# OpenPPL/ppq

Hardware: AMD Instinct MI355X
Metric: calibration samples/sec (RuntimeCalibrationPass, KL 2048-bin, ResNet-50 INT8) (higher is better)
Workload: dtype f32; 1 GPU; ResNet-50 topology (53 Conv + 1 Gemm, BN folded, seeded He init), RuntimeCalibrationPass kl 2048 bins, per-tensor INT8 activations, per-channel INT8 weights, 279 batches x 32 x 3x224x224 per GPU; samples=8928, batch=32, observed_tensors=72, rccl_ranks=1, async_observe=False, cache_params=False, channels_last=False, fuse_params=True, batch_observations=True, reuse_activations=False, replayed_batches=0, hip_graph=auto, graph_replays=0, miopen_find=False

## Files before the change

include/ppq_hip.h:

```cpp
#ifndef PPQ_HIP_H_
#define PPQ_HIP_H_

#include <stdint.h>

#ifdef __cplusplus
extern "C" {
#endif

typedef enum {
    PPQHIP_OK = 0,
    PPQHIP_ERR_INVALID_VALUE = -1,
    PPQHIP_ERR_UNSUPPORTED = -2,
    PPQHIP_ERR_HIP = -3
} ppqhip_status;

#define PPQHIP_ABI_VERSION 4

const char* ppqhip_last_error(void);
int ppqhip_version(void);
int ppqhip_device_arch(char* buf, int n);

int ppqhip_fq_linear_t(const float* x, const float* scale, const float* offset, float* out,
                       int64_t n, int clip_min, int clip_max, int rounding, void* stream);

// ... 49 lines not shown
    int64_t n, num_channel, elem_per_channel;
    int32_t clip_min, clip_max;
} ppqhip_lsq_job;
int ppqhip_fq_linear_c_bwd_multi(const ppqhip_lsq_job* jobs, int num_jobs, int rounding, void* stream);

int ppqhip_fq_float_t(const float* x, const float* scale, const float* offset, float* out,
                      int64_t n, int exponent, int mantissa, float clip_min, float clip_max,
                      int rounding, void* stream);

int ppqhip_fq_float_c(const float* x, const float* scale, const float* offset, float* out,
                      int64_t n, int64_t num_channel, int64_t elem_per_channel,
                      int exponent, int mantissa, float clip_min, float clip_max,
                      int rounding, void* stream);

typedef struct ppqhip_float_search_job {
    const float* x;
    int64_t rows, row_len;
    int32_t exponent, mantissa;
    float clip_min, clip_max;
} ppqhip_float_search_job;
int64_t ppqhip_float_scale_search_table_bytes(int num_jobs);
int ppqhip_float_scale_search(const ppqhip_float_search_job* jobs, int num_jobs, const float* candidates,
                              int num_candidates, int rounding, void* device_table, double* out, void* stream);

typedef struct ppqhip_fq_float_job {
    const float* x;
    const float* scale;
    const float* offset;
    float* out;
    int64_t n, num_channel, elem_per_channel;
    int32_t exponent, mantissa;
    float clip_min, clip_max;
} ppqhip_fq_float_job;
int64_t ppqhip_fq_float_multi_table_bytes(int num_jobs);
int ppqhip_fq_float_multi(const ppqhip_fq_float_job* jobs, int num_jobs, int rounding, void* device_table,
                          int upload, void* stream);

int ppqhip_fq_float_c_bwd(const float* x, const float* scale, const float* offset,
                          const float* grad_y, float* grad_x, float* grad_s, int64_t n,
                          int64_t num_channel, int64_t elem_per_channel,
                          int exponent, int mantissa, float clip_min, float clip_max,
                          int rounding, void* stream);

int64_t ppqhip_hist_workspace_bytes(int64_t n, int64_t num_bins);
int ppqhip_hist_sym_t(const float* x, int64_t n, float hist_scale, int clip_outliers,
                      int32_t* hist, int64_t num_bins, void* workspace, void* stream);

int ppqhip_hist_asym_t(const float* x, int64_t n, float min_value, float max_value,
                       int clip_outliers, int32_t* hist, int64_t num_bins, void* workspace,
                       void* stream);

int ppqhip_hist_sym_c(const float* x, int64_t n, int64_t num_channel, int64_t elem_per_channel,
                      float hist_scale, int clip_outliers, int32_t* hist, int64_t num_bins,
                      void* stream);

int ppqhip_hist_sym_c_scales(const float* x, int64_t n, int64_t num_channel, int64_t elem_per_channel,
                             const float* hist_scales, int clip_outliers, int32_t* hist,
                             int64_t num_bins, void* stream);
int ppqhip_hist_asym_c_ranges(const float* x, int64_t n, int64_t num_channel, int64_t elem_per_channel,
                              const float* mins, const float* maxs, int clip_outliers, int32_t* hist,
                              int64_t num_bins, void* stream);

int64_t ppqhip_quantile_workspace_bytes(int64_t n);
int ppqhip_quantile_t(const float* x, int64_t n, float q, float* dest, uint32_t* hint, void* workspace,
                      void* stream);

typedef struct ppqhip_quantile_job {
    const float* x;
    float* dest;
    uint32_t* hint;
    int64_t n;
} ppqhip_quantile_job;
int64_t ppqhip_quantile_multi_workspace_bytes(int num_jobs, int64_t total_elems);
int ppqhip_quantile_t_multi(const ppqhip_quantile_job* jobs, int num_jobs, float q, void* workspace,
                            void* stream);
void ppqhip_quantile_debug_layout(int64_t* out);
void ppqhip_quantile_hot_layout(int64_t* out);

int ppqhip_isotone_t(const float* x, int64_t n, float* dest, void* workspace, void* stream);

int64_t ppqhip_minmax_workspace_bytes(int64_t n);
int ppqhip_minmax_t(const float* x, int64_t n, float* minmax, void* workspace, void* stream);

int ppqhip_minmax_c(const float* x, int64_t n, int64_t num_channel, int64_t elem_per_channel,
                    float* mins, float* maxs, void* stream);

typedef struct ppqhip_minmax_c_job {
    const float* x;
    float* mins;
    float* maxs;
    int64_t n, num_channel, elem_per_channel;
    int32_t fresh, reserved;
} ppqhip_minmax_c_job;
int ppqhip_minmax_c_multi(const ppqhip_minmax_c_job* jobs, int num_jobs, void* stream);

int ppqhip_channel_sum(const float* x, int64_t n, int64_t num_channel, int64_t elem_per_channel,
                       double* sums, void* stream);

int64_t ppqhip_hist_rows(void);
int ppqhip_hist_sym_t_rows(const float* x, int64_t n, float hist_scale, int clip_outliers,
                           int32_t* rows, int64_t num_bins, void* stream);
int ppqhip_hist_asym_t_rows(const float* x, int64_t n, float min_value, float max_value,
                            int clip_outliers, int32_t* rows, int64_t num_bins, void* stream);
typedef struct ppqhip_minmax_job {
    const float* x;
    float* slots;
    int64_t n;
} ppqhip_minmax_job;
int ppqhip_minmax_t_slots_multi(const ppqhip_minmax_job* jobs, int num_jobs, void* stream);

typedef struct ppqhip_hist_job {
    const float* x;
    int32_t* rows;
    int64_t n;
    float p0, p1;
} ppqhip_hist_job;
int ppqhip_hist_t_rows_multi(const ppqhip_hist_job* jobs, int num_jobs, int asymmetric,
                             int clip_outliers, int64_t num_bins, void* stream);
int ppqhip_hist_rows_finish(const int32_t* rows, int64_t num_bins, int32_t* hist, void* stream);
int ppqhip_check_bin_rule(const float* x, int64_t n, float min_value, float hist_scale, int asymmetric, uint64_t* out, void* stream);
int64_t ppqhip_minmax_slots(void);
int ppqhip_minmax_t_slots(const float* x, int64_t n, float* slots, void* stream);
int ppqhip_minmax_slots_finish(const float* slots, float* minmax, void* stream);

float ppqhip_mse_loss_host(const int64_t* hist, int64_t num_bins, int start, int step, int end);

int64_t ppqhip_mse_search_workspace_bytes(int64_t num_hist);
int ppqhip_mse_search(const int32_t* hist, int64_t num_hist, int64_t num_bins,
                      const double* hist_scale, const double* min_value,
                      int quant_min, int quant_max, int symmetrical, int32_t* best,
                      void* workspace, void* stream);

int64_t ppqhip_kl_num_candidates(int64_t num_bins, int num_of_bits);
int ppqhip_kl_losses(const int32_t* hist, int64_t num_hist, int64_t num_bins, int num_of_bits,
                     double* losses, void* stream);

int ppqhip_tensor_clip_t(const float* value, const float* reference, const float* limit,
                         float* out, int64_t n, void* stream);
int ppqhip_tensor_clip_c(const float* value, const float* reference, const float* limit,
                         float* out, int64_t n, int64_t num_channel, int64_t elem_per_channel,
                         void* stream);
int ppqhip_rounding_loss(const float* x, const float* scale, const float* offset, float* out,
                         int64_t n, int64_t num_channel, int64_t elem_per_channel,
                         int clip_min, int clip_max, int rounding, void* stream);
int ppqhip_rounding_loss_bwd(const float* x, const float* dy, const float* scale,
                             const float* offset, float* dx, int64_t n, int64_t num_channel,
                             int64_t elem_per_channel, int clip_min, int clip_max, int rounding,
                             void* stream);

int ppqhip_bias_act(float* y, const float* bias, int64_t n, int64_t num_channel, int64_t elem_per_channel,
                    int relu, void* stream);
int ppqhip_bias_add_act(float* a, const float* bias_a, float* b, const float* bias_b, float* out,
                        int64_t n, int64_t num_channel, int64_t elem_per_channel, int relu, void* stream);

typedef struct ppqhip_adaround_job {
    const float* w;
    const float* v;
    const float* scale;
    const float* offset;
    float* out;
    const float* dy;
    int64_t n, num_channel, elem_per_channel;
    int32_t qmin, qmax;
} ppqhip_adaround_job;
int ppqhip_adaround_fwd_multi(const ppqhip_adaround_job* jobs, int num_jobs, void* stream);
int ppqhip_adaround_bwd_multi(const ppqhip_adaround_job* jobs, int num_jobs, const float* reg, void* stream);

typedef struct ppqhip_roundtune_job {
    const float* w;
    const float* r;
    const float* scale;
    const float* offset;
    float* out;
    int64_t n, num_channel, elem_per_channel;
    int32_t qmin, qmax;
} ppqhip_roundtune_job;
int ppqhip_roundtune_fwd_multi(const ppqhip_roundtune_job* jobs, int num_jobs, void* stream);

typedef struct ppqhip_fetch_rows_job {
    const float* x;
    const int32_t* index;
    float* out;
    int64_t rows, row_len, count;
} ppqhip_fetch_rows_job;
int ppqhip_fetch_rows_multi(const ppqhip_fetch_rows_job* jobs, int num_jobs, void* stream);
typedef struct ppqhip_measure_rows_job {
    const float* p;
    const float* r;
    const int32_t* index;
    double* sums;
    int64_t rows, row_len, count;
} ppqhip_measure_rows_job;
int ppqhip_measure_rows_multi(const ppqhip_measure_rows_job* jobs, int num_jobs, void* stream);
enum { PPQHIP_MEASURE_SNR = 0, PPQHIP_MEASURE_MSE = 1, PPQHIP_MEASURE_COSINE = 2 };
enum { PPQHIP_REDUCE_MEAN = 0, PPQHIP_REDUCE_MAX = 1 };
typedef struct ppqhip_measure_finish_job {
    const double* sums;
    double* acc;
    float* row_out;
    int64_t rows, count;
    int32_t method, reduce;
} ppqhip_measure_finish_job;
int ppqhip_measure_finish_multi(const ppqhip_measure_finish_job* jobs, int num_jobs, void* stream);

typedef struct ppqhip_equalize_segment {
    const float* base;
    int64_t extent;
    int64_t div, a, b;
    int64_t outer, stride, run;
    float multiplier;
    int32_t downstream;
} ppqhip_equalize_segment;
typedef struct ppqhip_equalize_scale_job {
    const ppqhip_equalize_segment* segments;
    float* scale;
    int32_t num_segments, num_channel;
    float value_threshold;
    int32_t reserved;
} ppqhip_equalize_scale_job;
int ppqhip_equalize_scale_multi(const ppqhip_equalize_scale_job* jobs, int num_jobs, void* stream);
typedef struct ppqhip_equalize_apply_job {
    float* x;
    const float* scale;
    int64_t n, run, inner, group_out;
    int64_t num_scale;
    int32_t divide, reserved;
} ppqhip_equalize_apply_job;
int ppqhip_equalize_apply_multi(const ppqhip_equalize_apply_job* jobs, int num_jobs, void* stream);

typedef struct ppqhip_split_plan_job {
    const ppqhip_equalize_segment* segments;
    int32_t* src_of;
    int32_t* count;
    int32_t num_segments, num_channel;
    float value_threshold;
    int32_t reserved;
} ppqhip_split_plan_job;
int ppqhip_split_plan_multi(const ppqhip_split_plan_job* jobs, int num_jobs, void* stream);
typedef struct ppqhip_split_apply_job {
    const float* x;
    float* out;
    const int32_t* src_of;
    int64_t n, run;
    int32_t num_channel, count;
} ppqhip_split_apply_job;
int ppqhip_split_apply_multi(const ppqhip_split_apply_job* jobs, int num_jobs, void* stream);

typedef struct ppqhip_ssd_scales_job {
    ppqhip_equalize_segment first, last;
    const float* act_range;
    float* scales;
    float* ranges;
    int32_t num_channel;
    float channel_ratio;
} ppqhip_ssd_scales_job;
int ppqhip_ssd_scales_multi(const ppqhip_ssd_scales_job* jobs, int num_jobs, void* stream);
typedef struct ppqhip_ssd_apply_job {
    const float* x;
    float* out;
    const float* scales;
    int64_t n, run, inner, group_out;
    int64_t num_channel;
    int32_t divide, reserved;
} ppqhip_ssd_apply_job;
int ppqhip_ssd_apply_multi(const ppqhip_ssd_apply_job* jobs, int num_jobs, void* stream);
typedef struct ppqhip_fq_measure_rows_job {
    const float* y;
    const float* r;
    const float* scale;
    const float* offset;
    double* sums;
    int64_t rows, count;
    int64_t num_channel, elem_per_channel;
    int32_t clip_min, clip_max, rounding, reserved;
} ppqhip_fq_measure_rows_job;
int ppqhip_fq_measure_rows_multi(const ppqhip_fq_measure_rows_job* jobs, int num_jobs, void* stream);

typedef struct ppqhip_stat_job {
    const float* p;
    const float* r;
    float* rec;
    int64_t n;
    int32_t bins, reserved;
} ppqhip_stat_job;
int ppqhip_stat_moments_multi(const ppqhip_stat_job* jobs, int num_jobs, void* stream);
int ppqhip_stat_shape_multi(const ppqhip_stat_job* jobs, int num_jobs, void* stream);

enum { PPQHIP_MXFP8_E4M3 = 0, PPQHIP_MXFP8_E5M2 = 1, PPQHIP_MXFP6_E3M2 = 2, PPQHIP_MXFP6_E2M3 = 3, PPQHIP_MXFP4_E2M1 = 4,
       PPQHIP_MXINT8 = 5 };
int ppqhip_mx_fq(const float* x, float* y, uint8_t* scale_codes, int64_t outer, int64_t axis_len, int64_t inner, int format,
                 void* stream);
typedef struct ppqhip_mx_job {
    const float* x;
    float* y;
    uint8_t* scale_codes;
    int64_t outer, axis_len, inner;
    int32_t format, reserved;
} ppqhip_mx_job;
int ppqhip_mx_fq_multi(const ppqhip_mx_job* jobs, int num_jobs, void* stream);

int ppqhip_mx_pack(const float* x, uint8_t* elements, uint8_t* scales, int64_t outer, int64_t axis_len, int64_t inner, int format,
                   void* stream);
typedef struct ppqhip_mx_pack_job {
    const float* x;
    uint8_t* elements;
    uint8_t* scales;
// ... 35 lines not shown
```

ppq_amd/_lib.py:

```python
import ctypes
import os

_HERE = os.path.dirname(os.path.abspath(__file__))
LIB_PATH = os.path.join(_HERE, 'libppq_hip.so')

c_f32p = ctypes.c_void_p
c_i32p = ctypes.c_void_p
c_f64p = ctypes.c_void_p
c_i64 = ctypes.c_int64
c_int = ctypes.c_int
c_flt = ctypes.c_float
c_vp = ctypes.c_void_p

ABI_VERSION = 4


class ProfEntry(ctypes.Structure):
    _fields_ = [('name', ctypes.c_char * 48), ('launches', ctypes.c_int64),
                ('total_ms', ctypes.c_double), ('total_bytes', ctypes.c_double)]


PROTOTYPES = {
    'ppqhip_last_error': (ctypes.c_char_p, []),
    'ppqhip_version': (c_int, []),
    'ppqhip_device_arch': (c_int, [ctypes.c_char_p, c_int]),
    'ppqhip_fq_linear_t': (c_int, [c_f32p, c_f32p, c_f32p, c_f32p, c_i64, c_int, c_int, c_int, c_vp]),
    'ppqhip_fq_linear_c': (c_int, [c_f32p, c_f32p, c_f32p, c_f32p, c_i64, c_i64, c_i64, c_int, c_int, c_int, c_vp]),
    'ppqhip_to_int_t': (c_int, [c_f32p, c_f32p, c_f32p, c_vp, c_i64, c_int, c_int, c_int, c_int, c_vp]),
    'ppqhip_to_int_c': (c_int, [c_f32p, c_f32p, c_f32p, c_vp, c_i64, c_i64, c_i64, c_int, c_int, c_int, c_int, c_vp]),
    'ppqhip_fq_linear_t_bwd': (c_int, [c_f32p, c_f32p, c_f32p, c_f32p, c_f32p, c_f32p, c_i64, c_int, c_int, c_int,
                                       c_vp]),
    'ppqhip_fq_linear_c_bwd': (c_int, [c_f32p, c_f32p, c_f32p, c_f32p, c_f32p, c_f32p, c_i64, c_i64, c_i64, c_int,
                                       c_int, c_int, c_vp]),
    'ppqhip_fq_linear_c_bwd_multi': (c_int, [c_vp, c_int, c_int, c_vp]),
    'ppqhip_fq_linear_t_bwd_partials': (c_i64, [c_i64]),
    'ppqhip_fq_linear_t_bwd_main': (c_int, [c_f32p, c_f32p, c_f32p, c_f32p, c_f32p, c_f32p, c_i64, c_int, c_int, c_int, c_vp]),
    'ppqhip_lsq_finish_multi': (c_int, [c_vp, c_int, c_vp]),
    'ppqhip_bias_act': (c_int, [c_f32p, c_f32p, c_i64, c_i64, c_i64, c_int, c_vp]),
    'ppqhip_bias_add_act': (c_int, [c_f32p, c_f32p, c_f32p, c_f32p, c_f32p, c_i64, c_i64, c_i64, c_int, c_vp]),
    'ppqhip_fq_float_t': (c_int, [c_f32p, c_f32p, c_f32p, c_f32p, c_i64, c_int, c_int, c_flt, c_flt, c_int, c_vp]),
    'ppqhip_fq_float_c': (c_int, [c_f32p, c_f32p, c_f32p, c_f32p, c_i64, c_i64, c_i64, c_int, c_int, c_flt, c_flt,
                                  c_int, c_vp]),
    'ppqhip_fq_float_c_bwd': (c_int, [c_f32p, c_f32p, c_f32p, c_f32p, c_f32p, c_f32p, c_i64, c_i64, c_i64, c_int,
                                      c_int, c_flt, c_flt, c_int, c_vp]),
    'ppqhip_hist_workspace_bytes': (c_i64, [c_i64, c_i64]),
    'ppqhip_hist_sym_t': (c_int, [c_f32p, c_i64, c_flt, c_int, c_i32p, c_i64, c_vp, c_vp]),
    'ppqhip_hist_asym_t': (c_int, [c_f32p, c_i64, c_flt, c_flt, c_int, c_i32p, c_i64, c_vp, c_vp]),
    'ppqhip_hist_sym_c': (c_int, [c_f32p, c_i64, c_i64, c_i64, c_flt, c_int, c_i32p, c_i64, c_vp]),
    'ppqhip_hist_sym_c_scales': (c_int, [c_f32p, c_i64, c_i64, c_i64, c_f32p, c_int, c_i32p, c_i64, c_vp]),
    'ppqhip_hist_asym_c_ranges': (c_int, [c_f32p, c_i64, c_i64, c_i64, c_f32p, c_f32p, c_int, c_i32p, c_i64, c_vp]),
    'ppqhip_quantile_workspace_bytes': (c_i64, [c_i64]),
    'ppqhip_quantile_t': (c_int, [c_f32p, c_i64, c_flt, c_f32p, c_vp, c_vp, c_vp]),
    'ppqhip_isotone_t': (c_int, [c_f32p, c_i64, c_f32p, c_vp, c_vp]),
    'ppqhip_minmax_workspace_bytes': (c_i64, [c_i64]),
    'ppqhip_minmax_t': (c_int, [c_f32p, c_i64, c_f32p, c_vp, c_vp]),
    'ppqhip_minmax_c': (c_int, [c_f32p, c_i64, c_i64, c_i64, c_f32p, c_f32p, c_vp]),
    'ppqhip_minmax_c_multi': (c_int, [c_vp, c_int, c_vp]),
    'ppqhip_fq_linear_multi_table_bytes': (c_i64, [c_int]),
    'ppqhip_fq_linear_multi': (c_int, [c_vp, c_int, c_int, c_vp, c_int, c_vp]),
    'ppqhip_float_scale_search_table_bytes': (c_i64, [c_int]),
    'ppqhip_float_scale_search': (c_int, [c_vp, c_int, c_vp, c_int, c_int, c_vp, c_vp, c_vp]),
    'ppqhip_fq_float_multi_table_bytes': (c_i64, [c_int]),
    'ppqhip_fq_float_multi': (c_int, [c_vp, c_int, c_int, c_vp, c_int, c_vp]),
    'ppqhip_quantile_multi_workspace_bytes': (c_i64, [c_int, c_i64]),
    'ppqhip_quantile_t_multi': (c_int, [c_vp, c_int, c_flt, c_vp, c_vp]),
    'ppqhip_quantile_debug_layout': (None, [c_vp]),
    'ppqhip_quantile_hot_layout': (None, [c_vp]),
    'ppqhip_minmax_t_slots_multi': (c_int, [c_vp, c_int, c_vp]),
    'ppqhip_hist_t_rows_multi': (c_int, [c_vp, c_int, c_int, c_int, c_i64, c_vp]),
    'ppqhip_channel_sum': (c_int, [c_f32p, c_i64, c_i64, c_i64, c_f64p, c_vp]),
    'ppqhip_hist_rows': (c_i64, []),
    'ppqhip_hist_sym_t_rows': (c_int, [c_f32p, c_i64, c_flt, c_int, c_i32p, c_i64, c_vp]),
    'ppqhip_hist_asym_t_rows': (c_int, [c_f32p, c_i64, c_flt, c_flt, c_int, c_i32p, c_i64, c_vp]),
    'ppqhip_hist_rows_finish': (c_int, [c_i32p, c_i64, c_i32p, c_vp]),
    'ppqhip_check_bin_rule': (c_int, [c_f32p, c_i64, c_flt, c_flt, c_int, c_vp, c_vp]),
    'ppqhip_minmax_slots': (c_i64, []),
    'ppqhip_minmax_t_slots': (c_int, [c_f32p, c_i64, c_f32p, c_vp]),
    'ppqhip_minmax_slots_finish': (c_int, [c_f32p, c_f32p, c_vp]),
    'ppqhip_mse_loss_host': (c_flt, [ctypes.POINTER(ctypes.c_int64), c_i64, c_int, c_int, c_int]),
    'ppqhip_mse_search_workspace_bytes': (c_i64, [c_i64]),
    'ppqhip_mse_search': (c_int, [c_i32p, c_i64, c_i64, c_f64p, c_f64p, c_int, c_int, c_int, c_i32p, c_vp, c_vp]),
    'ppqhip_kl_num_candidates': (c_i64, [c_i64, c_int]),
    'ppqhip_kl_losses': (c_int, [c_i32p, c_i64, c_i64, c_int, c_f64p, c_vp]),
    'ppqhip_tensor_clip_t': (c_int, [c_f32p, c_f32p, c_f32p, c_f32p, c_i64, c_vp]),
    'ppqhip_tensor_clip_c': (c_int, [c_f32p, c_f32p, c_f32p, c_f32p, c_i64, c_i64, c_i64, c_vp]),
    'ppqhip_rounding_loss': (c_int, [c_f32p, c_f32p, c_f32p, c_f32p, c_i64, c_i64, c_i64, c_int, c_int, c_int, c_vp]),
    'ppqhip_rounding_loss_bwd': (c_int, [c_f32p, c_f32p, c_f32p, c_f32p, c_f32p, c_i64, c_i64, c_i64, c_int, c_int,
                                         c_int, c_vp]),
    'ppqhip_adaround_fwd_multi': (c_int, [c_vp, c_int, c_vp]),
    'ppqhip_adaround_bwd_multi': (c_int, [c_vp, c_int, c_f32p, c_vp]),
    'ppqhip_roundtune_fwd_multi': (c_int, [c_vp, c_int, c_vp]),
    'ppqhip_equalize_scale_multi': (c_int, [c_vp, c_int, c_vp]),
    'ppqhip_equalize_apply_multi': (c_int, [c_vp, c_int, c_vp]),
    'ppqhip_split_plan_multi': (c_int, [c_vp, c_int, c_vp]),
    'ppqhip_split_apply_multi': (c_int, [c_vp, c_int, c_vp]),
    'ppqhip_ssd_scales_multi': (c_int, [c_vp, c_int, c_vp]),
    'ppqhip_ssd_apply_multi': (c_int, [c_vp, c_int, c_vp]),
    'ppqhip_fq_measure_rows_multi': (c_int, [c_vp, c_int, c_vp]),
    'ppqhip_fetch_rows_multi': (c_int, [c_vp, c_int, c_vp]),
    'ppqhip_measure_rows_multi': (c_int, [c_vp, c_int, c_vp]),
    'ppqhip_measure_finish_multi': (c_int, [c_vp, c_int, c_vp]),
    'ppqhip_stat_moments_multi': (c_int, [c_vp, c_int, c_vp]),
    'ppqhip_stat_shape_multi': (c_int, [c_vp, c_int, c_vp]),
    'ppqhip_mx_fq': (c_int, [c_f32p, c_f32p, c_vp, c_i64, c_i64, c_i64, c_int, c_vp]),
    'ppqhip_mx_fq_multi': (c_int, [c_vp, c_int, c_vp]),
    'ppqhip_mx_pack': (c_int, [c_f32p, c_vp, c_vp, c_i64, c_i64, c_i64, c_int, c_vp]),
    'ppqhip_mx_pack_multi': (c_int, [c_vp, c_int, c_vp]),
    'ppqhip_mx_unpack': (c_int, [c_vp, c_vp, c_f32p, c_i64, c_i64, c_i64, c_int, c_vp]),
    'ppqhip_mx_unpack_multi': (c_int, [c_vp, c_int, c_vp]),
    'ppqhip_mx_gemm': (c_int, [c_vp, c_vp, c_int, c_vp, c_vp, c_int, c_f32p, c_f32p, c_i64, c_i64, c_i64, c_vp]),
    'ppqhip_prof_enable': (c_int, [c_int]),
    'ppqhip_prof_collect': (c_int, [ctypes.POINTER(ProfEntry), c_int]),
    'ppqhip_prof_event_overhead_us': (ctypes.c_double, [c_vp, c_int]),
}

if not os.path.exists(LIB_PATH):
    raise ImportError(
        f'{LIB_PATH} is missing: the HIP kernel library has not been built.  Run '
        '`python -c "import __graft_entry__ as g; g.build()"` or `make -C ppq_amd/csrc` (needs hipcc, '
        'targets gfx950).  ppq_amd has no CPU / PyTorch fallback by design.')

import torch

_torch_hip = os.path.join(os.path.dirname(torch.__file__), 'lib', 'libamdhip64.so')
if os.path.exists(_torch_hip):
    ctypes.CDLL(_torch_hip, mode=ctypes.RTLD_GLOBAL)

try:
    lib = ctypes.CDLL(LIB_PATH)
except OSError as e:
    raise ImportError(f'cannot load {LIB_PATH}: {e}') from e

for _name, (_res, _args) in PROTOTYPES.items():
    _fn = getattr(lib, _name)
    _fn.restype = _res
    _fn.argtypes = _args


if lib.ppqhip_version() != ABI_VERSION:
    raise ImportError(f'{LIB_PATH} has ABI version {lib.ppqhip_version()}, this package needs {ABI_VERSION}: rebuild it '
                      '(`make -C ppq_amd/csrc` or `python -c "import __graft_entry__ as g; g.build()"`)')


def last_error() -> str:
    msg = lib.ppqhip_last_error()
    return msg.decode('utf-8', 'replace') if msg else ''
```

ppq_amd/calibration.py:

```python
import time
from math import ceil
from typing import Callable, Dict, Iterable, List

from .core import QuantizationStates, state_value
from .distributed import merge_observers
from .observer import OperationObserver, TorchHistObserver, render_observers


class QuantizationOptimizationPass:
    def __init__(self, name: str = 'Default Quanzation Optim') -> None:
        self.name = name

    def apply(self, graph, **kwargs) -> None:
        self.optimize(graph, **kwargs)

    def optimize(self, graph, **kwargs) -> None:
        raise NotImplementedError('Implement this function first.')

    def __str__(self) -> str:
        return 'QuantizationOptimizationPass[' + self.name + ']'


class RuntimeCalibrationPass(QuantizationOptimizationPass):
    AUTO_GRAPH_ISSUE_FRACTION = 0.7
    AUTO_GRAPH_MIN_STEPS = 12

    def __init__(self, method: str = None, override: bool = False, calib_steps: int = 32,
                 process_group=None, check_steps: bool = True, async_observe: bool = False,
                 use_hip_graph: bool = False, batch_observations: bool = True,
                 reuse_activations: bool = False, reuse_budget_bytes: int = 64 << 30,
                 queue_bytes: int = None) -> None:
        super().__init__(name='PPQ Runtime Calibration Pass')
        self._method = method
        self._observers: Dict[str, OperationObserver] = {}
        self._collate_fn = None
        self._calib_steps = calib_steps
        self._override = override
        self._process_group = process_group
        self._check_steps = check_steps
        self._async_observe = async_observe
        self._use_hip_graph = use_hip_graph
        self._batch_observations = batch_observations
        self._queue = None
        self._reuse_activations = reuse_activations
        self._queue_bytes = queue_bytes
        self._reuse_budget = reuse_budget_bytes
        self._replay: list = []
        self._replay_bytes = 0
        self.replay_peak_bytes = 0
        self.replayed_batches = 0
        self._recording = False
        self.graph_replays = 0
        self.graph_decisions = []
        self.merge_stats = []
        self._side_stream = None

    def _batches(self, dataloader: Iterable) -> list:
        out = []
        for calib_epoch in range(ceil(self._calib_steps / len(dataloader))):
            for data in dataloader:
                if self._collate_fn is not None:
                    data = self._collate_fn(data)
                out.append(data)
                if len(out) >= self._calib_steps: return out
        return out

    def _graph_replayable(self, batches: list, hooks: Dict[str, object]) -> bool:
        import torch
        from .observer import ConstantObserver, TorchHistObserver, TorchMinMaxObserver, TorchMSEObserver
        if not self._use_hip_graph or len(batches) < 4: return False
        if not all(isinstance(b, torch.Tensor) and b.is_cuda and b.shape == batches[0].shape
                   and b.dtype == batches[0].dtype for b in batches): return False
        safe = (TorchMinMaxObserver, TorchHistObserver, TorchMSEObserver, ConstantObserver)
        return all(type(ob) in safe for hook in hooks.values() for ob in hook._observer_table.values())

    @ staticmethod
    def _forward_fn(executor):
        return executor.forward

    def _forward(self, executor, data, hooks, output_names):
        import torch
        recording = self._queue is not None and self._recording
        if recording: self._queue.recorder = []
        with torch.no_grad():
            self._forward_fn(executor)(inputs=data, hooks=hooks, output_names=output_names)
        if self._queue is not None: self._queue.flush()
        if recording:
            rec, self._queue.recorder = self._queue.recorder, None
            size = sum(v.numel() * 4 for _, v in rec)
            if self._replay_bytes + size <= self._reuse_budget:
                self._replay.append(rec); self._replay_bytes += size
                self.replay_peak_bytes = max(self.replay_peak_bytes, self._replay_bytes)
            else: self._recording = False

    def _replay_phase2(self, batches: list) -> int:
        n = min(len(self._replay), len(batches))
        for i in range(n):
            for ob, value in self._replay[i]: ob.observe(value)
            self._queue.flush()
            self._replay[i] = None
        self._replay, self._replay_bytes = [], 0
        self.replayed_batches += n
        return n

    def calibrate(self, desc: str, dataloader: Iterable, executor, hooks: Dict[str, object],
                  output_names: List[str] = None):
        import torch
        batches = self._batches(dataloader)
        if self._replay and not self._recording:
            batches = batches[self._replay_phase2(batches):]
            if not batches: return
        if not self._graph_replayable(batches, hooks):
            for data in batches:
                self._forward(executor, data, hooks, output_names)
            return
        self._forward(executor, batches[0], hooks, output_names)
        first = 1
        if self._use_hip_graph == 'auto':
            torch.cuda.synchronize()
            t0 = time.perf_counter()
            self._forward(executor, batches[1], hooks, output_names)
            t1 = time.perf_counter()
            torch.cuda.synchronize()
            t2 = time.perf_counter()
            first = 2
            launch_bound = (t1 - t0) > self.AUTO_GRAPH_ISSUE_FRACTION * (t2 - t0)
            self.graph_decisions.append({'phase': desc, 'issue_ms': (t1 - t0) * 1e3, 'total_ms': (t2 - t0) * 1e3,
                                         'graph': bool(launch_bound and len(batches) - first >= self.AUTO_GRAPH_MIN_STEPS)})
            if not self.graph_decisions[-1]['graph']:
                for data in batches[first:]:
                    self._forward(executor, data, hooks, output_names)
                return
        self._recording = False
        static_in = torch.empty_like(batches[0])
        torch.cuda.synchronize()
        graph = torch.cuda.CUDAGraph()
        with torch.cuda.graph(graph):
            self._forward(executor, static_in, hooks, output_names)
            if self._side_stream is not None:
                torch.cuda.current_stream().wait_stream(self._side_stream)
        for data in batches[first:]:
            static_in.copy_(data, non_blocking=True)
            graph.replay()
            self.graph_replays += 1

    def _all_tensor_observers(self):
        return [ob for op_ob in self._observers.values() for ob in op_ob.observers()]

    def _render(self):
        observers = self._all_tensor_observers()
        if self._queue is not None: self._queue.flush()
        if self._side_stream is not None:
            import torch
            torch.cuda.current_stream().wait_stream(self._side_stream)
        if merge_observers(observers, group=self._process_group):
            from . import distributed
            self.merge_stats.append(dict(distributed.last_merge_stats))
        render_observers(observers)

    def optimize(self, graph, dataloader: Iterable, executor, calib_steps: int = 32,
                 collate_fn: Callable = None, **kwargs) -> None:
        if collate_fn is not None: self._collate_fn = collate_fn
        if calib_steps is not None: self._calib_steps = calib_steps
        if self._check_steps:
            assert self._calib_steps >= 8, (
                'Insufficient Calibration Detected, to get a better quantization performance, '
                'more calibration steps is required, we strongly recommend you to prepare more calibration data '
                'and more calibration steps is preferred here. (at least 8)')
            assert self._calib_steps <= 512, (
                'Calibration steps is too large, ppq can quantize your network within 8-512 '
                'calibration steps. More calibration steps will greatly delay ppq\'s calibration procedure. '
                'Reset your calib_steps parameter please.')

        if self._override:
            for operation in graph.operations.values():
                if not hasattr(operation, 'config'): continue
                for config, var in operation.config_with_variable:
                    if (not var.is_parameter and state_value(config.state) == QuantizationStates.ACTIVATED.value
                            and config.dominated_by == config):
                        config.state = type(config.state).INITIAL

        self._observers = {}
        hooks = {}
        import torch
        if self._async_observe and torch.cuda.is_available():
            self._side_stream = torch.cuda.Stream()
        for op_name, operation in graph.operations.items():
            if not hasattr(operation, 'config'): continue
            for config, var in operation.config_with_variable:
                if not var.is_parameter and self._method is not None:
                    config.observer_algorithm = self._method
            observer = OperationObserver(operation=executor._graph.operations[op_name], monitor_parameter=False)
            observer.hook.stream = self._side_stream
            self._observers[op_name] = observer
            hooks[op_name] = observer.hook

        self._queue = None
        if self._batch_observations and self._side_stream is None:
            from .observer import ObservationQueue
            self._queue = ObservationQueue() if self._queue_bytes is None else ObservationQueue(self._queue_bytes)
        for ob in self._all_tensor_observers(): ob.queue = self._queue

        self._replay, self._replay_bytes = [], 0
        self._recording = bool(self._reuse_activations and self._queue is not None)
        self.calibrate(desc='Calibration Progress(Phase 1)', dataloader=dataloader, executor=executor,
                       hooks=hooks, output_names=None)
        self._recording = False
        self._render()
        if self._replay:
            for observer in self._observers.values():
                for cfg, ob in observer.hook._observer_table.items():
                    if (not getattr(ob._watch_on, 'is_parameter', False)
                            and QuantizationStates.is_activated(cfg.state)):
                        self._replay, self._replay_bytes = [], 0
                        break
                if not self._replay: break

        pop_list = []
        for op_name, observer in self._observers.items():
            if all([not isinstance(var_observer, TorchHistObserver)
                    for var_observer in observer.observers()]):
                pop_list.append(op_name)
        for op_name in pop_list:
            self._observers.pop(op_name)
            hooks.pop(op_name)

        if len(hooks) > 0:
            self.calibrate(desc='Calibration Progress(Phase 2)', dataloader=dataloader, executor=executor,
                           hooks=hooks, output_names=None)
            self._render()


class PPLDSPTIReCalibrationPass(RuntimeCalibrationPass):
    def __init__(self, method: str = None, override: bool = False) -> None:
        super().__init__(method, override)
        self.name = 'PPQ ReCalibration For Computing Op Pass'

    def optimize(self, graph, dataloader: Iterable, executor, calib_steps: int, collate_fn: Callable = None, **kwargs) -> None:
# ... 91 lines not shown
```

ppq_amd/csrc/epilogue.hip:

```cpp
#include "common.hpp"

namespace ppqhip {
namespace {

constexpr int kEpTileU = 2;
constexpr int kEpSmallU = 1;
constexpr long long kEpSmallElems = 1ll << 20;

struct EpArgs {
    float* a;
    const float* bias_a;
    float* b;
    const float* bias_b;
    float* out;
    uint32_t nvec;
    uint32_t tail;
    int ntail;
    FastDiv epc;
    FastDiv nc;
};

__device__ __forceinline__ uint32_t channel_of(uint32_t i, const FastDiv& epc, const FastDiv& nc) {
    const uint32_t row = fdiv(i, epc);
    return row - fdiv(row, nc) * nc.d;
}

__device__ __forceinline__ float act(float v, bool relu) {
    return (relu && !__builtin_isnan(v)) ? __builtin_fmaxf(v, 0.f) : v;
}

__device__ __forceinline__ float4 add4(const float4& x, const float4& y) {
    return make_float4(x.x + y.x, x.y + y.y, x.z + y.z, x.w + y.w);
}

template <bool RELU>
__device__ __forceinline__ float4 act4(const float4& v) {
    return make_float4(act(v.x, RELU), act(v.y, RELU), act(v.z, RELU), act(v.w, RELU));
}

template <bool PLANE>
__device__ __forceinline__ float4 bias4(const float* __restrict__ bias, uint32_t v, const FastDiv& epc, const FastDiv& nc) {
    if (PLANE) {
        const float t = bias[channel_of(v, epc, nc)];
        return make_float4(t, t, t, t);
    }
    const uint32_t i = v * 4u;
    return make_float4(bias[channel_of(i, epc, nc)], bias[channel_of(i + 1, epc, nc)], bias[channel_of(i + 2, epc, nc)],
                       bias[channel_of(i + 3, epc, nc)]);
}

template <bool RESID, bool BIAS_B, bool RELU>
__device__ __forceinline__ void epilogue_elem(const EpArgs& p, uint32_t i, const FastDiv& epc) {
    const uint32_t c = channel_of(i, epc, p.nc);
    const float x = p.a[i] + p.bias_a[c];
    if (!RESID) { p.a[i] = act(x, RELU); return; }
    p.a[i] = x;
    float y = p.b[i];
    if (BIAS_B) { y = y + p.bias_b[c]; p.b[i] = y; }
    p.out[i] = act(x + y, RELU);
}

template <int U, bool RESID, bool BIAS_B, bool RELU, bool PLANE>
__global__ __launch_bounds__(kBlock) void epilogue_kernel(EpArgs p) {
    const uint32_t base = blockIdx.x * (kBlock * U) + threadIdx.x;
    float4* a4 = reinterpret_cast<float4*>(p.a);
    float4* b4 = reinterpret_cast<float4*>(p.b);
    float4* o4 = reinterpret_cast<float4*>(p.out);
    float4 a[U], ba[U], b[U], bb[U];
#pragma unroll
    for (int k = 0; k < U; k++) {
        const uint32_t vv = min(base + k * kBlock, p.nvec - 1);
        a[k] = a4[vv];
        ba[k] = bias4<PLANE>(p.bias_a, vv, p.epc, p.nc);
        if (RESID) b[k] = b4[vv];
        if (BIAS_B) bb[k] = bias4<PLANE>(p.bias_b, vv, p.epc, p.nc);
    }
#pragma unroll
    for (int k = 0; k < U; k++) {
        const uint32_t vv = base + k * kBlock;
        if (vv >= p.nvec) continue;
        const float4 x = add4(a[k], ba[k]);
        if (!RESID) { a4[vv] = act4<RELU>(x); continue; }
        a4[vv] = x;
        float4 y = b[k];
        if (BIAS_B) { y = add4(y, bb[k]); b4[vv] = y; }
        o4[vv] = act4<RELU>(add4(x, y));
    }
    if (!PLANE && blockIdx.x == 0 && (int)threadIdx.x < p.ntail)
        epilogue_elem<RESID, BIAS_B, RELU>(p, p.tail + threadIdx.x, p.epc);
}

template <bool RESID, bool BIAS_B, bool RELU>
__global__ __launch_bounds__(kBlock) void epilogue_scalar_kernel(EpArgs p) {
    const uint32_t stride = gridDim.x * kBlock;
    for (uint32_t i = blockIdx.x * kBlock + threadIdx.x; i < (uint32_t)p.ntail; i += stride)
        epilogue_elem<RESID, BIAS_B, RELU>(p, i, p.epc);
}

template <bool RESID, bool BIAS_B, bool RELU>
void launch_epilogue(EpArgs p, int64_t n, int64_t C, int64_t epc, bool aligned, hipStream_t st) {
    p.nc = make_fastdiv((uint32_t)C);
    if (!aligned || n < 4) {
        p.nvec = 0; p.tail = 0; p.ntail = (int)n;
        p.epc = make_fastdiv((uint32_t)epc);
        hipLaunchKernelGGL((epilogue_scalar_kernel<RESID, BIAS_B, RELU>), dim3(stream_grid(n, kBlock)), dim3(kBlock), 0, st, p);
        return;
    }
    p.nvec = (uint32_t)(n >> 2);
    p.tail = p.nvec * 4u;
    p.ntail = (int)(n & 3);
    const bool plane = (epc % 4 == 0);
    p.epc = make_fastdiv((uint32_t)(plane ? epc / 4 : epc));
#define PPQ_LAUNCH_EP(U, PLANE)                                                                                          \
    hipLaunchKernelGGL((epilogue_kernel<U, RESID, BIAS_B, RELU, PLANE>), dim3((p.nvec + kBlock * U - 1) / (kBlock * U)),   \
                       dim3(kBlock), 0, st, p)
    if (n <= kEpSmallElems) {
        if (plane) PPQ_LAUNCH_EP(kEpSmallU, true); else PPQ_LAUNCH_EP(kEpSmallU, false);
    } else {
        if (plane) PPQ_LAUNCH_EP(kEpTileU, true); else PPQ_LAUNCH_EP(kEpTileU, false);
    }
#undef PPQ_LAUNCH_EP
}

int validate(int64_t n, int64_t C, int64_t epc, const char* what) {
    if (n <= 0 || n > 0x7fffffffLL) {
        set_error("%s: n=%lld is empty or has more than 2^31 - 1 elements", what, (long long)n);
        return PPQHIP_ERR_INVALID_VALUE;
    }
    if (C <= 0 || epc <= 0 || C > 0x7fffffffLL || epc > 0x7fffffffLL || n % (C * epc) != 0) {
        set_error("%s: n=%lld is not [outer, %lld channels, %lld elem/channel]", what, (long long)n, (long long)C,
                  (long long)epc);
        return PPQHIP_ERR_INVALID_VALUE;
    }
    return PPQHIP_OK;
}

}
}

using namespace ppqhip;

extern "C" {

int ppqhip_bias_act(float* y, const float* bias, int64_t n, int64_t num_channel, int64_t elem_per_channel, int relu,
                    void* stream) {
    if (int st = validate(n, num_channel, elem_per_channel, "bias_act")) return st;
    if (!y || !bias) { set_error("bias_act: null pointer"); return PPQHIP_ERR_INVALID_VALUE; }
    hipStream_t s = (hipStream_t)stream;
    EpArgs p{};
    p.a = y; p.bias_a = bias;
    const bool aligned = aligned16(y);
    if (relu) launch_epilogue<false, false, true>(p, n, num_channel, elem_per_channel, aligned, s);
    else launch_epilogue<false, false, false>(p, n, num_channel, elem_per_channel, aligned, s);
    return finish_launch("bias_act");
}

int ppqhip_bias_add_act(float* a, const float* bias_a, float* b, const float* bias_b, float* out, int64_t n,
                        int64_t num_channel, int64_t elem_per_channel, int relu, void* stream) {
    if (int st = validate(n, num_channel, elem_per_channel, "bias_add_act")) return st;
    if (!a || !bias_a || !b || !out) { set_error("bias_add_act: null pointer"); return PPQHIP_ERR_INVALID_VALUE; }
    hipStream_t s = (hipStream_t)stream;
    EpArgs p{};
    p.a = a; p.bias_a = bias_a; p.b = b; p.bias_b = bias_b; p.out = out;
    const bool aligned = aligned16(a) && aligned16(b) && aligned16(out);
    if (bias_b) {
        if (relu) launch_epilogue<true, true, true>(p, n, num_channel, elem_per_channel, aligned, s);
        else launch_epilogue<true, true, false>(p, n, num_channel, elem_per_channel, aligned, s);
    } else {
        if (relu) launch_epilogue<true, false, true>(p, n, num_channel, elem_per_channel, aligned, s);
        else launch_epilogue<true, false, false>(p, n, num_channel, elem_per_channel, aligned, s);
    }
    return finish_launch("bias_add_act");
}

}
```

ppq_amd/csrc/hist.hip:

```cpp
#include "common.hpp"

namespace ppqhip {

constexpr int kMaxLdsBins = 16384;
constexpr int kLdsBudgetInts = 2048;
constexpr int kHistBlock = 512;
constexpr int kHistWgPerCu = 2;
constexpr int kHistU = 2;
constexpr int kHistMinTiles = 2;
constexpr int kHistAtomicMaxWg = 128;
constexpr long long kHistNtElems = 48ll << 20;
constexpr int kHistRows = kNumCU * kHistWgPerCu;
constexpr uint32_t kTileVec = (uint32_t)kHistBlock * kHistU;
constexpr uint32_t kTileElems = kTileVec * 4;
static_assert(kHistBlock % 64 == 0 && kHistBlock >= 64 && kHistBlock <= 1024, "histogram workgroup: whole waves");

typedef float v2f __attribute__((ext_vector_type(2)));

struct BinRule {
    float a;
    float hs;
    float rcp;
    int bins;
    int clip;
    int asym;
};
static BinRule make_rule(float a, float hs, int bins, int clip, int asym) {
    BinRule r; r.a = a; r.hs = hs; r.rcp = 1.0f / hs; r.bins = bins; r.clip = clip; r.asym = asym;
    return r;
}

__device__ __forceinline__ bool quotient_is_safe(float t) {
    return __builtin_fabsf(t - __builtin_rintf(t)) >= __builtin_fabsf(t) * 0x1p-22f;
}

__device__ __forceinline__ int f2i_abs(float t) {
    int r;
    asm("v_cvt_i32_f32_e64 %0, |%1|" : "=v"(r) : "v"(t));
    return r;
}
__device__ __forceinline__ int f2i_floor(float t) {
    int r;
    asm("v_cvt_flr_i32_f32 %0, %1" : "=v"(r) : "v"(t));
    return r;
}

template <bool ASYM, bool CLIP, bool HOT>
struct Binner : WaveBinCounter<ASYM, CLIP, HOT> {
    using Base = WaveBinCounter<ASYM, CLIP, HOT>;
    using Base::h; using Base::last; using Base::hot_bin; using Base::hot_cnt;
    float a0, hs, rcp;

    __device__ __forceinline__ void set_rule(float a, float scale) { a0 = a; hs = scale; rcp = 1.0f / scale; }

    __device__ __forceinline__ void bins4(const float4& v, int (&b)[4]) const {
        v2f x01 = {v.x, v.y}, x23 = {v.z, v.w};
        if (ASYM) { x01 = x01 - a0; x23 = x23 - a0; }
        const v2f t01 = x01 * rcp, t23 = x23 * rcp;
        const v2f r01 = {__builtin_rintf(t01.x), __builtin_rintf(t01.y)};
        const v2f r23 = {__builtin_rintf(t23.x), __builtin_rintf(t23.y)};
        const v2f d01 = t01 - r01, d23 = t23 - r23;
        const v2f e01 = t01 * 0x1p-22f, e23 = t23 * 0x1p-22f;
        const bool u0 = !(__builtin_fabsf(d01.x) >= __builtin_fabsf(e01.x));
        const bool u1 = !(__builtin_fabsf(d01.y) >= __builtin_fabsf(e01.y));
        const bool u2 = !(__builtin_fabsf(d23.x) >= __builtin_fabsf(e23.x));
        const bool u3 = !(__builtin_fabsf(d23.y) >= __builtin_fabsf(e23.y));
        b[0] = ASYM ? f2i_floor(t01.x) : f2i_abs(t01.x);
        b[1] = ASYM ? f2i_floor(t01.y) : f2i_abs(t01.y);
        b[2] = ASYM ? f2i_floor(t23.x) : f2i_abs(t23.x);
        b[3] = ASYM ? f2i_floor(t23.y) : f2i_abs(t23.y);
        if (u0 | u1 | u2 | u3) {
            if (u0) b[0] = exact_bin(ASYM ? x01.x : __builtin_fabsf(v.x));
            if (u1) b[1] = exact_bin(ASYM ? x01.y : __builtin_fabsf(v.y));
            if (u2) b[2] = exact_bin(ASYM ? x23.x : __builtin_fabsf(v.z));
            if (u3) b[3] = exact_bin(ASYM ? x23.y : __builtin_fabsf(v.w));
        }
    }
    __device__ __forceinline__ int exact_bin(float a) const { return f2i_sat(__builtin_floorf(a / hs)); }

    __device__ __forceinline__ int bin1(float v) const {
        const float a = ASYM ? (v - a0) : __builtin_fabsf(v);
        const float t = a * rcp;
        if (quotient_is_safe(t)) return ASYM ? f2i_floor(t) : f2i_abs(t);
        return exact_bin(a);
    }

};

constexpr int kReduceBins = 32, kReduceSlices = 32, kReduceBlock = kReduceBins * kReduceSlices;
__global__ __launch_bounds__(kReduceBlock) void hist_reduce_kernel(const int* __restrict__ partial, int count, int bins,
                                                                   int* __restrict__ hist) {
    __shared__ int lds[kReduceSlices][kReduceBins];
    const int lane_bin = threadIdx.x % kReduceBins, slice = threadIdx.x / kReduceBins;
    const int b = blockIdx.x * kReduceBins + lane_bin;
    int total = 0;
    if (b < bins) {
        int i = slice;
        for (; i + 15 * kReduceSlices < count; i += 16 * kReduceSlices) {
            int v[16];
#pragma unroll
            for (int k = 0; k < 16; k++) v[k] = partial[(size_t)(i + k * kReduceSlices) * bins + b];
#pragma unroll
            for (int k = 0; k < 16; k++) total += v[k];
        }
        for (; i < count; i += kReduceSlices) total += partial[(size_t)i * bins + b];
    }
    lds[slice][lane_bin] = total;
    __syncthreads();
    if (slice == 0 && b < bins) {
        int t = 0;
#pragma unroll
        for (int k = 0; k < kReduceSlices; k++) t += lds[k][lane_bin];
        if (t) hist[b] += t;
    }
}

constexpr int kMultiMax = 96;
enum FlushMode : int {
    FLUSH_ROWS_ADD = 0,
    FLUSH_ROWS_STORE = 1,
    FLUSH_ATOMIC = 2
};
struct HistJob {
    const float* x;
    int* rows;
    uint32_t n;
    float a, hs;
    uint32_t first_tile;
};
struct HistJobs {
    HistJob job[kMultiMax];
    uint32_t count;
    uint32_t total_tiles;
    int bins, copies, mode;
};
__host__ __device__ inline uint32_t job_tiles(uint32_t n, bool vec_ok) {
    if (!vec_ok) return (n + kTileElems - 1) / kTileElems;
    const uint32_t full = (n >> 2) / kTileVec;
    return full + (n > full * kTileElems ? 1u : 0u);
}

__device__ __forceinline__ void lds_hist_flush(int* lds, int bins, int copies, int* __restrict__ dst, int mode) {
    asm volatile("s_waitcnt lgkmcnt(0)" ::: "memory");
    __syncthreads();
    for (int b = threadIdx.x; b < bins; b += kHistBlock) {
        int s = 0;
        for (int c = 0; c < copies; c++) { s += lds[c * bins + b]; lds[c * bins + b] = 0; }
        if (mode == FLUSH_ROWS_STORE) dst[b] = s;
        else if (s) {
            if (mode == FLUSH_ROWS_ADD) dst[b] += s;
            else atomicAdd(&dst[b], s);
        }
    }
    __syncthreads();
}

template <bool ASYM, bool CLIP, bool HOT, bool NT>
__global__ __launch_bounds__(kHistBlock, (kHistBlock * kHistWgPerCu + 255) / 256)
void hist_persistent_kernel(const HistJobs jobs) {
    extern __shared__ int lds[];
    const uint32_t G = gridDim.x, g = blockIdx.x;
    uint32_t t, t_end;
    even_split(jobs.total_tiles, G, g, t, t_end);
    const int bins = jobs.bins, copies = jobs.copies;
    bool zeroed = false;
    auto zero_lds = [&]() {
        if (zeroed) return;
        for (int i = threadIdx.x; i < copies * bins; i += kHistBlock) lds[i] = 0;
        asm volatile("s_waitcnt lgkmcnt(0)\n\ts_barrier" ::: "memory");
        zeroed = true;
    };
    if (t >= t_end) {
        if (jobs.mode == FLUSH_ROWS_STORE) for (int b = threadIdx.x; b < bins; b += kHistBlock) jobs.job[0].rows[(size_t)g * bins + b] = 0;
        return;
    }
    uint32_t lo = 0, hi = jobs.count;
    while (hi - lo > 1) {
        const uint32_t mid = (lo + hi) >> 1;
        if (jobs.job[mid].first_tile <= t) lo = mid; else hi = mid;
    }
    Binner<ASYM, CLIP, HOT> acc;
    acc.init(lds + ((threadIdx.x >> 6) % copies) * bins, bins);

    for (uint32_t j = lo; t < t_end; j++) {
        const HistJob& job = jobs.job[j];
        const uint32_t j_end = (j + 1 < jobs.count) ? jobs.job[j + 1].first_tile : jobs.total_tiles;
        uint32_t k = t - job.first_tile;
        const uint32_t k1 = min(t_end, j_end) - job.first_tile;
        t = min(t_end, j_end);
        acc.set_rule(job.a, job.hs);
        const float* __restrict__ x = job.x;
        const uint32_t n = job.n;
        const bool vec_ok = (reinterpret_cast<uintptr_t>(x) & 15u) == 0;
        const uint32_t full = vec_ok ? (n >> 2) / kTileVec : 0u;
        const uint32_t kf = min(k1, full);
        if (k < kf) {
            const float4* xv = reinterpret_cast<const float4*>(x) + threadIdx.x;
            float4 bufa[kHistU], bufb[kHistU];
            auto fetch = [&](float4 (&buf)[kHistU], uint32_t tile) {
                const float4* p = xv + (size_t)tile * kTileVec;
#pragma unroll
                for (int u = 0; u < kHistU; u++) buf[u] = load4<NT>(p + u * kHistBlock);
            };
            auto consume = [&](const float4 (&buf)[kHistU], uint32_t tile) {
#pragma unroll
                for (int u = 0; u < kHistU; u++) {
                    int b[4];
                    acc.bins4(buf[u], b);
                    if (u == 0) acc.elect(b[0], true);
                    if (CLIP && HOT) acc.commit4_exec(b);
                    else {
                        acc.template commit<true>(b[0], true); acc.template commit<true>(b[1], true);
                        acc.template commit<true>(b[2], true); acc.template commit<true>(b[3], true);
                    }
                }
            };
            fetch(bufa, k);
            zero_lds();
            for (;;) {
                fetch(bufb, min(k + 1, kf - 1));
                consume(bufa, k);
                if (++k >= kf) break;
                fetch(bufa, min(k + 1, kf - 1));
                consume(bufb, k);
                if (++k >= kf) break;
            }
        }
        zero_lds();
        for (; k < k1; k++) {
            const uint32_t e0 = k * kTileElems + threadIdx.x;
#pragma unroll 4
            for (int r = 0; r < 4 * kHistU; r++) {
                const uint32_t i = e0 + r * kHistBlock;
                const bool in = i < n;
                const float a = in ? x[i] : 0.f;
                const int b = acc.bin1(a);
                if ((r & 3) == 0) acc.elect(b, in);
                acc.template commit<false>(b, in);
            }
        }
// ... 659 lines not shown
```

ppq_amd/ffi.py:

```python
import math
import threading
import weakref
from typing import List

import numpy as np
import torch

from . import _lib
from ._lib import lib

_KERNEL_FAILURE = 'Kernel Failure, '


_raw_stream = torch._C._cuda_getCurrentRawStream
_get_device = torch._C._cuda_getDevice


def _stream() -> int:
    return _raw_stream(_get_device())


def _check(t: torch.Tensor, dtype: torch.dtype, name: str) -> None:
    if not isinstance(t, torch.Tensor):
        raise TypeError(f'{name}: expected a torch.Tensor, got {type(t)}')
# ... 7 lines not shown

_F32 = torch.float32


def _f32(t, name):
    try:
        if t.dtype is _F32 and t.is_cuda and t.numel() > 0: return
    except AttributeError:
        pass
    _check(t, torch.float32, name + '(Expect to be FP32)')


def _dense(t: torch.Tensor, channel_axis=None) -> torch.Tensor:
    if t.is_contiguous(): return t
    if channel_axis is None or channel_axis % t.dim() == 0:
        if t.dim() == 4 and t.is_contiguous(memory_format=torch.channels_last): return t
        if t.dim() == 5 and t.is_contiguous(memory_format=torch.channels_last_3d): return t
    return t.contiguous()


def _raise(status: int) -> None:
    if status != 0:
        raise RuntimeError(_KERNEL_FAILURE + _lib.last_error())


def _geometry(shape, channel_axis: int):
    ndim = len(shape)
    if channel_axis < 0: channel_axis += ndim
    if not 0 <= channel_axis < ndim:
        raise RuntimeError(_KERNEL_FAILURE + f'channel_axis {channel_axis} out of range for a {ndim}-d tensor')
    epc = 1
    for d in shape[channel_axis + 1:]:
        epc *= int(d)
    return int(shape[channel_axis]), epc


class _DeviceOf:
    __slots__ = ('idx', 'prev')

    def __init__(self, t: torch.Tensor):
        self.idx = t.device.index
        self.prev = None

    def __enter__(self):
        if self.idx is not None and self.idx != _get_device():
            self.prev = _get_device()
            torch.cuda.set_device(self.idx)

    def __exit__(self, *a):
        if self.prev is not None:
            torch.cuda.set_device(self.prev)


_workspaces = {}
_MAX_WORKSPACES = 16


def _workspace(device: torch.device, nbytes: int) -> torch.Tensor:
    key = (device.index, _stream())
    ws = _workspaces.pop(key, None)
    if ws is None or ws.numel() < nbytes:
        ws = torch.empty(max(nbytes, 1 << 16), dtype=torch.uint8, device=device)
    _workspaces[key] = ws
    while len(_workspaces) > _MAX_WORKSPACES:
        _workspaces.pop(next(iter(_workspaces)))
    return ws


_MINMAX_JOB = np.dtype([('x', '<u8'), ('slots', '<u8'), ('n', '<i8')])
_FQ_JOB = np.dtype([('x', '<u8'), ('scale', '<u8'), ('offset', '<u8'), ('out', '<u8'), ('n', '<i8'),
                    ('num_channel', '<i8'), ('elem_per_channel', '<i8'), ('clip_min', '<i4'), ('clip_max', '<i4')])
_FQ_FLOAT_JOB = np.dtype([('x', '<u8'), ('scale', '<u8'), ('offset', '<u8'), ('out', '<u8'), ('n', '<i8'),
                          ('num_channel', '<i8'), ('elem_per_channel', '<i8'), ('exponent', '<i4'), ('mantissa', '<i4'),
                          ('clip_min', '<f4'), ('clip_max', '<f4')])
_FLOAT_SEARCH_JOB = np.dtype([('x', '<u8'), ('rows', '<i8'), ('row_len', '<i8'), ('exponent', '<i4'), ('mantissa', '<i4'),
                              ('clip_min', '<f4'), ('clip_max', '<f4')])
_LSQ_JOB = np.dtype([('x', '<u8'), ('scale', '<u8'), ('offset', '<u8'), ('grad_y', '<u8'), ('grad_x', '<u8'), ('grad_s', '<u8'),
                     ('n', '<i8'), ('num_channel', '<i8'), ('elem_per_channel', '<i8'), ('clip_min', '<i4'), ('clip_max', '<i4')])
_LSQ_FINISH_JOB = np.dtype([('partial', '<u8'), ('grad_s', '<u8'), ('n', '<i8'), ('clip_min', '<i4'), ('clip_max', '<i4')])
_MINMAX_C_JOB = np.dtype([('x', '<u8'), ('mins', '<u8'), ('maxs', '<u8'), ('n', '<i8'), ('num_channel', '<i8'),
                          ('elem_per_channel', '<i8'), ('fresh', '<i4'), ('reserved', '<i4')])
_QUANTILE_JOB = np.dtype([('x', '<u8'), ('dest', '<u8'), ('hint', '<u8'), ('n', '<i8')])

_owner_hints = weakref.WeakKeyDictionary()
_hint_owner = threading.local()


def quantile_hint(device: torch.device) -> torch.Tensor:
    return torch.zeros(8, dtype=torch.int32, device=device)


class quantile_hint_owner:
    __slots__ = ('owner', 'prev')

    def __init__(self, owner):
        self.owner, self.prev = owner, None

    def __enter__(self):
        self.prev = getattr(_hint_owner, 'current', None)
        _hint_owner.current = self.owner
        return self

    def __exit__(self, *a):
        _hint_owner.current = self.prev


def _owner_quantile_hint(device: torch.device, numel: int, q: float):
    owner = getattr(_hint_owner, 'current', None)
    if owner is None: return None
    try: per = _owner_hints.setdefault(owner, {})
    except TypeError: return None
    key = (device.index, int(numel), float(q))
    h = per.get(key)
    if h is None: h = per[key] = quantile_hint(device)
    return h


_HIST_JOB = np.dtype([('x', '<u8'), ('rows', '<u8'), ('n', '<i8'), ('p0', '<f4'), ('p1', '<f4')])


def _epilogue_geometry(ts, bias_list):
    t0 = ts[0]
    if not isinstance(t0, torch.Tensor) or t0.dtype is not _F32 or not t0.is_cuda or t0.dim() != 4 or t0.numel() == 0:
        return None
    shape, strides, dev = t0.shape, t0.stride(), t0.device
    for t in ts[1:]:
        if not isinstance(t, torch.Tensor) or t.dtype is not _F32 or t.device != dev or t.shape != shape or t.stride() != strides:
            return None
    C = int(shape[1])
    for bias in bias_list:
        if (not isinstance(bias, torch.Tensor) or bias.dtype is not _F32 or bias.device != dev or bias.dim() != 1
                or bias.numel() != C or not bias.is_contiguous()):
            return None
    if t0.is_contiguous(): return C, int(shape[2]) * int(shape[3])
    if t0.is_contiguous(memory_format=torch.channels_last): return C, 1
    return None


def bias_act_(y: torch.Tensor, bias: torch.Tensor, relu: bool) -> bool:
    geo = _epilogue_geometry([y], [bias])
    if geo is None: return False
    with _DeviceOf(y):
        _raise(lib.ppqhip_bias_act(y.data_ptr(), bias.data_ptr(), y.numel(), geo[0], geo[1], 1 if relu else 0, _stream()))
    return True


def bias_add_act(a: torch.Tensor, bias_a: torch.Tensor, b: torch.Tensor, bias_b, relu: bool):
    geo = _epilogue_geometry([a, b], [bias_a] if bias_b is None else [bias_a, bias_b])
    if geo is None or a.data_ptr() == b.data_ptr(): return None
    out = torch.empty_like(a)
    with _DeviceOf(a):
        _raise(lib.ppqhip_bias_add_act(a.data_ptr(), bias_a.data_ptr(), b.data_ptr(), 0 if bias_b is None else bias_b.data_ptr(),
                                       out.data_ptr(), a.numel(), geo[0], geo[1], 1 if relu else 0, _stream()))
    return out


_ADAROUND_JOB = np.dtype([('w', '<u8'), ('v', '<u8'), ('scale', '<u8'), ('offset', '<u8'), ('out', '<u8'), ('dy', '<u8'),
                          ('n', '<i8'), ('num_channel', '<i8'), ('elem_per_channel', '<i8'), ('qmin', '<i4'), ('qmax', '<i4')])


def _adaround_table(items, outs, dys=None):
    n = len(items)
    if len(outs) != n or (dys is not None and len(dys) != n):
        raise RuntimeError(_KERNEL_FAILURE + 'AdaRound: argument lists differ in length')
    jobs = np.zeros(n, dtype=_ADAROUND_JOB)
    dev = items[0][0].device
    for k, (w, v, s, o, axis, qmin, qmax) in enumerate(items):
        ts = [('Value', w), ('Rounding', v), ('Scale', s), ('Offset', o), ('Out', outs[k])] + ([('Dy', dys[k])] if dys is not None else [])
        for name, t in ts:
            _f32(t, name)
            if t.device != dev: raise RuntimeError(_KERNEL_FAILURE + f'AdaRound: item {k}: {name} is on another device')
            if not t.is_contiguous(): raise RuntimeError(_KERNEL_FAILURE + f'AdaRound: item {k}: {name} is not contiguous')
        for name, t in ts[1:2] + ts[4:]:
            if t.shape != w.shape: raise RuntimeError(_KERNEL_FAILURE + f'AdaRound: item {k}: {name} is not shaped like the weight')
        C, epc = _geometry(w.shape, axis) if axis is not None else (1, w.numel())
        if s.numel() != C or o.numel() != C:
            raise RuntimeError(_KERNEL_FAILURE + f'AdaRound: item {k}: scale / offset need {C} elements')
        jobs[k] = (w.data_ptr(), v.data_ptr(), s.data_ptr(), o.data_ptr(), outs[k].data_ptr(),
                   dys[k].data_ptr() if dys is not None else 0, w.numel(), C, epc, int(qmin), int(qmax))
    return jobs


def adaround_forward_multi(items, outs=None) -> List[torch.Tensor]:
    if not items: return []
    if outs is None: outs = [torch.empty_like(it[0]) for it in items]
    jobs = _adaround_table(items, outs)
    with _DeviceOf(items[0][0]):
        _raise(lib.ppqhip_adaround_fwd_multi(jobs.ctypes.data, len(items), _stream()))
    return outs


def adaround_backward_multi(items, dys, reg: torch.Tensor, dvs=None) -> List[torch.Tensor]:
    if not items: return []
    _f32(reg, 'Reg')
    if reg.numel() != 3 or not reg.is_contiguous() or reg.device != items[0][0].device:
        raise RuntimeError(_KERNEL_FAILURE + 'AdaRound: reg must be a contiguous float32[3] on the weights\' device')
    if dvs is None: dvs = [torch.empty_like(it[0]) for it in items]
    jobs = _adaround_table(items, dvs, dys)
    with _DeviceOf(items[0][0]):
        _raise(lib.ppqhip_adaround_bwd_multi(jobs.ctypes.data, len(items), reg.data_ptr(), _stream()))
    return dvs


_ROUNDTUNE_JOB = np.dtype([('w', '<u8'), ('r', '<u8'), ('scale', '<u8'), ('offset', '<u8'), ('out', '<u8'),
                           ('n', '<i8'), ('num_channel', '<i8'), ('elem_per_channel', '<i8'), ('qmin', '<i4'), ('qmax', '<i4')])


def _roundtune_table(items, outs):
    n = len(items)
    if len(outs) != n: raise RuntimeError(_KERNEL_FAILURE + 'RoundTuning: argument lists differ in length')
    jobs = np.zeros(n, dtype=_ROUNDTUNE_JOB)
    dev = items[0][0].device
    for k, (w, r, s, o, axis, qmin, qmax) in enumerate(items):
        ts = [('Value', w), ('Rounding', r), ('Scale', s), ('Offset', o), ('Out', outs[k])]
        for name, t in ts:
            _f32(t, name)
            if t.device != dev: raise RuntimeError(_KERNEL_FAILURE + f'RoundTuning: item {k}: {name} is on another device')
            if not t.is_contiguous(): raise RuntimeError(_KERNEL_FAILURE + f'RoundTuning: item {k}: {name} is not contiguous')
        for name, t in ts[1:2] + ts[4:]:
            if t.shape != w.shape: raise RuntimeError(_KERNEL_FAILURE + f'RoundTuning: item {k}: {name} is not shaped like the weight')
        C, epc = _geometry(w.shape, axis) if axis is not None else (1, w.numel())
        if s.numel() != C or o.numel() != C:
            raise RuntimeError(_KERNEL_FAILURE + f'RoundTuning: item {k}: scale / offset need {C} elements')
        jobs[k] = (w.data_ptr(), r.data_ptr(), s.data_ptr(), o.data_ptr(), outs[k].data_ptr(), w.numel(), C, epc, int(qmin), int(qmax))
    return jobs


def roundtune_forward_multi(items, outs=None) -> List[torch.Tensor]:
    if not items: return []
    if outs is None: outs = [torch.empty_like(it[0]) for it in items]
    jobs = _roundtune_table(items, outs)
    with _DeviceOf(items[0][0]):
        _raise(lib.ppqhip_roundtune_fwd_multi(jobs.ctypes.data, len(items), _stream()))
    return outs


_EQ_SEGMENT = np.dtype([('base', '<u8'), ('extent', '<i8'), ('div', '<i8'), ('a', '<i8'), ('b', '<i8'), ('outer', '<i8'),
                        ('stride', '<i8'), ('run', '<i8'), ('multiplier', '<f4'), ('downstream', '<i4')])
_EQ_SCALE_JOB = np.dtype([('segments', '<u8'), ('scale', '<u8'), ('num_segments', '<i4'), ('num_channel', '<i4'),
                          ('value_threshold', '<f4'), ('reserved', '<i4')])
_EQ_APPLY_JOB = np.dtype([('x', '<u8'), ('scale', '<u8'), ('n', '<i8'), ('run', '<i8'), ('inner', '<i8'), ('group_out', '<i8'),
                          ('num_scale', '<i8'), ('divide', '<i4'), ('reserved', '<i4')])


def _eq_tensor(t, what: str, k: int, dev):
    _f32(t, what)
    if t.device != dev: raise RuntimeError(_KERNEL_FAILURE + f'Equalization: item {k}: {what} is on another device')
    if not t.is_contiguous(): raise RuntimeError(_KERNEL_FAILURE + f'Equalization: item {k}: {what} is not contiguous')


def _segment_record(segment, k: int, dev, what: str = 'Value') -> tuple:
    t, div, a, b, outer, stride, run, mult, down = segment
    _eq_tensor(t, what, k, dev)
    return (t.data_ptr(), t.numel(), int(div), int(a), int(b), int(outer), int(stride), int(run), float(mult), 1 if down else 0)


class EqualizeTable:
    __slots__ = ('jobs', 'segments', 'keep', 'entry')

    def __init__(self, jobs, segments, keep, entry):
        self.jobs, self.segments, self.keep, self.entry = jobs, segments, keep, entry

    def __len__(self) -> int: return len(self.jobs)

    def run(self) -> None:
        if len(self.jobs) == 0: return
        with _DeviceOf(self.keep[0]):
            _raise(self.entry(self.jobs.ctypes.data, len(self.jobs), _stream()))


def equalize_scale_table(items) -> EqualizeTable:
    jobs = np.zeros(len(items), dtype=_EQ_SCALE_JOB)
    segs = np.zeros(sum(len(it[2]) for it in items), dtype=_EQ_SEGMENT)
    keep, records = [], []
    dev = items[0][0].device if items else None
    for k, (scale, threshold, segments) in enumerate(items):
        _eq_tensor(scale, 'Scale', k, dev)
        keep.append(scale)
        jobs[k] = (segs.ctypes.data + len(records) * _EQ_SEGMENT.itemsize, scale.data_ptr(), len(segments), scale.numel(), float(threshold), 0)
        for segment in segments:
            records.append(_segment_record(segment, k, dev))
            keep.append(segment[0])
    segs[:] = records
    return EqualizeTable(jobs, segs, keep, lib.ppqhip_equalize_scale_multi)


def equalize_apply_table(items) -> EqualizeTable:
    jobs = np.zeros(len(items), dtype=_EQ_APPLY_JOB)
    keep = []
    dev = items[0][0].device if items else None
    for k, (x, scale, run, inner, group_out, divide) in enumerate(items):
        _eq_tensor(x, 'Value', k, dev); _eq_tensor(scale, 'Scale', k, dev)
        keep += [x, scale]
        jobs[k] = (x.data_ptr(), scale.data_ptr(), x.numel(), int(run), int(inner), int(group_out), scale.numel(), 1 if divide else 0, 0)
    return EqualizeTable(jobs, None, keep, lib.ppqhip_equalize_apply_multi)


def equalize_scale_multi(items) -> None:
    (items if isinstance(items, EqualizeTable) else equalize_scale_table(items)).run()


def equalize_apply_multi(items) -> None:
    (items if isinstance(items, EqualizeTable) else equalize_apply_table(items)).run()


_SPLIT_PLAN_JOB = np.dtype([('segments', '<u8'), ('src_of', '<u8'), ('count', '<u8'), ('num_segments', '<i4'), ('num_channel', '<i4'),
# ... 1498 lines not shown
```

ppq_amd/harness.py:

```python
from typing import Callable, Dict, List, Optional

import torch
import torch.nn.functional as F

from .core import LinearQuantizationConfig, QuantizationStates, TensorQuantizationConfig, is_initial
from .core import QuantizationProperty as P
from .qfunction import PPQuantFunction

PASSIVE_OPERATIONS = {'MaxPool', 'GlobalMaxPool', 'Reshape', 'Flatten', 'Identity', 'Dropout', 'Slice', 'Pad', 'Resize',
                      'Split', 'Transpose', 'Interp', 'Squeeze', 'Unsqueeze'}
COMPUTING_OP = {'Conv', 'Gemm', 'ConvTranspose', 'MatMul'}


class Variable:
    def __init__(self, name: str, value: torch.Tensor = None, is_parameter: bool = False):
        self.name = name
        self.value = value
        self.stored_value = None
        self.is_parameter = is_parameter
        self.dest_ops: List['Operation'] = []
        self.source_op: Optional['Operation'] = None

    def __hash__(self): return hash(self.name)
    def __eq__(self, o): return isinstance(o, Variable) and o.name == self.name
# ... 60 lines not shown
        return self

    def baking_parameters(self, quant_func: Callable):
        for config, var in self.config_with_variable:
            if var.is_parameter and QuantizationStates.is_activated(config.state):
                var.value = quant_func(var.value, config)
                config.state = (QuantizationStates.BAKED if config.state == QuantizationStates.ACTIVATED
                                else QuantizationStates.PASSIVE_BAKED)


class BaseGraph:
    def __init__(self, name: str):
        self.name = name
        self.operations: Dict[str, Operation] = {}
        self.variables: Dict[str, Variable] = {}
        self.inputs: Dict[str, Variable] = {}
        self.outputs: Dict[str, Variable] = {}

    def create_variable(self, name: str, value=None, is_parameter=False) -> Variable:
        v = Variable(name, value, is_parameter)
        self.variables[name] = v
        return v

    def create_operation(self, op_type: str, name: str, inputs: List[Variable], attributes: dict = None) -> Variable:
        out = self.create_variable(name + '_out')
        op = Operation(name, op_type, attributes, list(inputs), [out])
        out.source_op = op
        for v in inputs: v.dest_ops.append(op)
        self.operations[name] = op
        return out

    def topological_sort(self) -> List[Operation]:
        return list(self.operations.values())


def _forward(op: Operation, x: List[torch.Tensor]):
    t, a = op.type, op.attributes
    if t == 'Conv':
        return F.conv2d(x[0], x[1], x[2] if len(x) > 2 else None, stride=a.get('strides', 1),
                        padding=a.get('pads', 0), groups=a.get('group', 1))
    if t == 'Gemm': return F.linear(x[0], x[1], x[2] if len(x) > 2 else None)
    if t == 'MatMul': return torch.matmul(x[0], x[1])
    if t == 'Relu': return F.relu(x[0])
    if t == 'Gelu': return F.gelu(x[0])
    if t == 'Add': return x[0] + x[1]
    if t == 'MaxPool': return F.max_pool2d(x[0], a['kernel_shape'], a.get('strides', 1), a.get('pads', 0))
    if t == 'GlobalAveragePool': return F.adaptive_avg_pool2d(x[0], 1)
    if t == 'Flatten': return torch.flatten(x[0], 1)
    if t == 'LayerNormalization': return F.layer_norm(x[0], x[0].shape[-1:], x[1], x[2])
    if t == 'Softmax': return F.softmax(x[0], dim=a.get('axis', -1))
    if t == 'Mul': return x[0] * (x[1] if len(x) > 1 else a['value'])
    if t == 'Reshape': return x[0].reshape(a['shape'])
    if t == 'Transpose': return x[0].permute(a['perm'])
    if t == 'Concat': return torch.cat([v.expand(x[-1].shape[0], *v.shape[1:]) if v.shape[0] == 1 else v for v in x],
                                       dim=a.get('axis', 1))
    if t == 'Slice': return x[0].narrow(a['axis'], a['start'], a['length'])
    if t == 'Resize': return F.interpolate(x[0], scale_factor=a.get('scale', 2), mode=a.get('mode', 'nearest'))
    raise NotImplementedError(f'Graph op: {op.name}({op.type}) has no backend implementation')


class EpilogueGroup:
    __slots__ = ('kind', 'ops', 'convs', 'add', 'relu')

    def __init__(self, kind, ops, convs, add, relu):
        self.kind, self.ops, self.convs, self.add, self.relu = kind, ops, convs, add, relu

    def __repr__(self): return f'{self.kind}({", ".join(op.name for op in self.ops)})'


def _in_cfg(op, i):
    return op.config.input_quantization_config[i] if isinstance(op, QuantableOperation) else None


def _out_cfg(op, i):
    return op.config.output_quantization_config[i] if isinstance(op, QuantableOperation) else None


def plan_epilogues(operations: List[Operation], hooks: Dict[str, object] = None, keep=(), passes_through: Callable = None,
                   grad_enabled: bool = False) -> List[EpilogueGroup]:
    if grad_enabled: return []
    from .observer import CalibrationHook
    hooks = hooks or {}
    keep = set(keep)
    if passes_through is None:
        def passes_through(c): return not QuantizationStates.is_activated(c.state)

    def through(*cfgs): return all(c is None or passes_through(c) for c in cfgs)

    def hooks_ok(members, unwritten):
        for op in members:
            h = hooks.get(op.name)
            if h is None: continue
            if type(h) is not CalibrationHook: return False
            if any(c is not None and c in h._observer_table for c in unwritten): return False
        return True

    def conv_ok(op):
        return (op.type == 'Conv' and len(op.inputs) == 3 and op.inputs[2].is_parameter and len(op.outputs) == 1
                and op.outputs[0].name not in keep)

    def only_feeds(v, op): return len(v.dest_ops) == 1 and v.dest_ops[0] is op

    def relu_after(op, i):
        if i >= len(operations): return None
        r = operations[i]
        out = op.outputs[0]
        if r.type != 'Relu' or len(r.inputs) != 1 or r.inputs[0] is not out or not only_feeds(out, r) or out.name in keep:
            return None
        return r

    def try_p2(i):
        for n_conv in (2, 1):
            j = i + n_conv
            if j + 1 >= len(operations): continue
            add, convs = operations[j], operations[i:j]
            if add.type != 'Add' or len(add.inputs) != 2 or len(add.outputs) != 1 or not all(conv_ok(c) for c in convs): continue
            by_out = {c.outputs[0].name: c for c in convs}
            x0, x1 = add.inputs
            if x0.name not in by_out or x0 is x1: continue
            if n_conv == 2 and x1.name not in by_out: continue
            ordered = [by_out[x0.name]] + ([by_out[x1.name]] if n_conv == 2 else [])
            if not all(only_feeds(c.outputs[0], add) for c in convs): continue
            relu = relu_after(add, j + 1)
            if relu is None: continue
            unwritten = (_out_cfg(add, 0), _in_cfg(relu, 0))
            between = [_out_cfg(c, 0) for c in convs] + [_in_cfg(add, 0), _in_cfg(add, 1)]
            if not through(*unwritten, *between): return None
            members = list(operations[i:j + 2])
            if not hooks_ok(members, unwritten): return None
            return EpilogueGroup('P2', members, ordered, add, relu)
        return None

    def try_p1(i):
        conv = operations[i]
        if not conv_ok(conv): return None
        relu = relu_after(conv, i + 1)
        if relu is None: return None
        unwritten = (_out_cfg(conv, 0), _in_cfg(relu, 0))
        if not through(*unwritten) or not hooks_ok([conv, relu], unwritten): return None
        return EpilogueGroup('P1', [conv, relu], [conv], None, relu)

    groups, i = [], 0
    while i < len(operations):
        g = try_p2(i) if operations[i].type == 'Conv' else None
        if g is None and operations[i].type == 'Conv': g = try_p1(i)
        if g is None:
            i += 1
            continue
        groups.append(g)
        i += len(g.ops)
    return groups


class TorchExecutor:
    def __init__(self, graph: BaseGraph, device: str = 'cuda'):
        self._graph = graph
        self._device = device
        self._default_quant_fn = PPQuantFunction
        self.cache_parameter_quantization = False
        self._param_cache: Dict[str, tuple] = {}
        self.fuse_parameter_quantization = True
        self._plans: list = []
        self._plan_signature = None
        self._plan_cache: Dict[tuple, list] = {}
        self._fused: Dict[tuple, torch.Tensor] = {}
        self._delegates: Dict[object, Callable] = {}
        self.fuse_epilogues = True
        self._epilogue_cache: Dict[tuple, dict] = {}
        self.channels_last = False
        for v in graph.variables.values():
            if v.is_parameter and v.value is not None: v.value = v.value.to(device)

    def use_channels_last(self) -> 'TorchExecutor':
        self.channels_last = True
        for v in self._graph.variables.values():
            if v.is_parameter and isinstance(v.value, torch.Tensor) and v.value.dim() == 4:
                v.value = v.value.contiguous(memory_format=torch.channels_last)
        return self

    def _place(self, value: torch.Tensor) -> torch.Tensor:
        value = value.to(self._device)
        if self.channels_last and value.dim() == 4: value = value.contiguous(memory_format=torch.channels_last)
        return value

    def register_quantize_delegate(self, config, delegator: Callable) -> None:
        self._delegates[config] = delegator

    def remove_quantize_delegate(self, config) -> None:
        self._delegates.pop(config, None)

    def quantize_function(self, tensor: torch.Tensor, config=None) -> torch.Tensor:
        if self._delegates and config in self._delegates:
            return self._delegates[config](tensor, config)
        return self._default_quant_fn(tensor, config)

    def forward_with_gradient(self, inputs, output_names: List[str] = None, hooks=None):
        return TorchExecutor.forward.__wrapped__(self, inputs, output_names, hooks)

    def partial_graph_forward(self, operations: List[Operation], feed_dict: Dict[str, torch.Tensor],
                              output_names: List[str], with_gradient: bool = False) -> List[torch.Tensor]:
        if not with_gradient:
            with torch.no_grad(): return self._partial_graph_forward(operations, feed_dict, output_names)
        return self._partial_graph_forward(operations, feed_dict, output_names)

    def _partial_graph_forward(self, operations, feed_dict, output_names):
        g = self._graph
        for name, value in feed_dict.items(): g.variables[name].value = self._place(value)
        results = [None] * len(output_names)
        self._fused_parameters(operations)
        plan, fused_done = self._epilogue_plan(operations, None, output_names), set()
        for op in operations:
            if op.name in fused_done: continue
            grp = plan.get(op.name)
            vals = self._run_epilogue(grp, lambda v: v.value, None) if grp is not None else None
            if vals is not None:
                for m in grp.ops:
                    fused_done.add(m.name)
                    for v in m.outputs:
                        v.value = vals[v.name]
                        if v.name in output_names: results[output_names.index(v.name)] = v.value
                continue
            raw_in = [v.value for v in op.inputs]
            if any(x is None for x in raw_in):
                raise ValueError(f'partial_graph_forward: input of {op.name} was not fed')
            if isinstance(op, QuantableOperation):
                qin = [self._quantize_parameter(v, c) if v.is_parameter else self.quantize_function(x, c)
                       for v, x, c in zip(op.inputs, raw_in, op.config.input_quantization_config)]
            else: qin = raw_in
            outs = _forward(op, qin)
            outs = list(outs) if isinstance(outs, (list, tuple)) else [outs]
            if isinstance(op, QuantableOperation):
                outs = [self.quantize_function(y, c) for y, c in zip(outs, op.config.output_quantization_config)]
            for v, y in zip(op.outputs, outs):
                v.value = y
                if v.name in output_names: results[output_names.index(v.name)] = y
        for v in g.variables.values():
            if not v.is_parameter: v.value = None
        return results

    def _fused_parameters(self, operations=None) -> None:
        self._fused = {}
        if not self.fuse_parameter_quantization or self._default_quant_fn is not PPQuantFunction: return
        from .ffi import FloatingQuantizePlan, LinearQuantizePlan
        todo, sig = [], []
        for op in (self._graph.operations.values() if operations is None else operations):
            if not isinstance(op, QuantableOperation): continue
            for v, c in zip(op.inputs, op.config.input_quantization_config):
                if not (v.is_parameter and isinstance(v.value, torch.Tensor) and v.value.is_cuda): continue
                if not QuantizationStates.is_activated(c.state) or c in self._delegates: continue
                pol = c.policy
                floating = pol.has_property(P.FLOATING)
                if not (pol.has_property(P.LINEAR) or floating) or pol.has_property(P.DYNAMIC): continue
                if v.value.dtype != torch.float32 or v.value.requires_grad or v.value.numel() == 0: continue
                if not (isinstance(c.scale, torch.Tensor) and isinstance(c.offset, torch.Tensor)): continue
                axis = c.channel_axis if pol.has_property(P.PER_CHANNEL) else None
                if not LinearQuantizePlan.accepts(v.value, c.scale, c.offset, axis): continue
                rnd = int(getattr(c.rounding, 'value', c.rounding))
                todo.append((v, c, axis, rnd, floating))
                sig.append((v.name, id(c), v.value.data_ptr(), c.scale.data_ptr(), c.offset.data_ptr(), tuple(v.value.shape), c.scale.numel(),
                            axis, c.quant_min, c.quant_max, rnd, floating,
                            (c.exponent_bits, c.mantissa_bits) if floating else None))
        if not todo:
            self._plans, self._plan_signature = [], None
            return
        cached = self._plan_cache.get(tuple(sig))
        if cached is not None:
            self._plan_cache[tuple(sig)] = self._plan_cache.pop(tuple(sig))
            self._plans, self._plan_signature = cached, sig
        if sig != self._plan_signature:
            groups: Dict[tuple, list] = {}
            for item in todo: groups.setdefault((item[3], item[4]), []).append(item)
            self._plans = []
            for (rnd, floating), items in groups.items():
                if floating:
                    plan = FloatingQuantizePlan([(v.value, c.scale, c.offset, axis, c.exponent_bits, c.mantissa_bits,
                                                  c.quant_min, c.quant_max) for v, c, axis, _, _ in items], rounding=rnd)
                else:
                    plan = LinearQuantizePlan([(v.value, c.scale, c.offset, axis, c.quant_min, c.quant_max)
                                               for v, c, axis, _, _ in items], rounding=rnd)
                self._plans.append((plan, [(v.name, id(c)) for v, c, _, _, _ in items]))
            self._plan_signature = sig
            if len(self._plan_cache) >= 8: self._plan_cache.pop(next(iter(self._plan_cache)))
            self._plan_cache[tuple(sig)] = self._plans
        for plan, keys in self._plans:
            for key, out in zip(keys, plan.run()): self._fused[key] = out

    def _epilogue_plan(self, operations: List[Operation], hooks, output_names) -> Dict[str, EpilogueGroup]:
        if not self.fuse_epilogues or torch.is_grad_enabled() or self._default_quant_fn is not PPQuantFunction: return {}
        states = tuple(c.state for op in operations if isinstance(op, QuantableOperation)
                       for c in (*op.config.input_quantization_config, *op.config.output_quantization_config))
        sig = (tuple(op.name for op in operations), tuple((k, id(h)) for k, h in hooks.items()) if hooks else (),
               tuple(output_names or ()), tuple(id(c) for c in self._delegates), states)
        plan = self._epilogue_cache.get(sig)
        if plan is None:
            delegates = self._delegates

            def passes_through(c): return not QuantizationStates.is_activated(c.state) and c not in delegates
            groups = plan_epilogues(operations, hooks, set(self._graph.outputs) | set(output_names or ()), passes_through)
            plan = {g.ops[0].name: g for g in groups}
            if len(self._epilogue_cache) >= 8: self._epilogue_cache.pop(next(iter(self._epilogue_cache)))
            self._epilogue_cache[sig] = plan
        return plan

    def _run_epilogue(self, grp: EpilogueGroup, raw_of: Callable, hooks) -> Optional[Dict[str, torch.Tensor]]:
        from .ffi import bias_act_, bias_add_act
        for conv in grp.convs:
            x, w = raw_of(conv.inputs[0]), conv.inputs[1].value
            if not (isinstance(x, torch.Tensor) and x.is_cuda and x.dtype == torch.float32 and x.dim() == 4
                    and isinstance(w, torch.Tensor) and w.dim() == 4): return None
            fmt = torch.channels_last if self.channels_last else torch.contiguous_format
            if not (x.is_contiguous(memory_format=fmt) and w.is_contiguous(memory_format=fmt)): return None
        if grp.add is not None:
            b_var = grp.add.inputs[1]
            if b_var.source_op not in grp.convs:
                b = raw_of(b_var)
                if not (isinstance(b, torch.Tensor) and b.is_cuda and b.dtype == torch.float32): return None
        hooks = hooks or {}
        ys, biases, qins = {}, {}, {}
        for conv in grp.ops[:len(grp.convs)]:
            raw_in = [raw_of(v) for v in conv.inputs]
            qin, in_cfgs = raw_in, None
            if isinstance(conv, QuantableOperation):
                in_cfgs = list(conv.config.input_quantization_config)
                qin = [self._quantize_parameter(v, c) if v.is_parameter else self.quantize_function(x, c)
                       for v, x, c in zip(conv.inputs, raw_in, in_cfgs)]
            hook = hooks.get(conv.name)
            if hook is not None: qin = hook.pre_forward_hook(inputs=raw_in, quant_inputs=qin, quant_configs=in_cfgs)
            a = conv.attributes
            ys[conv.name] = F.conv2d(qin[0], qin[1], None, stride=a.get('strides', 1), padding=a.get('pads', 0),
                                     groups=a.get('group', 1))
            biases[conv.name] = qin[2]
            qins[conv.name] = qin
        if grp.kind == 'P1':
            conv = grp.convs[0]
            y = ys[conv.name]
            if not bias_act_(y, biases[conv.name], relu=True):
                y.add_(biases[conv.name].view(1, -1, 1, 1)).relu_()
            tail = {conv.name: y, grp.relu.name: y}
        else:
            conv_a = grp.convs[0]
            a = ys[conv_a.name]
            conv_b = grp.convs[1] if len(grp.convs) > 1 else None
            b = ys[conv_b.name] if conv_b is not None else raw_of(grp.add.inputs[1])
            out = bias_add_act(a, biases[conv_a.name], b, biases[conv_b.name] if conv_b is not None else None, relu=True)
            if out is None:
                a.add_(biases[conv_a.name].view(1, -1, 1, 1))
                if conv_b is not None: b.add_(biases[conv_b.name].view(1, -1, 1, 1))
                out = F.relu(a + b)
            tail = {conv_a.name: a, grp.add.name: out, grp.relu.name: out}
            if conv_b is not None: tail[conv_b.name] = b
        values: Dict[str, torch.Tensor] = {}
        for op in grp.ops:
            hook = hooks.get(op.name)
            quantable = isinstance(op, QuantableOperation)
            if op.type != 'Conv':
                raw_in = [values[v.name] if v.name in values else raw_of(v) for v in op.inputs]
                qin, in_cfgs = raw_in, None
                if quantable:
                    in_cfgs = list(op.config.input_quantization_config)
                    qin = [self.quantize_function(x, c) for x, c in zip(raw_in, in_cfgs)]
                if hook is not None: hook.pre_forward_hook(inputs=raw_in, quant_inputs=qin, quant_configs=in_cfgs)
            outs = fp_outs = [tail[op.name]]
            out_cfgs = None
            if quantable:
                out_cfgs = list(op.config.output_quantization_config)
                outs = [self.quantize_function(y, c) for y, c in zip(outs, out_cfgs)]
            if hook is not None:
                outs = hook.post_forward_hook(outputs=fp_outs, quant_outputs=outs, quant_configs=out_cfgs)
            for v, y in zip(op.outputs, outs): values[v.name] = y
        return values

    def _quantize_parameter(self, var: Variable, config) -> torch.Tensor:
        hit = self._fused.get((var.name, id(config)))
        if hit is not None: return hit
        """A parameter and its scale do not change between calibration forwards, so its fake-quantised
        value is computed once and kept resident (the reference recomputes it every forward until
        ParameterBakingPass; same values, ppq/executor/torch.py:516-518).  The cache entry is keyed on
        the identity + version of value, scale and offset and on the config state."""
        if not self.cache_parameter_quantization or not QuantizationStates.is_activated(config.state):
            return self.quantize_function(var.value, config)
        key = (var.value.data_ptr(), var.value._version, id(config.scale), config.scale._version,
               id(config.offset), config.offset._version, int(getattr(config.state, 'value', config.state)))
        hit = self._param_cache.get(var.name)
        if hit is not None and hit[0] == key: return hit[1]
        q = self.quantize_function(var.value, config)
        self._param_cache[var.name] = (key, q)
        return q

    @ torch.no_grad()
    def forward_cached(self, inputs, output_names: List[str], cache: Dict[str, torch.Tensor]) -> List[torch.Tensor]:
        g = self._graph
        if isinstance(inputs, torch.Tensor): inputs = {next(iter(g.inputs)): inputs}
        elif isinstance(inputs, (list, tuple)): inputs = {k: v for k, v in zip(g.inputs, inputs)}
        for name, value in inputs.items():
            if name not in cache: cache[name] = self._place(value)
        need, stack = set(), [g.variables[n] for n in output_names]
        while stack:
            v = stack.pop()
            if v.name in cache or v.is_parameter: continue
            op = v.source_op
            if op is None: raise ValueError(f'forward_cached: graph input {v.name} was not fed')
            if op.name in need: continue
            need.add(op.name)
            stack.extend(op.inputs)
        ops = [op for op in g.topological_sort() if op.name in need]
        if ops: self._fused_parameters(ops)
        plan, fused_done = (self._epilogue_plan(ops, None, output_names) if ops else {}), set()
        for op in ops:
            if op.name in fused_done: continue
            grp = plan.get(op.name)
            vals = (self._run_epilogue(grp, lambda v: v.value if v.is_parameter else cache[v.name], None)
                    if grp is not None else None)
            if vals is not None:
                hidden = grp.relu.inputs[0].name
                for m in grp.ops:
                    fused_done.add(m.name)
                    for v in m.outputs:
                        if v.name != hidden: cache[v.name] = vals[v.name]
                continue
            raw_in = [v.value if v.is_parameter else cache[v.name] for v in op.inputs]
            if isinstance(op, QuantableOperation):
                qin = [self._quantize_parameter(v, c) if v.is_parameter else self.quantize_function(x, c)
                       for v, x, c in zip(op.inputs, raw_in, op.config.input_quantization_config)]
            else: qin = raw_in
            outs = _forward(op, qin)
            outs = list(outs) if isinstance(outs, (list, tuple)) else [outs]
            if isinstance(op, QuantableOperation):
                outs = [self.quantize_function(y, c) for y, c in zip(outs, op.config.output_quantization_config)]
            for v, y in zip(op.outputs, outs): cache[v.name] = y
        return [cache[n] for n in output_names]

    @ torch.no_grad()
    def forward(self, inputs, output_names: List[str] = None, hooks: Dict[str, object] = None) -> List[torch.Tensor]:
        g = self._graph
        if isinstance(inputs, torch.Tensor): inputs = {next(iter(g.inputs)): inputs}
        elif isinstance(inputs, (list, tuple)): inputs = {k: v for k, v in zip(g.inputs, inputs)}
        for name, value in inputs.items(): g.variables[name].value = self._place(value)
        stop_early = output_names is not None and not hooks
        if output_names is None: output_names = list(g.outputs)
        results = [None] * len(output_names)
        visited = set()
        self._fused_parameters()
        ops = g.topological_sort()
        plan, fused_done = self._epilogue_plan(ops, hooks, output_names), set()

        def finish(op, outs):
            for v, y in zip(op.outputs, outs):
                v.value = y
                if v.name in output_names: results[output_names.index(v.name)] = y
            visited.add(op.name)
            for v in op.inputs:
                if not v.is_parameter and all(d.name in visited for d in v.dest_ops): v.value = None

        for op in ops:
            if op.name in fused_done: continue
            grp = plan.get(op.name)
            vals = self._run_epilogue(grp, lambda v: v.value, hooks) if grp is not None else None
            if vals is not None:
                for m in grp.ops:
                    fused_done.add(m.name)
                    finish(m, [vals[v.name] for v in m.outputs])
                if stop_early and all(r is not None for r in results): break
                continue
            hook = hooks.get(op.name) if hooks else None
            raw_in = [v.value for v in op.inputs]
            qin = raw_in
            quantable = isinstance(op, QuantableOperation)
            if quantable:
                in_cfgs = list(op.config.input_quantization_config)
                qin = [self._quantize_parameter(v, c) if v.is_parameter else self.quantize_function(x, c)
                       for v, x, c in zip(op.inputs, raw_in, in_cfgs)]
            if hook is not None:
                qin = hook.pre_forward_hook(inputs=raw_in, quant_inputs=qin, quant_configs=in_cfgs)
            outs = _forward(op, qin)
            outs = list(outs) if isinstance(outs, (list, tuple)) else [outs]
            fp_outs = outs
            if quantable:
                out_cfgs = list(op.config.output_quantization_config)
                outs = [self.quantize_function(y, c) for y, c in zip(outs, out_cfgs)]
            if hook is not None:
                outs = hook.post_forward_hook(outputs=fp_outs, quant_outputs=outs, quant_configs=out_cfgs)
            finish(op, outs)
            if stop_early and all(r is not None for r in results): break
        for v in g.variables.values():
            if not v.is_parameter: v.value = None
        return results


def quantize_graph(graph: BaseGraph, activation_algorithm: str = 'kl', per_channel_weight: bool = True,
                   symmetrical: bool = True, weight_symmetrical: bool = True, num_of_bits: int = 8,
                   hist_bins: int = None, fp8: bool = False, passive_bias: bool = False) -> None:
    qmin, qmax = (-(2 ** (num_of_bits - 1)), 2 ** (num_of_bits - 1) - 1) if symmetrical else (0, 2 ** num_of_bits - 1)
    wmin, wmax = (-(2 ** (num_of_bits - 1)), 2 ** (num_of_bits - 1) - 1) if weight_symmetrical else (0, 2 ** num_of_bits - 1)

    def act_cfg():
        if fp8:
            from .core import FloatingQuantizationConfig
            return FloatingQuantizationConfig(calibration='floating')
        c = LinearQuantizationConfig(symmetrical=symmetrical, quant_min=qmin, quant_max=qmax, num_of_bits=num_of_bits,
                                     calibration=activation_algorithm)
        if hist_bins is not None: c.detail['OBSERVER_KL_HIST_BINS_MANUL_OVERRIDE'] = hist_bins
        return c

    for name, op in list(graph.operations.items()):
        in_cfgs = []
        for i, v in enumerate(op.inputs):
            if v.is_parameter and op.type in COMPUTING_OP and i == 1:
                in_cfgs.append(LinearQuantizationConfig(symmetrical=weight_symmetrical, quant_min=wmin, quant_max=wmax,
                                                        num_of_bits=num_of_bits, calibration='minmax',
                                                        channel_axis=0 if per_channel_weight else None))
            elif v.is_parameter and passive_bias and not fp8 and op.type in COMPUTING_OP and i == 2:
                in_cfgs.append(LinearQuantizationConfig(symmetrical=True, quant_min=-(2 ** 31 - 1), quant_max=2 ** 31 - 1, num_of_bits=32,
                                                        calibration=None, channel_axis=0 if per_channel_weight else None))
                in_cfgs[-1].state = QuantizationStates.PASSIVE_INIT
            elif v.is_parameter:
                c = act_cfg(); c.state = QuantizationStates.FP32
                in_cfgs.append(c)
            else:
                in_cfgs.append(act_cfg())
        qop = QuantableOperation(op, OperationQuantizationConfig(in_cfgs, [act_cfg() for _ in op.outputs]))
        for v in qop.inputs: v.dest_ops[v.dest_ops.index(op)] = qop
# ... 253 lines not shown
```

ppq_amd/observer.py:

```python
from typing import Dict, List, Optional, Sequence, Tuple

import weakref

import numpy as np
import torch

from .core import (OBSERVER_FLOATING_MSE_FETCHES, OBSERVER_ISOTONE_OBSERVER_AXIS, OBSERVER_KL_HIST_BINS, OBSERVER_KL_HIST_BINS_MANUL_OVERRIDE,
                   OBSERVER_MIN_SCALE, OBSERVER_MIN_SCALE_MANUL_OVERRIDE, OBSERVER_MSE_HIST_BINS,
                   OBSERVER_PERCENTILE, OBSERVER_PERCENTILE_MANUL_OVERRIDE, is_initial, set_activated)
from .core import QuantizationProperty as P
from .core import RoundingPolicy
from .ffi import CUDA, quantile_hint
from .round import ppq_numerical_round, ppq_round_to_power_of_2


def minmax_to_scale_offset(min_val: float, max_val: float, config,
                           scale_threshold: float = OBSERVER_MIN_SCALE) -> Tuple[float, float]:
    if OBSERVER_MIN_SCALE_MANUL_OVERRIDE in config.detail:
        scale_threshold = config.detail[OBSERVER_MIN_SCALE_MANUL_OVERRIDE]
    scale, offset = 1, 0
    if min_val > 0: min_val = 0
    if max_val < 0: max_val = 0
    if config.policy.has_property(P.ASYMMETRICAL):
        range = float(max_val - min_val)
        scale = range / (config.quant_max - config.quant_min)
        scale = max(scale, scale_threshold)
        offset = ppq_numerical_round(float(-min_val / scale))
    elif config.policy.has_property(P.SYMMETRICAL):
        range = 2 * float(max(abs(max_val), abs(min_val)))
        scale = range / (config.quant_max - config.quant_min)
        scale = max(scale, scale_threshold)
        offset = 0
    else:
        raise TypeError('Tensor Min Max Observer Excepts either ASYMMETRICAL or SYMMETRICAL quantization config.')
    if config.policy.has_property(P.POWER_OF_2):
        scale = ppq_round_to_power_of_2(scale, policy=RoundingPolicy.ROUND_UP)
    return scale, offset


def minmax_to_scale_offset_channels(mins: np.ndarray, maxs: np.ndarray, config,
                                    scale_threshold: float = OBSERVER_MIN_SCALE) -> Tuple[list, list]:
    if config.policy.has_property(P.POWER_OF_2) or mins.dtype != np.float32 or maxs.dtype != np.float32:
        pairs = [minmax_to_scale_offset(a, b, config, scale_threshold) for a, b in zip(mins, maxs)]
        return [p[0] for p in pairs], [p[1] for p in pairs]
    if OBSERVER_MIN_SCALE_MANUL_OVERRIDE in config.detail:
        scale_threshold = config.detail[OBSERVER_MIN_SCALE_MANUL_OVERRIDE]
    zero = np.float32(0)
    lo = np.where(mins > 0, zero, mins)
    hi = np.where(maxs < 0, zero, maxs)
    levels = config.quant_max - config.quant_min
    if config.policy.has_property(P.ASYMMETRICAL):
        with np.errstate(over='ignore', divide='ignore', invalid='ignore'):
            scale = (hi - lo).astype(np.float64) / levels
            scale = np.where(scale_threshold > scale, scale_threshold, scale)
            offset = np.rint(((-lo) / scale.astype(np.float32)).astype(np.float64))
        return scale.tolist(), [int(v) for v in offset.tolist()]
    if config.policy.has_property(P.SYMMETRICAL):
        a, b = np.abs(hi), np.abs(lo)
        m = np.where(b > a, b, a)
        scale = 2 * m.astype(np.float64) / levels
        scale = np.where(scale_threshold > scale, scale_threshold, scale)
        return scale.tolist(), [0] * int(scale.size)
    raise TypeError('Tensor Min Max Observer Excepts either ASYMMETRICAL or SYMMETRICAL quantization config.')


_DEFERRED_SETS: Optional[list] = None


def _set_per_tensor(config, scale: float, offset: float, device) -> None:
    if _DEFERRED_SETS is not None:
        _DEFERRED_SETS.append((config, scale, offset, device))
        return
    config.scale = torch.tensor([scale], dtype=torch.float32, device=device).squeeze(0)
    config.offset = torch.tensor([offset], dtype=torch.float32, device=device).squeeze(0)
    set_activated(config)


def _flush_deferred_sets(pending: list) -> None:
    by_dev: Dict[object, list] = {}
    for item in pending: by_dev.setdefault(torch.device(item[3]), []).append(item)
    for dev, items in by_dev.items():
        chunks = [np.asarray(v, dtype=np.float32).reshape(-1) for _, s, o, _ in items for v in (s, o)]
        flat = torch.from_numpy(np.concatenate(chunks)).to(dev)
        pos = 0
        for k, (config, s, _, _) in enumerate(items):
            if isinstance(s, (list, tuple)):
                C = len(s)
                config.scale, config.offset = flat[pos: pos + C], flat[pos + C: pos + 2 * C]
                pos += 2 * C
            else:
                config.scale, config.offset = flat[pos], flat[pos + 1]
                pos += 2
            set_activated(config)


class ObservationQueue:
    def __init__(self, max_pending_bytes: int = 4 << 30):
        self._minmax = []
        self._minmax_c = []
        self._hist = {}
        self._quantile = {}
        self._bytes = 0
        self._max = max_pending_bytes
        self.launches = 0
        self.recorder: Optional[list] = None

    def __len__(self):
        return (len(self._minmax) + len(self._minmax_c) + sum(len(v) for v in self._hist.values())
                + sum(len(v) for v in self._quantile.values()))

    def _grow(self, value) -> None:
        self._bytes += value.numel() * 4
        if self._bytes > self._max: self.flush()

    def add_minmax(self, value: torch.Tensor, slots: torch.Tensor) -> None:
        self._minmax.append((value, slots))
        self._grow(value)

    def add_minmax_c(self, value: torch.Tensor, channel_axis: int, mins: torch.Tensor, maxs: torch.Tensor, fresh: bool) -> None:
        if any(m.data_ptr() == mins.data_ptr() for _, _, m, _, _ in self._minmax_c): self.flush()
        self._minmax_c.append((value, channel_axis, mins, maxs, bool(fresh)))
        self._grow(value)

    def add_hist(self, value: torch.Tensor, rows: torch.Tensor, asymmetric: bool, p0: float, p1: float = 0.0) -> None:
        self._hist.setdefault((bool(asymmetric), rows.shape[1], value.device), []).append((value, rows, p0, p1))
        self._grow(value)

    def add_quantile(self, value: torch.Tensor, q: float, hint: Optional[torch.Tensor] = None) -> torch.Tensor:
        dest = torch.empty(2, dtype=torch.float32, device=value.device)
        self._quantile.setdefault((float(q), value.device), []).append((value, dest, hint))
        self._grow(value)
        return dest

    def flush(self) -> None:
        if self._quantile:
            pending, self._quantile = self._quantile, {}
            for (q, _), items in pending.items():
                hints, seen = [h for _, _, h in items], set()
                for k in range(len(hints) - 1, -1, -1):
                    if hints[k] is None: continue
                    key = hints[k].data_ptr()
                    if key in seen: hints[k] = None
                    else: seen.add(key)
                CUDA.Quantile_Multi([v for v, _, _ in items], q, [d for _, d, _ in items], hints)
                self.launches += 1
        if self._minmax:
            by_dev = {}
            for v, sl in self._minmax: by_dev.setdefault(v.device, []).append((v, sl))
            self._minmax = []
            for items in by_dev.values():
                CUDA.MinMax_T_Slots_Multi([v for v, _ in items], [sl for _, sl in items])
                self.launches += 1
        if self._minmax_c:
            by_dev = {}
            for it in self._minmax_c: by_dev.setdefault(it[0].device, []).append(it)
            self._minmax_c = []
            for dev, items in by_dev.items():
                CUDA.MinMax_C_Multi([i[0] for i in items], [i[1] for i in items], [i[2] for i in items],
                                    [i[3] for i in items], [i[4] for i in items])
                self.launches += 1
        if self._hist:
            pending, self._hist = self._hist, {}
            for (asym, _, _), items in pending.items():
                vs, rows = [i[0] for i in items], [i[1] for i in items]
                if asym:
                    CUDA.Histogram_Asymmetric_T_Rows_Multi([i[2] for i in items], [i[3] for i in items], vs, rows)
                else:
                    CUDA.Histogram_T_Rows_Multi(vs, rows, [i[2] for i in items])
                self.launches += 1
        self._bytes = 0


SIBLING_PREFETCH = False
_LIVE_OBSERVERS: "weakref.WeakSet" = weakref.WeakSet()
_PREFETCHING = False


def _prefetch_siblings(ob) -> None:
    global _PREFETCHING
    if not SIBLING_PREFETCH or _PREFETCHING: return
    _PREFETCHING = True
    try:
        def device_of(o):
            t = getattr(o, '_hist', None) if getattr(o, '_hist', None) is not None else getattr(o, '_range', None)
            return None if t is None else t.device
        dev = device_of(ob)
        sibs = [o for o in list(_LIVE_OBSERVERS) if isinstance(o, TorchMinMaxObserver) and is_initial(o._quant_cfg) and device_of(o) == dev]
        if ob not in sibs: sibs.append(ob)
        _prefetch(sibs)
    finally:
        _PREFETCHING = False


class BaseTensorObserver:
    queue: Optional[ObservationQueue] = None

    def __init__(self, watch_on, quant_cfg):
        self._watch_on = watch_on
        self._quant_cfg = quant_cfg
        _LIVE_OBSERVERS.add(self)

    def _drain(self) -> None:
        if self.queue is not None and len(self.queue): self.queue.flush()

    def observe(self, value):
        raise NotImplementedError('Implement this function first.')

    def render_quantization_config(self):
        raise NotImplementedError('Implement this function first.')

    def __str__(self) -> str:
        return ('PPQ Tensor Observer (' + self.__class__.__name__ + ') mount on variable ' +
                getattr(self._watch_on, 'name', str(self._watch_on)) + ' observing algorithm: ' +
                str(self._quant_cfg.observer_algorithm))

    def report(self) -> str:
        return ''

    def pending_range(self) -> Optional[torch.Tensor]:
        return None

    def take_range(self, host: np.ndarray) -> None:
        """Receive the host copy of ``pending_range()`` (fetched for all observers at once)."""

    def reducible(self) -> List[Tuple[torch.Tensor, str]]:
        return []

    def gatherable(self) -> List[torch.Tensor]:
        return []

    def take_gathered(self, merged: List[torch.Tensor]) -> None:
        pass


_RANGE_SEEDS: Dict[object, tuple] = {}


def _range_seed(device) -> tuple:
    hit = _RANGE_SEEDS.get(device)
    if hit is None:
        one = torch.tensor([float('inf'), float('-inf')], dtype=torch.float32, device=device)
        hit = _RANGE_SEEDS[device] = (one, one.repeat(CUDA.minmax_slots(), 1).contiguous())
    return hit


class TorchMinMaxObserver(BaseTensorObserver):
    def __init__(self, watch_on, quant_cfg):
        super().__init__(watch_on, quant_cfg)
        self._range: Optional[torch.Tensor] = None
        self._slots: Optional[torch.Tensor] = None
        self._slots_dirty = False
        self._queued_c = False
        self._host_range: Optional[np.ndarray] = None
        self._observed = False

    @ torch.no_grad()
    def observe(self, value: torch.Tensor):
        assert isinstance(value, torch.Tensor), 'TorchMinMaxObserver can only deal with torch Tensor values'
        assert value.numel() > 0, (f'You are observing an empty tensor({getattr(self._watch_on, "name", "")}).')
        if not is_initial(self._quant_cfg): return
        cfg = self._quant_cfg
        if cfg.policy.has_property(P.PER_TENSOR):
            if self._range is None:
                seed = _range_seed(value.device)
                self._range = seed[0].clone()
                self._slots = seed[1].clone()
            if self.queue is not None and value.is_cuda: self.queue.add_minmax(value, self._slots)
            else: CUDA.MinMax_T_Slots(value, self._slots)
            self._slots_dirty = True
        elif cfg.policy.has_property(P.PER_CHANNEL):
            queued = (self.queue is not None and value.is_cuda and CUDA.minmax_c_outer_is_one(value, cfg.channel_axis))
            fresh = False
            if self._range is None:
                C = value.shape[cfg.channel_axis]
                self._range = torch.empty((2, C), dtype=torch.float32, device=value.device)
                fresh = queued and CUDA.minmax_c_fresh_ok(value, cfg.channel_axis)
                if not fresh: self._range[0].fill_(float('inf')); self._range[1].fill_(float('-inf'))
            if queued:
                self.queue.add_minmax_c(value, cfg.channel_axis, self._range[0], self._range[1], fresh)
                self._queued_c = True
            else: CUDA.MinMax_C(value, cfg.channel_axis, self._range[0], self._range[1])
        else:
            raise TypeError('Min-max Observer only work with per-tensor or per-channel quantize policy.')
        self._observed = True
        self._host_range = None

    def _fold(self) -> None:
        if self._queued_c:
            self._drain()
            self._queued_c = False
        if self._slots_dirty:
            self._drain()
            CUDA.MinMax_Slots_Finish(self._slots, self._range)
            self._slots_dirty = False

    def pending_range(self):
        if not (is_initial(self._quant_cfg) and self._observed): return None
        self._fold()
        return self._range

    def take_range(self, host: np.ndarray) -> None:
        self._host_range = host

    def reducible(self):
        if self._range is None: return []
        self._fold()
        if self._range.ndim == 1: return [(self._range[0:1], 'min'), (self._range[1:2], 'max')]
        return [(self._range[0], 'min'), (self._range[1], 'max')]

    def _range_on_host(self) -> np.ndarray:
        if not self._observed:
            raise ValueError('Can not render quantization config yet, Observer data collator is empty. '
                             'Invoke observe() function before render config.')
        if self._host_range is None: _prefetch_siblings(self)
        if self._host_range is None:
            self._fold()
            self._host_range = self._range.cpu().numpy()
        return self._host_range

    def render_quantization_config(self):
        if not is_initial(self._quant_cfg): return
        cfg = self._quant_cfg
        r = self._range_on_host()
        device = self._range.device
        if cfg.policy.has_property(P.PER_TENSOR):
            scale, offset = minmax_to_scale_offset(min_val=float(r[0]), max_val=float(r[1]), config=cfg)
            _set_per_tensor(cfg, scale, offset, device)
        elif cfg.policy.has_property(P.PER_CHANNEL):
            scales, offsets = minmax_to_scale_offset_channels(np.ascontiguousarray(r[0]), np.ascontiguousarray(r[1]), cfg)
            if _DEFERRED_SETS is not None:
                _DEFERRED_SETS.append((cfg, scales, offsets, device))
                return
            cfg.scale = torch.tensor(scales, dtype=torch.float32, device=device)
            cfg.offset = torch.tensor(offsets, dtype=torch.float32, device=device)
            set_activated(cfg)
        else:
            raise TypeError('Min-max Observer only work with per-tensor or per-channel quantize policy.')


class TorchHistObserver(TorchMinMaxObserver):
    def __init__(self, watch_on, quant_cfg, hist_bins: int = OBSERVER_KL_HIST_BINS):
        self._phase = 'Detecting Minmax'
        self._hist = None
        self._rows = None
        self._rows_dirty = False
        self._hist_scale = None
        self._min = None
        self._max = None
        self._losses: Optional[np.ndarray] = None
        if OBSERVER_KL_HIST_BINS_MANUL_OVERRIDE in quant_cfg.detail:
            hist_bins = quant_cfg.detail[OBSERVER_KL_HIST_BINS_MANUL_OVERRIDE]
        self._hist_bins = hist_bins
        super().__init__(watch_on, quant_cfg)

    def observe(self, value: torch.Tensor):
        if not is_initial(self._quant_cfg): return
        assert value.numel() > 0, (f'You are observing an empty tensor({getattr(self._watch_on, "name", "")}).')
        if self._phase == 'Detecting Minmax':
            if self.queue is not None and self.queue.recorder is not None and value.is_cuda:
                self.queue.recorder.append((self, value))
            return super().observe(value)
        elif self._phase == 'Collating Hist':
            self._losses = None
            if getattr(self, '_best', None) is not None: self._best = None
            if self._hist is None:
                self._hist = torch.zeros(size=(self._hist_bins,), dtype=torch.int32, device=value.device)
                if self._hist_bins <= 16384:
                    self._rows = torch.zeros(size=(CUDA.hist_rows(), self._hist_bins), dtype=torch.int32,
                                             device=value.device)
            if self._quant_cfg.policy.has_property(P.ASYMMETRICAL):
                if self._rows is not None:
                    if self.queue is not None: self.queue.add_hist(value, self._rows, True, self._min, self._max)
                    else: CUDA.Histogram_Asymmetric_T_Rows(self._min, self._max, tensor=value, rows=self._rows)
                    self._rows_dirty = True
                else:
                    CUDA.Histogram_Asymmetric_T(self._min, self._max, tensor=value, histogram=self._hist)
            elif self._quant_cfg.policy.has_property(P.SYMMETRICAL):
                if self._rows is not None:
                    if self.queue is not None: self.queue.add_hist(value, self._rows, False, self._hist_scale)
                    else: CUDA.Histogram_T_Rows(tensor=value, rows=self._rows, scale=self._hist_scale)
                    self._rows_dirty = True
                else:
                    CUDA.Histogram_T(tensor=value, histogram=self._hist, scale=self._hist_scale)
            else:
                raise TypeError('Quantization Property is invalid, expect either ASYMMETRICAL or SYMMETRICAL config here.')

    def pending_range(self):
        return super().pending_range() if self._phase == 'Detecting Minmax' else None

    def _fold_hist(self) -> None:
        if self._rows_dirty:
            self._drain()
            CUDA.Histogram_Rows_Finish(self._rows, self._hist)
            self._rows_dirty = False
            if self._rows.is_cuda: self._rows.record_stream(torch.cuda.current_stream(self._rows.device))
            self._rows = None

    def histogram(self) -> Optional[torch.Tensor]:
        self._fold_hist()
        return self._hist

    def reducible(self):
        if self._phase == 'Detecting Minmax': return super().reducible()
        return [(self.histogram(), 'sum')] if self._hist is not None else []

    search_kind = 'kl'

    def search_key(self):
        return ('kl', self._hist_bins, self._quant_cfg.num_of_bits)

    def take_losses(self, losses: np.ndarray) -> None:
        self._losses = losses

    def hist_to_scale_offset(self, histogram: torch.Tensor, hist_bins: int, hist_scale: float, config,
                             scale_threshold: float = OBSERVER_MIN_SCALE) -> Tuple[float, int]:
        if config.policy.has_property(P.ASYMMETRICAL):
            raise PermissionError('KL observer is not designed for ASYMMETRICAL quantization')
        if OBSERVER_MIN_SCALE_MANUL_OVERRIDE in config.detail:
            scale_threshold = config.detail[OBSERVER_MIN_SCALE_MANUL_OVERRIDE]
        quant_bins = 2 ** (config.num_of_bits - 1)
        if self._losses is None: _prefetch_siblings(self)
        if self._losses is None:
            self._losses = CUDA.KLLosses(histogram, config.num_of_bits).cpu().numpy()[0]
        losses = [{'kl': float(kl), 'bin_range': (j + 1) * quant_bins} for j, kl in enumerate(self._losses)]
        best_bin_range = sorted(losses, key=lambda x: x['kl'])[0]['bin_range']
        scale, offset = (best_bin_range / self._hist_bins) * hist_scale * (self._hist_bins / quant_bins), 0
        scale = max(scale, scale_threshold)
        if config.policy.has_property(P.POWER_OF_2):
            scale = ppq_round_to_power_of_2(scale, policy=RoundingPolicy.ROUND_HALF_UP)
        return scale, offset

    def render_quantization_config(self):
        if not is_initial(self._quant_cfg): return
        if not self._quant_cfg.policy.has_property(P.PER_TENSOR):
            raise ValueError('Hist observer can only apply with per-tensor quantization config.')
        if self._phase == 'Detecting Minmax':
            r = self._range_on_host()
            min_val, max_val = float(r[0]), float(r[1])
            if self._quant_cfg.policy.has_property(P.SYMMETRICAL):
                hist_range = float(max(abs(max_val), abs(min_val)))
            else:
                hist_range = max_val - min_val
            self._min = min_val
            self._max = max_val
            self._hist_scale = hist_range / self._hist_bins
            self._phase = 'Collating Hist'
        elif self._phase == 'Collating Hist':
            if self._hist is None:
                raise ValueError('Can not render quantization config yet, histogram is empty. '
                                 'Invoke observe() function before render config.')
            scale, offset = self.hist_to_scale_offset(histogram=self.histogram(), hist_bins=self._hist_bins,
                                                      hist_scale=self._hist_scale, config=self._quant_cfg)
            _set_per_tensor(self._quant_cfg, scale, offset, self._hist.device)


class ChannelwiseKLObserver(TorchHistObserver):
    def __init__(self, watch_on, quant_cfg, hist_bins: int = OBSERVER_KL_HIST_BINS):
        super().__init__(watch_on, quant_cfg, hist_bins)
        if not quant_cfg.policy.has_property(P.PER_CHANNEL) or not quant_cfg.policy.has_property(P.SYMMETRICAL):
            raise TypeError('ChannelwiseKLObserver needs a symmetrical per-channel config.')
        self._scales_dev: Optional[torch.Tensor] = None

    def observe(self, value: torch.Tensor):
        if not is_initial(self._quant_cfg): return
        assert value.numel() > 0, (f'You are observing an empty tensor({getattr(self._watch_on, "name", "")}).')
        if self._phase == 'Detecting Minmax':
            return TorchMinMaxObserver.observe(self, value)
        C = value.shape[self._quant_cfg.channel_axis]
        if self._hist is None:
            self._hist = torch.zeros(size=(C, self._hist_bins), dtype=torch.int32, device=value.device)
        CUDA.Histogram_C_Scales(value, self._quant_cfg.channel_axis, self._hist, self._scales_dev)

    def histogram(self): return self._hist

    def render_quantization_config(self):
        cfg = self._quant_cfg
        if not is_initial(cfg): return
        if self._phase == 'Detecting Minmax':
            r = self._range_on_host()
            hs = [float(max(abs(float(hi)), abs(float(lo)))) / self._hist_bins for lo, hi in zip(r[0], r[1])]
            self._hist_scale = hs
            self._scales_dev = torch.tensor(hs, dtype=torch.float32, device=self._range.device)
            self._phase = 'Collating Hist'
            return
        if self._hist is None:
            raise ValueError('Can not render quantization config yet, histogram is empty. '
                             'Invoke observe() function before render config.')
        losses = CUDA.KLLosses(self._hist, cfg.num_of_bits).cpu().numpy()
        scales = []
        for c in range(self._hist.shape[0]):
            self._losses = losses[c]
            scale, _ = self.hist_to_scale_offset(self._hist[c], self._hist_bins, self._hist_scale[c], cfg)
            scales.append(scale)
        self._losses = None
        cfg.scale = torch.tensor(scales, dtype=torch.float32, device=self._hist.device)
        cfg.offset = torch.zeros(len(scales), dtype=torch.float32, device=self._hist.device)
        set_activated(cfg)


class TorchPercentileObserver(BaseTensorObserver):
    def __init__(self, watch_on, quant_cfg):
        super().__init__(watch_on, quant_cfg)
        if OBSERVER_PERCENTILE_MANUL_OVERRIDE not in quant_cfg.detail:
            self._percentile = OBSERVER_PERCENTILE
        else: self._percentile = quant_cfg.detail[OBSERVER_PERCENTILE_MANUL_OVERRIDE]
        self._percentile_collector = []
        self._sum: Optional[torch.Tensor] = None
        self._hint: Optional[torch.Tensor] = None

    @ torch.no_grad()
    def observe(self, value: torch.Tensor):
        if not is_initial(self._quant_cfg): return
        assert value is not None, ('You are observing an Empty Tensor. '
                                   '(This Error is usually due to you have a wrong Quantizer configuration.)')
        assert value.numel() > 0, (f'You are observing an empty tensor({getattr(self._watch_on, "name", "")}).')
        assert isinstance(value, torch.Tensor), 'TorchMinMaxObserver can only deal with torch Tensor values'
        if self._quant_cfg.policy.has_property(P.PER_TENSOR):
            if value.is_cuda and (self._hint is None or self._hint.device != value.device):
                self._hint = quantile_hint(value.device)
            if self.queue is not None and value.is_cuda:
                self._percentile_collector.append(self.queue.add_quantile(value, self._percentile, self._hint).view(1, -1))
            else:
                self._percentile_collector.append(CUDA.Quantile_Hinted(value, self._percentile, self._hint).view(1, -1))
        elif self._quant_cfg.policy.has_property(P.PER_CHANNEL):
            raise PermissionError('Percentile observer can not deal with per channel quantization.')
        else:
            raise TypeError('Min-max Observer only work with per-tensor or per-channel quantize policy.')

    def _fold(self):
        self._drain()
        if self._percentile_collector:
            stacked = torch.cat(self._percentile_collector, dim=0).float()
            part = torch.cat([stacked.sum(dim=0), stacked.new_tensor([float(stacked.shape[0])])])
            self._sum = part if self._sum is None else self._sum + part
            self._percentile_collector = []

    def reducible(self):
        self._fold()
        return [(self._sum, 'sum')] if self._sum is not None else []

    def render_quantization_config(self):
        if not is_initial(self._quant_cfg): return
        if self._quant_cfg.policy.has_property(P.PER_TENSOR):
            single_shard = self._sum is None
            if single_shard and len(self._percentile_collector) == 0:
                raise ValueError('Can not render quantization config yet, Observer data collator is empty. '
                                 'Invoke observe() function before render config.')
            self._drain()
            if single_shard:
                device = self._percentile_collector[-1].device
                mean = torch.cat(self._percentile_collector, dim=0).float().mean(dim=0).cpu()
            else:
                self._fold()
                device = self._sum.device
                mean = (self._sum[:2] / self._sum[2]).cpu()
            scale, offset = minmax_to_scale_offset(min_val=mean[1].item(), max_val=mean[0].item(),
                                                   config=self._quant_cfg)
            _set_per_tensor(self._quant_cfg, scale, offset, device)
        elif self._quant_cfg.policy.has_property(P.PER_CHANNEL):
            raise PermissionError('Percentile observer can not deal with per channel quantization.')
        else:
            raise TypeError('Min-max Observer only work with per-tensor or per-channel quantize policy.')


class TorchMSEObserver(TorchHistObserver):
    search_kind = 'mse'

    def __init__(self, watch_on, quant_cfg, bins: int = OBSERVER_MSE_HIST_BINS):
        super().__init__(watch_on, quant_cfg)
        self._hist_bins = bins
        self._best: Optional[np.ndarray] = None

    def search_key(self):
        cfg = self._quant_cfg
        return ('mse', self._hist_bins, cfg.quant_min, cfg.quant_max, cfg.policy.has_property(P.SYMMETRICAL))

    def take_best(self, best: np.ndarray) -> None:
        self._best = best

    def compute_mse_loss(self, histogram: list, start: int, step: int, end: int) -> float:
        return CUDA.compute_mse_loss(histogram=histogram, start=start, step=step, end=end)

    def hist_to_scale_offset(self, histogram: torch.Tensor, hist_bins: int, hist_scale: float, config,
                             scale_threshold: float = OBSERVER_MIN_SCALE) -> Tuple[float, int]:
        if OBSERVER_MIN_SCALE_MANUL_OVERRIDE in config.detail:
            scale_threshold = config.detail[OBSERVER_MIN_SCALE_MANUL_OVERRIDE]
        if config.policy.has_property(P.PER_CHANNEL):
            raise PermissionError('Torch Mse observer do not support PER_CHANNEL policy now, please wait.')
        symmetrical = config.policy.has_property(P.SYMMETRICAL)
        if self._best is None: _prefetch_siblings(self)
        if self._best is None:
            dev = histogram.device
            self._best = CUDA.MseSearch(histogram.reshape(1, -1),
                                        torch.tensor([hist_scale], dtype=torch.float64, device=dev),
                                        torch.tensor([self._min], dtype=torch.float64, device=dev),
                                        config.quant_min, config.quant_max, symmetrical).cpu().numpy()[0]
        best_start, best_end = int(self._best[0]), int(self._best[1])
        if not symmetrical:
            range_min, range_max = (best_start * hist_scale) + self._min, (best_end * hist_scale) + self._min
        else:
            range_min, range_max = -(best_end * hist_scale), (best_end * hist_scale)
        return minmax_to_scale_offset(range_min, range_max, config, scale_threshold)


class ChannelwiseMSEObserver(TorchMSEObserver):
    def __init__(self, watch_on, quant_cfg, bins: int = OBSERVER_MSE_HIST_BINS):
        super().__init__(watch_on, quant_cfg, bins)
        if not quant_cfg.policy.has_property(P.PER_CHANNEL):
            raise TypeError('ChannelwiseMSEObserver needs a per-channel config.')
        self._mins_dev = self._maxs_dev = self._scales_dev = None

    def observe(self, value: torch.Tensor):
        if not is_initial(self._quant_cfg): return
        assert value.numel() > 0, (f'You are observing an empty tensor({getattr(self._watch_on, "name", "")}).')
        if self._phase == 'Detecting Minmax':
            return TorchMinMaxObserver.observe(self, value)
        cfg = self._quant_cfg
        C = value.shape[cfg.channel_axis]
        if self._hist is None:
            self._hist = torch.zeros(size=(C, self._hist_bins), dtype=torch.int32, device=value.device)
        if cfg.policy.has_property(P.ASYMMETRICAL):
            CUDA.Histogram_Asymmetric_C_Ranges(value, cfg.channel_axis, self._hist, self._mins_dev, self._maxs_dev)
        else:
            CUDA.Histogram_C_Scales(value, cfg.channel_axis, self._hist, self._scales_dev)

    def histogram(self): return self._hist

    def reducible(self):
        if self._phase == 'Detecting Minmax': return TorchMinMaxObserver.reducible(self)
        return [(self._hist, 'sum')] if self._hist is not None else []

    def render_quantization_config(self):
        cfg = self._quant_cfg
        if not is_initial(cfg): return
        sym = cfg.policy.has_property(P.SYMMETRICAL)
        if self._phase == 'Detecting Minmax':
            r = self._range_on_host()
            self._min = [float(v) for v in r[0]]
            self._max = [float(v) for v in r[1]]
            self._hist_scale = [(float(max(abs(hi), abs(lo))) if sym else (hi - lo)) / self._hist_bins
                                for lo, hi in zip(self._min, self._max)]
            dev = self._range.device
            self._mins_dev = torch.tensor(self._min, dtype=torch.float32, device=dev)
            self._maxs_dev = torch.tensor(self._max, dtype=torch.float32, device=dev)
            self._scales_dev = torch.tensor(self._hist_scale, dtype=torch.float32, device=dev)
            self._phase = 'Collating Hist'
            return
        if self._hist is None:
            raise ValueError('Can not render quantization config yet, histogram is empty. '
                             'Invoke observe() function before render config.')
        dev = self._hist.device
        best = CUDA.MseSearch(self._hist, torch.tensor(self._hist_scale, dtype=torch.float64, device=dev),
                              torch.tensor(self._min, dtype=torch.float64, device=dev), cfg.quant_min, cfg.quant_max,
                              sym).cpu().numpy()
        scale_threshold = cfg.detail.get(OBSERVER_MIN_SCALE_MANUL_OVERRIDE, OBSERVER_MIN_SCALE)
        scales, offsets = [], []
        for c in range(self._hist.shape[0]):
            start, end, hs = int(best[c][0]), int(best[c][1]), self._hist_scale[c]
            if sym: range_min, range_max = -(end * hs), (end * hs)
            else: range_min, range_max = (start * hs) + self._min[c], (end * hs) + self._min[c]
            s_, o_ = minmax_to_scale_offset(range_min, range_max, cfg, scale_threshold)
            scales.append(s_); offsets.append(o_)
        cfg.scale = torch.tensor(scales, dtype=torch.float32, device=dev)
        cfg.offset = torch.tensor(offsets, dtype=torch.float32, device=dev)
        set_activated(cfg)


class ConstantObserver(BaseTensorObserver):
    def __init__(self, watch_on, quant_cfg):
        super().__init__(watch_on, quant_cfg)
        self._value_shape = None
        self._value_device = None

    @ torch.no_grad()
    def observe(self, value: torch.Tensor):
        if not is_initial(self._quant_cfg): return
        self._value_shape = value.shape
        self._value_device = value.device

    def render_quantization_config(self):
        if not is_initial(self._quant_cfg): return
        device = self._value_device
        cfg = self._quant_cfg
        if cfg.policy.has_property(P.FLOATING):
            if cfg.policy.has_property(P.PER_TENSOR):
                _set_per_tensor(cfg, 1.0, 0.0, device)
            elif cfg.policy.has_property(P.PER_CHANNEL):
                num = self._value_shape[cfg.channel_axis]
                cfg.scale = torch.ones(num, dtype=torch.float32, device=device)
                cfg.offset = torch.zeros(num, dtype=torch.float32, device=device)
                set_activated(cfg)
        else:
            raise TypeError('This Observer is designed for floating quantization.')


def tensor_random_fetch(tensor: torch.Tensor, num_of_fetches: int = 1024) -> torch.Tensor:
    tensor = tensor.flatten()
    indexer = torch.randint(low=0, high=tensor.numel(), size=[num_of_fetches], device=tensor.device)
    return tensor.index_select(dim=0, index=indexer)


def channel_random_fetch(tensor: torch.Tensor, fetchs_per_channel: int = 1024, channel_axis: int = 0) -> torch.Tensor:
    tensor = tensor.transpose(0, channel_axis).flatten(start_dim=1)
    indexer = torch.randint(low=0, high=tensor.shape[-1], size=[fetchs_per_channel], device=tensor.device)
    return tensor.index_select(dim=-1, index=indexer)


class DirectMSEObserver(BaseTensorObserver):
    SCALE_CANDIDATES = [.0078125, .03125, .125, 1.0, 4.0, 16.0, 64.0]

    def __init__(self, watch_on, quant_cfg):
        super().__init__(watch_on, quant_cfg)
        if not quant_cfg.policy.has_property(P.FLOATING):
            raise TypeError('MSE Floating Observer is designed for floating quantization.')
        if not quant_cfg.policy.has_property(P.POWER_OF_2):
            raise TypeError('MSE Floating Observer is designed for power-of-2 quantization.')
        self._collector = []
        self._fetches = OBSERVER_FLOATING_MSE_FETCHES

    @ torch.no_grad()
    def observe(self, value: torch.Tensor):
        if not is_initial(self._quant_cfg): return
        cfg = self._quant_cfg
        if cfg.policy.has_property(P.PER_CHANNEL):
            if getattr(self._watch_on, 'is_parameter', False):
                value = torch.transpose(value, dim0=0, dim1=cfg.channel_axis)
                self._collector.append(torch.flatten(value, start_dim=1))
            else:
                self._collector.append(channel_random_fetch(value, fetchs_per_channel=self._fetches,
                                                            channel_axis=cfg.channel_axis))
        if cfg.policy.has_property(P.PER_TENSOR):
            self._collector.append(tensor_random_fetch(value, num_of_fetches=self._fetches))

    def search_item(self):
        cfg = self._quant_cfg
        if cfg.policy.has_property(P.PER_CHANNEL): fp = torch.cat(self._collector, dim=-1).contiguous()
        else: fp = torch.cat(self._collector, dim=0).reshape(1, -1).contiguous()
        return (fp, cfg.exponent_bits, cfg.mantissa_bits, cfg.quant_min, cfg.quant_max)

    def take_squared_errors(self, sse: torch.Tensor, row_len: int) -> None:
        per_channel = self._quant_cfg.policy.has_property(P.PER_CHANNEL)
        self._sse = sse if per_channel else sse.reshape(-1)
        self._count = torch.full([sse.shape[0] if per_channel else 1], float(row_len), dtype=torch.float64, device=sse.device)

    def take_best(self, index) -> None:
        self._best = list(index)

    def _squared_errors(self):
        item = self.search_item()
        r = int(getattr(self._quant_cfg.rounding, 'value', self._quant_cfg.rounding))
        self.take_squared_errors(CUDA.FloatScaleSearch([item], self.SCALE_CANDIDATES, r), item[0].shape[1])
        return self._sse, self._count

    def reducible(self):
        if not is_initial(self._quant_cfg) or not self._collector: return []
        self._sse, self._count = self._squared_errors()
        return [(self._sse, 'sum'), (self._count, 'sum')]

    def render_quantization_config(self):
        if not is_initial(self._quant_cfg): return
        if not self._collector:
            raise PermissionError('Observer collector is empty, you should invoke observe function'
                                  ' before render quantization config.')
        cfg = self._quant_cfg
        r = int(getattr(cfg.rounding, 'value', cfg.rounding))
        e, m, lo, hi = cfg.exponent_bits, cfg.mantissa_bits, cfg.quant_min, cfg.quant_max
        best = getattr(self, '_best', None)
        if best is not None:
            dev = self._collector[0].device
            cfg.scale = torch.tensor([self.SCALE_CANDIDATES[i] for i in best], dtype=torch.float32, device=dev)
            cfg.offset = torch.zeros(len(best), dtype=torch.float32, device=dev)
            self._best = self._sse = None
            set_activated(cfg)
            return
        merged = getattr(self, '_sse', None)
        if merged is not None:
            mean = merged / (self._count.unsqueeze(-1) if merged.ndim == 2 else self._count)
            dev = merged.device
            if cfg.policy.has_property(P.PER_CHANNEL):
                index = torch.argmin(mean, dim=-1).cpu().tolist()
                cfg.scale = torch.tensor([self.SCALE_CANDIDATES[i] for i in index], dtype=torch.float32, device=dev)
                cfg.offset = torch.zeros(len(index), dtype=torch.float32, device=dev)
            else:
                best_scale = sorted(zip(mean.cpu().tolist(), self.SCALE_CANDIDATES))[0][1]
                cfg.scale = torch.tensor([best_scale], dtype=torch.float32, device=dev)
                cfg.offset = torch.zeros(1, dtype=torch.float32, device=dev)
            self._sse = None
            set_activated(cfg)
            return
        if cfg.policy.has_property(P.PER_CHANNEL):
            fp = torch.cat(self._collector, dim=-1).contiguous()
            C = fp.shape[0]
            zeros = torch.zeros(C, dtype=torch.float32, device=fp.device)
            losses = []
            for scale in self.SCALE_CANDIDATES:
                s = torch.full([C], scale, dtype=torch.float32, device=fp.device)
                qt = CUDA.FloatingQuantize_C(fp, s, zeros, 0, e, m, lo, hi, r)
                losses.append(torch.mean(torch.square(qt - fp), dim=-1, keepdim=True))
            index = torch.argmin(torch.cat(losses, dim=-1), dim=-1).cpu().tolist()
            cfg.scale = torch.tensor([self.SCALE_CANDIDATES[i] for i in index], dtype=torch.float32, device=fp.device)
            cfg.offset = zeros
        else:
            fp = torch.cat(self._collector, dim=0).contiguous()
            zero = torch.zeros(1, dtype=torch.float32, device=fp.device)
            losses = []
            for scale in self.SCALE_CANDIDATES:
                s = torch.full([1], scale, dtype=torch.float32, device=fp.device)
                qt = CUDA.FloatingQuantize_T(fp, s, zero, e, m, lo, hi, r)
                losses.append(torch.mean(torch.square(qt - fp)).reshape(1))
            host = torch.cat(losses).cpu().tolist()
            best_scale = sorted(zip(host, self.SCALE_CANDIDATES))[0][1]
            cfg.scale = torch.tensor([best_scale], dtype=torch.float32, device=fp.device)
            cfg.offset = zero
        set_activated(cfg)


class TorchIsotoneObserver(BaseTensorObserver):
    def __init__(self, watch_on, quant_cfg):
        super().__init__(watch_on, quant_cfg)
        self._pairs: List[torch.Tensor] = []
        self.axis = quant_cfg.detail.get(OBSERVER_ISOTONE_OBSERVER_AXIS, -1)

    @ torch.no_grad()
    def observe(self, value: torch.Tensor):
        if not is_initial(self._quant_cfg): return
        assert isinstance(value, torch.Tensor), 'IsotoneObserver can only deal with torch Tensor values'
        assert value.numel() > 0, f'You are observing an empty tensor({getattr(self._watch_on, "name", "?")}).'
        policy = self._quant_cfg.policy
        if policy.has_property(P.PER_CHANNEL):
            raise TypeError('Isotone Observer is not designed for channelwise quantization.')
        if not policy.has_property(P.PER_TENSOR):
            raise TypeError('Isotone Observer only work with per-tensor or per-channel quantize policy.')
        rows = value
        if rows.ndim > 1: rows = rows.transpose(self.axis, -1).flatten(0, -2)
        top2 = torch.topk(rows, k=2, dim=self.axis, largest=True, sorted=True).values
        self._pairs.append(top2.reshape(1, -1) if top2.ndim <= 1 else top2)

    def gatherable(self):
        if not is_initial(self._quant_cfg) or not self._pairs: return []
        self._pairs = [torch.cat(self._pairs, dim=0).contiguous()]
        return [self._pairs[0]]

    def take_gathered(self, merged):
        self._pairs = [merged[0]]

    def render_quantization_config(self):
        cfg = self._quant_cfg
        if not is_initial(cfg): return
        device = self._pairs[-1].device
        pairs = torch.cat(self._pairs, dim=0).cpu().numpy().astype(np.float32, copy=False)
        l1, l2 = pairs[:, 0], pairs[:, 1]
        if cfg.policy.has_property(P.SYMMETRICAL): l1, l2 = np.abs(l1), np.abs(l2)
        f32 = np.float32
        lower = np.maximum(l2 / f32(cfg.quant_max - .51), f32(0))
        upper = f32(2) * (l1 - np.maximum(l2, f32(0)))
        usable = (upper > lower) & (l1 > 0)

        def _tensor(v): return torch.tensor([v], dtype=torch.float32, device=device).squeeze(0)
        if not usable.any():
            scale, offset = minmax_to_scale_offset(min_val=0, max_val=l1[-1], config=cfg)
            cfg.scale, cfg.offset = _tensor(scale), _tensor(offset)
            set_activated(cfg)
            return
        ends = np.concatenate([upper[usable], lower[usable]])
        opens = np.concatenate([np.zeros(int(usable.sum()), np.int8), np.ones(int(usable.sum()), np.int8)])
        order = np.lexsort((opens, ends))
        depth = np.cumsum(np.where(opens[order] == 1, 1, -1))
        best = int(np.argmax(depth))
        cfg.scale, cfg.offset = _tensor(ends[order][best]), _tensor(0)
        set_activated(cfg)
        self.s_candidates = [(v, 'min' if o else 'max') for v, o in zip(ends[order].tolist(), opens[order].tolist())]


OBSERVER_TABLE = {
    'minmax': TorchMinMaxObserver,
    'kl': TorchHistObserver,
    'kl_channel': ChannelwiseKLObserver,
    'percentile': TorchPercentileObserver,
    'mse': TorchMSEObserver,
    'mse_channel': ChannelwiseMSEObserver,
    'isotone': TorchIsotoneObserver,
    'constant': ConstantObserver,
    'floating': DirectMSEObserver,
}


def register_calibration_observer(algorithm: str, observer: type) -> None:
    if not isinstance(observer, type):
        raise TypeError(f'You can only register an observer CLASS as custimized ppq observer, however {type(observer)} is given. ')
    if not issubclass(observer, BaseTensorObserver):
        raise TypeError('Regitsing observer must be a subclass of BaseTensorObserver.')
    OBSERVER_TABLE[str(algorithm).lower()] = observer


class TensorObserverFactroy:
    def __init__(self) -> None:
        raise NotImplementedError('Observer Factory can not be initialized, use TensorObserverFactroy.build_observer instead.')

    @ classmethod
    def build_observer(cls, variable, config) -> BaseTensorObserver:
        algorithm = str(config.observer_algorithm.lower())
        if algorithm not in OBSERVER_TABLE:
            raise ValueError(f'Observer type not understand, Except one of {OBSERVER_TABLE.keys()}, '
                             f'while {str(algorithm)} was given.')
        return OBSERVER_TABLE[algorithm](watch_on=variable, quant_cfg=config)


class CalibrationHook:
    def __init__(self, operation, observer_table: Dict[object, BaseTensorObserver], stream=None) -> None:
        self._hook_to = operation
        self._operation = operation
        self._observer_table = observer_table
        self.stream = stream

    def _observe_all(self, values: list, quant_configs: list) -> None:
        todo = [(v, self._observer_table[c]) for v, c in zip(values, quant_configs) if c in self._observer_table]
        if not todo: return
        if self.stream is None or not todo[0][0].is_cuda:
            for v, ob in todo: ob.observe(v)
            return
        self.stream.wait_stream(torch.cuda.current_stream(todo[0][0].device))
        with torch.cuda.stream(self.stream):
            capturing = torch.cuda.is_current_stream_capturing()
            for v, ob in todo:
                ob.observe(v)
                if not capturing: v.record_stream(self.stream)

    def pre_forward_hook(self, inputs: list, quant_inputs: list, quant_configs: list) -> list:
        self._observe_all(inputs, quant_configs)
        return quant_inputs

    def post_forward_hook(self, outputs: list, quant_outputs: list, quant_configs: list) -> list:
        self._observe_all(outputs, quant_configs)
        return quant_outputs

    def render_quantization_config(self):
        if self.stream is not None: torch.cuda.current_stream().wait_stream(self.stream)
        for _, observer in self._observer_table.items():
            observer.render_quantization_config()
            observer.report()

    def __str__(self) -> str:
        return ''.join([observer.__str__() + '\n' for _, observer in self._observer_table.items()])


class OperationObserver:
    def __init__(self, operation, monitor_parameter: bool = True, monitor_outputs: bool = True,
                 monitor_inputs: bool = True) -> None:
        if not hasattr(operation, 'config'):
            raise TypeError(f'Only QuantableOP instance can apply an Observer, while {type(operation)} was given.')
        self._operation = operation
        self._hook = self.build_hook(monitor_parameter=monitor_parameter, monitor_outputs=monitor_outputs,
                                     monitor_inputs=monitor_inputs)

    def render_quantization_config(self):
        self.hook.render_quantization_config()

    def build_hook(self, monitor_parameter: bool, monitor_outputs: bool, monitor_inputs: bool) -> CalibrationHook:
        observer_table = {}
        for var, config in zip(self._operation.inputs, self._operation.config.input_quantization_config):
            if is_initial(config):
                if var in self._operation.parameters and monitor_parameter:
                    observer_table[config] = TensorObserverFactroy.build_observer(var, config)
                elif monitor_inputs:
                    observer_table[config] = TensorObserverFactroy.build_observer(var, config)
        if monitor_outputs:
            for var, config in zip(self._operation.outputs, self._operation.config.output_quantization_config):
                if is_initial(config):
                    observer_table[config] = TensorObserverFactroy.build_observer(var, config)
        return CalibrationHook(operation=self._operation, observer_table=observer_table)

    @ property
    def hook(self) -> CalibrationHook:
        return self._hook

    def observers(self) -> List[BaseTensorObserver]:
        return list(self._hook._observer_table.values())

    def report(self) -> str:
        return str(self._hook)


def render_observers(observers: Sequence[BaseTensorObserver]) -> None:
    observers = [ob for ob in observers if is_initial(ob._quant_cfg)]
    _prefetch(observers)
    global _DEFERRED_SETS
    _DEFERRED_SETS = pending = []
    try:
        for ob in observers:
            ob.render_quantization_config()
    finally:
        _DEFERRED_SETS = None
        _flush_deferred_sets(pending)


def _prefetch(observers: Sequence[BaseTensorObserver]) -> None:
    pend = [(ob, ob.pending_range()) for ob in observers if getattr(ob, '_host_range', None) is None]
    pend = [(ob, r) for ob, r in pend if r is not None]
    if pend:
        flat = torch.cat([r.reshape(-1) for _, r in pend]).cpu().numpy()
        pos = 0
        for ob, r in pend:
            n = r.numel()
            ob.take_range(flat[pos: pos + n].reshape(tuple(r.shape)))
            pos += n
    groups: Dict[tuple, List[TorchHistObserver]] = {}
    for ob in observers:
        if isinstance(ob, TorchHistObserver) and ob._phase == 'Collating Hist' and ob._hist is not None:
            if ob._losses is not None or getattr(ob, '_best', None) is not None: continue
            if ob._quant_cfg.policy.has_property(P.PER_TENSOR):
                groups.setdefault(ob.search_key(), []).append(ob)
    for key, obs in groups.items():
        hists = torch.stack([ob.histogram() for ob in obs])
        if key[0] == 'kl':
            if any(ob._quant_cfg.policy.has_property(P.ASYMMETRICAL) for ob in obs): continue
            losses = CUDA.KLLosses(hists, key[2]).cpu().numpy()
            for ob, l in zip(obs, losses): ob.take_losses(l)
        else:
            dev = hists.device
            hs = torch.tensor([ob._hist_scale for ob in obs], dtype=torch.float64, device=dev)
            mn = torch.tensor([ob._min for ob in obs], dtype=torch.float64, device=dev)
            best = CUDA.MseSearch(hists, hs, mn, key[2], key[3], key[4]).cpu().numpy()
            for ob, b in zip(obs, best): ob.take_best(b)
    fobs = [ob for ob in observers if isinstance(ob, DirectMSEObserver) and ob._collector]
    if fobs:
        by_round: Dict[int, list] = {}
        for ob in fobs:
            if getattr(ob, '_sse', None) is None:
                by_round.setdefault(int(getattr(ob._quant_cfg.rounding, 'value', ob._quant_cfg.rounding)), []).append(ob)
        for r, obs in by_round.items():
            items = [ob.search_item() for ob in obs]
            sse = CUDA.FloatScaleSearch(items, DirectMSEObserver.SCALE_CANDIDATES, r)
            pos = 0
            for ob, it in zip(obs, items):
                rows = it[0].shape[0]
                ob.take_squared_errors(sse[pos: pos + rows], it[0].shape[1]); pos += rows
        means = [(ob._sse.reshape(-1, len(DirectMSEObserver.SCALE_CANDIDATES)) / ob._count.reshape(-1, 1)) for ob in fobs]
        best = torch.argmin(torch.cat(means), dim=-1).cpu().tolist()
        pos = 0
        for ob, m in zip(fobs, means):
            ob.take_best(best[pos: pos + m.shape[0]]); pos += m.shape[0]
```

Measured before the change: 3518 samples/s.

## Fuse calibration min/max and histogram statistics into bias-activation epilogue kernels

Adds epilogue kernels that apply bias, residual add and ReLU while also gathering per-tensor min/max or histogram statistics into the observer's slot or row buffers. The executor passes observer sinks to these kernels and skips the separate observe launches for tensors they have already covered. The aim is to avoid re-reading each activation from HBM in a standalone statistics kernel, and to cut kernel launches. In exchange, the epilogue kernels use more LDS and registers and carry more template variants. There is a fallback path for unsupported cases such as unaligned pointers, ReLU off, or histograms that exceed the LDS limit.

New measurement: 3604 samples/s, median of 4. +2.4%, better.

```diff
diff --git a/include/ppq_hip.h b/include/ppq_hip.h
--- a/include/ppq_hip.h
+++ b/include/ppq_hip.h
@@ -225,6 +225,20 @@
                     int relu, void* stream);
 int ppqhip_bias_add_act(float* a, const float* bias_a, float* b, const float* bias_b, float* out,
                         int64_t n, int64_t num_channel, int64_t elem_per_channel, int relu, void* stream);
+
+typedef struct ppqhip_epilogue_sink {
+    float* slots;
+    int32_t* rows;
+    int32_t kind;
+    int32_t num_bins, clip_outliers;
+    float p0, p1;
+    int32_t store;
+} ppqhip_epilogue_sink;
+int ppqhip_bias_act_stat(float* y, const float* bias, int64_t n, int64_t num_channel, int64_t elem_per_channel, int relu,
+                         const ppqhip_epilogue_sink* sinks, void* stream);
+int ppqhip_bias_add_act_stat(float* a, const float* bias_a, float* b, const float* bias_b, float* out, int64_t n,
+                             int64_t num_channel, int64_t elem_per_channel, int relu, const ppqhip_epilogue_sink* sinks,
+                             void* stream);
 
 typedef struct ppqhip_adaround_job {
     const float* w;
diff --git a/ppq_amd/_lib.py b/ppq_amd/_lib.py
--- a/ppq_amd/_lib.py
+++ b/ppq_amd/_lib.py
@@ -38,6 +38,8 @@
     'ppqhip_lsq_finish_multi': (c_int, [c_vp, c_int, c_vp]),
     'ppqhip_bias_act': (c_int, [c_f32p, c_f32p, c_i64, c_i64, c_i64, c_int, c_vp]),
     'ppqhip_bias_add_act': (c_int, [c_f32p, c_f32p, c_f32p, c_f32p, c_f32p, c_i64, c_i64, c_i64, c_int, c_vp]),
+    'ppqhip_bias_act_stat': (c_int, [c_f32p, c_f32p, c_i64, c_i64, c_i64, c_int, c_vp, c_vp]),
+    'ppqhip_bias_add_act_stat': (c_int, [c_f32p, c_f32p, c_f32p, c_f32p, c_f32p, c_i64, c_i64, c_i64, c_int, c_vp, c_vp]),
     'ppqhip_fq_float_t': (c_int, [c_f32p, c_f32p, c_f32p, c_f32p, c_i64, c_int, c_int, c_flt, c_flt, c_int, c_vp]),
     'ppqhip_fq_float_c': (c_int, [c_f32p, c_f32p, c_f32p, c_f32p, c_i64, c_i64, c_i64, c_int, c_int, c_flt, c_flt,
                                   c_int, c_vp]),
diff --git a/ppq_amd/calibration.py b/ppq_amd/calibration.py
--- a/ppq_amd/calibration.py
+++ b/ppq_amd/calibration.py
@@ -29,7 +29,7 @@
                  process_group=None, check_steps: bool = True, async_observe: bool = False,
                  use_hip_graph: bool = False, batch_observations: bool = True,
                  reuse_activations: bool = False, reuse_budget_bytes: int = 64 << 30,
-                 queue_bytes: int = None) -> None:
+                 queue_bytes: int = None, fuse_statistics: bool = True) -> None:
         super().__init__(name='PPQ Runtime Calibration Pass')
         self._method = method
         self._observers: Dict[str, OperationObserver] = {}
@@ -41,6 +41,7 @@
         self._async_observe = async_observe
         self._use_hip_graph = use_hip_graph
         self._batch_observations = batch_observations
+        self._fuse_statistics = fuse_statistics
         self._queue = None
         self._reuse_activations = reuse_activations
         self._queue_bytes = queue_bytes
@@ -82,8 +83,14 @@
         import torch
         recording = self._queue is not None and self._recording
         if recording: self._queue.recorder = []
-        with torch.no_grad():
-            self._forward_fn(executor)(inputs=data, hooks=hooks, output_names=output_names)
+        fuse = (self._fuse_statistics and self._queue is not None and not self._reuse_activations
+                and hasattr(executor, 'fuse_statistics'))
+        if fuse: previous, executor.fuse_statistics = executor.fuse_statistics, True
+        try:
+            with torch.no_grad():
+                self._forward_fn(executor)(inputs=data, hooks=hooks, output_names=output_names)
+        finally:
+            if fuse: executor.fuse_statistics = previous
         if self._queue is not None: self._queue.flush()
         if recording:
             rec, self._queue.recorder = self._queue.recorder, None
diff --git a/ppq_amd/csrc/epilogue.hip b/ppq_amd/csrc/epilogue.hip
--- a/ppq_amd/csrc/epilogue.hip
+++ b/ppq_amd/csrc/epilogue.hip
@@ -1,4 +1,5 @@
 #include "common.hpp"
+#include "hist_binner.hpp"
 
 namespace ppqhip {
 namespace {
@@ -120,6 +121,309 @@
         if (plane) PPQ_LAUNCH_EP(kEpTileU, true); else PPQ_LAUNCH_EP(kEpTileU, false);
     }
 #undef PPQ_LAUNCH_EP
+}
+
+constexpr int kEpSinks = 3;
+constexpr size_t kEpStatLdsBytes = 64u << 10;
+enum EpStat : int { EP_MINMAX = 0, EP_HIST_SYM = 1, EP_HIST_ASYM = 2 };
+
+struct EpSinkArg {
+    float* slots;
+    int* rows;
+    float a0, hs;
+    int lds_off;
+    int on;
+    int store;
+};
+struct EpStatArgs {
+    EpArgs p;
+    EpSinkArg sink[kEpSinks];
+    uint32_t tiles;
+    uint32_t full;
+    int bins;
+};
+
+template <bool RESID, bool BIAS_B, bool PLANE, int STAT, bool CLIP, bool NT>
+__global__ __launch_bounds__(kHistBlock, (kHistBlock * kHistWgPerCu + 255) / 256)
+void epilogue_stat_kernel(const EpStatArgs q) {
+    extern __shared__ int lds[];
+    constexpr bool HIST = STAT != EP_MINMAX, ASYM = STAT == EP_HIST_ASYM;
+    constexpr int NS = RESID ? 3 : 1;
+    const EpArgs& p = q.p;
+    const uint32_t g = blockIdx.x;
+    uint32_t t, t_end;
+    even_split(q.tiles, gridDim.x, g, t, t_end);
+    if (t >= t_end) return;
+    float4* a4 = reinterpret_cast<float4*>(p.a);
+    float4* b4 = reinterpret_cast<float4*>(p.b);
+    float4* o4 = reinterpret_cast<float4*>(p.out);
+    const int bins = q.bins;
+
+    Binner<ASYM, CLIP, true> acc[NS];
+    float mn[NS], mx[NS];
+#pragma unroll
+    for (int s = 0; s < NS; s++) {
+        if (HIST) { acc[s].init(lds + q.sink[s].lds_off, bins); acc[s].set_rule(q.sink[s].a0, q.sink[s].hs); }
+        mn[s] = INFINITY; mx[s] = -INFINITY;
+    }
+    bool zeroed = !HIST;
+    auto zero_lds = [&]() __attribute__((always_inline)) {
+        if (zeroed) return;
+        int total = 0;
+#pragma unroll
+        for (int s = 0; s < NS; s++) if (q.sink[s].on) total += bins;
+        for (int i = threadIdx.x; i < total; i += kHistBlock) lds[i] = 0;
+        asm volatile("s_waitcnt lgkmcnt(0)\n\ts_barrier" ::: "memory");
+        zeroed = true;
+    };
+    auto stat4 = [&](int s, const float4& v, bool first) __attribute__((always_inline)) {
+        if (!q.sink[s].on) return;
+        if (HIST) {
+            int b[4];
+            acc[s].bins4(v, b);
+            if (first) acc[s].elect(b[0], true);
+            if (CLIP) acc[s].commit4_exec(b);
+            else {
+                acc[s].template commit<true>(b[0], true); acc[s].template commit<true>(b[1], true);
+                acc[s].template commit<true>(b[2], true); acc[s].template commit<true>(b[3], true);
+            }
+        } else {
+            mn[s] = fminf(fminf(mn[s], v.x), fminf(v.y, fminf(v.z, v.w)));
+            mx[s] = fmaxf(fmaxf(mx[s], v.x), fmaxf(v.y, fmaxf(v.z, v.w)));
+        }
+    };
+    auto stat1 = [&](int s, float v, bool in, bool first) __attribute__((always_inline)) {
+        if (!q.sink[s].on) return;
+        if (HIST) {
+            const int b = acc[s].bin1(v);
+            if (first) acc[s].elect(b, in);
+            acc[s].template commit<false>(b, in);
+        } else if (in) { mn[s] = fminf(mn[s], v); mx[s] = fmaxf(mx[s], v); }
+    };
+
+    struct Tile { float4 a[kHistU], ba[kHistU], b[kHistU], bb[kHistU]; };
+    auto fetch = [&](Tile& T, uint32_t tile) __attribute__((always_inline)) {
+        const uint32_t v0 = tile * kTileVec + threadIdx.x;
+#pragma unroll
+        for (int u = 0; u < kHistU; u++) {
+            const uint32_t v = v0 + u * kHistBlock;
+            T.a[u] = load4<NT>(a4 + v);
+            T.ba[u] = bias4<PLANE>(p.bias_a, v, p.epc, p.nc);
+            if (RESID) T.b[u] = load4<NT>(b4 + v);
+            if (BIAS_B) T.bb[u] = bias4<PLANE>(p.bias_b, v, p.epc, p.nc);
+        }
+    };
+    auto consume = [&](const Tile& T, uint32_t tile) __attribute__((always_inline)) {
+        const uint32_t v0 = tile * kTileVec + threadIdx.x;
+#pragma unroll
+        for (int u = 0; u < kHistU; u++) {
+            const uint32_t v = v0 + u * kHistBlock;
+            const float4 x = add4(T.a[u], T.ba[u]);
+            if (!RESID) {
+                const float4 r = act4<true>(x);
+                a4[v] = r;
+                stat4(0, r, u == 0);
+            } else {
+                if (q.sink[0].store) a4[v] = x;
+                stat4(0, x, u == 0);
+                float4 y = T.b[u];
+                if (BIAS_B) { y = add4(y, T.bb[u]); if (q.sink[1].store) b4[v] = y; }
+                stat4(1, y, u == 0);
+                const float4 r = act4<true>(add4(x, y));
+                o4[v] = r;
+                stat4(2, r, u == 0);
+            }
+        }
+    };
+
+    const uint32_t kf = min(t_end, q.full);
+    if (t < kf) {
+        Tile ta, tb;
+        uint32_t k = t;
+        fetch(ta, k);
+        zero_lds();
+        for (;;) {
+            fetch(tb, min(k + 1, kf - 1));
+            consume(ta, k);
+            if (++k >= kf) break;
+            fetch(ta, min(k + 1, kf - 1));
+            consume(tb, k);
+            if (++k >= kf) break;
+        }
+    }
+    if (t_end > q.full) {
+        const uint32_t v0 = q.full * kTileVec + threadIdx.x;
+        const float4 zero4 = make_float4(0.f, 0.f, 0.f, 0.f);
+        Tile T;
+        bool in[kHistU];
+#pragma unroll
+        for (int u = 0; u < kHistU; u++) {
+            const uint32_t v = v0 + u * kHistBlock;
+            in[u] = v < p.nvec;
+            T.a[u] = T.ba[u] = T.b[u] = T.bb[u] = zero4;
+            if (in[u]) {
+                T.a[u] = a4[v];
+                T.ba[u] = bias4<PLANE>(p.bias_a, v, p.epc, p.nc);
+                if (RESID) T.b[u] = b4[v];
+                if (BIAS_B) T.bb[u] = bias4<PLANE>(p.bias_b, v, p.epc, p.nc);
+            }
+        }
+        zero_lds();
+        auto stat4m = [&](int s, const float4& w, bool ok) __attribute__((always_inline)) {
+            stat1(s, w.x, ok, true); stat1(s, w.y, ok, false); stat1(s, w.z, ok, false); stat1(s, w.w, ok, false);
+        };
+#pragma unroll
+        for (int u = 0; u < kHistU; u++) {
+            const uint32_t v = v0 + u * kHistBlock;
+            const float4 x = add4(T.a[u], T.ba[u]);
+            if (!RESID) {
+                const float4 r = act4<true>(x);
+                if (in[u]) a4[v] = r;
+                stat4m(0, r, in[u]);
+            } else {
+                if (in[u] && q.sink[0].store) a4[v] = x;
+                stat4m(0, x, in[u]);
+                float4 y = T.b[u];
+                if (BIAS_B) { y = add4(y, T.bb[u]); if (in[u] && q.sink[1].store) b4[v] = y; }
+                stat4m(1, y, in[u]);
+                const float4 r = act4<true>(add4(x, y));
+                if (in[u]) o4[v] = r;
+                stat4m(2, r, in[u]);
+            }
+        }
+        if (!PLANE && p.ntail > 0) {
+            const bool ok = (int)threadIdx.x < p.ntail;
+            const uint32_t i = ok ? p.tail + threadIdx.x : p.tail;
+            const uint32_t c = channel_of(i, p.epc, p.nc);
+            const float x = p.a[i] + p.bias_a[c];
+            if (!RESID) {
+                const float r = act(x, true);
+                if (ok) p.a[i] = r;
+                stat1(0, ok ? r : 0.f, ok, true);
+            } else {
+                if (ok && q.sink[0].store) p.a[i] = x;
+                stat1(0, ok ? x : 0.f, ok, true);
+                float y = p.b[i];
+                if (BIAS_B) { y = y + p.bias_b[c]; if (ok && q.sink[1].store) p.b[i] = y; }
+                stat1(1, ok ? y : 0.f, ok, true);
+                const float r = act(x + y, true);
+                if (ok) p.out[i] = r;
+                stat1(2, ok ? r : 0.f, ok, true);
+            }
+        }
+    }
+
+    if (HIST) {
+#pragma unroll
+        for (int s = 0; s < NS; s++) if (q.sink[s].on) acc[s].flush_hot();
+        asm volatile("s_waitcnt lgkmcnt(0)" ::: "memory");
+        __syncthreads();
+#pragma unroll
+        for (int s = 0; s < NS; s++) {
+            if (!q.sink[s].on) continue;
+            const int* h = lds + q.sink[s].lds_off;
+            int* __restrict__ dst = q.sink[s].rows + (size_t)g * bins;
+            for (int b = threadIdx.x; b < bins; b += kHistBlock) {
+                const int c = h[b];
+                if (c) dst[b] += c;
+            }
+        }
+    } else {
+        __shared__ float red[2 * NS * (kHistBlock / kWave)];
+        const int wid = threadIdx.x >> 6, lane = threadIdx.x & 63;
+#pragma unroll
+        for (int s = 0; s < NS; s++) {
+            const float lo = wave_min(mn[s]), hi = wave_max(mx[s]);
+            if (lane == 0) { red[(2 * s) * (kHistBlock / kWave) + wid] = lo; red[(2 * s + 1) * (kHistBlock / kWave) + wid] = hi; }
+        }
+        __syncthreads();
+#pragma unroll
+        for (int s = 0; s < NS; s++) {
+            if ((int)threadIdx.x != s || !q.sink[s].on) continue;
+            float lo = INFINITY, hi = -INFINITY;
+            for (int w = 0; w < kHistBlock / kWave; w++) {
+                lo = fminf(lo, red[(2 * s) * (kHistBlock / kWave) + w]);
+                hi = fmaxf(hi, red[(2 * s + 1) * (kHistBlock / kWave) + w]);
+            }
+            float* slot = q.sink[s].slots + 2 * (size_t)g;
+            slot[0] = fminf(lo, slot[0]);
+            slot[1] = fmaxf(hi, slot[1]);
+        }
+    }
+}
+
+template <bool RESID, bool BIAS_B, bool PLANE, bool NT>
+void launch_stat_kind(const EpStatArgs& q, int stat, bool clip, int grid, size_t lds, hipStream_t st) {
+#define PPQ_LAUNCH_EP_STAT(S, C)                                                                                         \
+    hipLaunchKernelGGL((epilogue_stat_kernel<RESID, BIAS_B, PLANE, S, C, NT>), dim3(grid), dim3(kHistBlock), lds, st, q)
+    if (stat == EP_MINMAX) PPQ_LAUNCH_EP_STAT(EP_MINMAX, false);
+    else if (stat == EP_HIST_SYM) { if (clip) PPQ_LAUNCH_EP_STAT(EP_HIST_SYM, true); else PPQ_LAUNCH_EP_STAT(EP_HIST_SYM, false); }
+    else { if (clip) PPQ_LAUNCH_EP_STAT(EP_HIST_ASYM, true); else PPQ_LAUNCH_EP_STAT(EP_HIST_ASYM, false); }
+#undef PPQ_LAUNCH_EP_STAT
+}
+
+template <bool RESID, bool BIAS_B>
+int launch_epilogue_stat(EpArgs p, int64_t n, int64_t C, int64_t epc, bool aligned, int relu, const ppqhip_epilogue_sink* sinks,
+                         hipStream_t st, const char* what) {
+    constexpr int NS = RESID ? 3 : 1;
+    if (sinks == nullptr) { set_error("%s: sinks is null", what); return PPQHIP_ERR_INVALID_VALUE; }
+    int kind = 0, bins = 0, clip = 0, on = 0;
+    for (int s = 0; s < NS; s++) {
+        const ppqhip_epilogue_sink& k = sinks[s];
+        if (k.kind < 0 || k.kind > 3) { set_error("%s: sink %d has kind %d", what, s, k.kind); return PPQHIP_ERR_INVALID_VALUE; }
+        if (k.kind == 0) continue;
+        if (kind != 0 && k.kind != kind) { set_error("%s: the sinks of one launch must have one kind", what); return PPQHIP_ERR_INVALID_VALUE; }
+        if (k.kind == 1 ? k.slots == nullptr : k.rows == nullptr) { set_error("%s: sink %d has a null buffer", what, s); return PPQHIP_ERR_INVALID_VALUE; }
+        if (k.kind != 1) {
+            if (k.num_bins <= 0 || (on && (k.num_bins != bins || (k.clip_outliers != 0) != (clip != 0)))) {
+                set_error("%s: the histogram sinks of one launch must share num_bins > 0 and clip_outliers", what);
+                return PPQHIP_ERR_INVALID_VALUE;
+            }
+            bins = k.num_bins; clip = k.clip_outliers;
+        }
+        kind = k.kind; on++;
+    }
+    const size_t lds = kind >= 2 ? sizeof(int) * (size_t)on * (size_t)bins : 0;
+    if (!aligned || !relu || lds > kEpStatLdsBytes) {
+        set_error("%s: not fused (unaligned pointer, relu off, or %zu B of LDS histograms)", what, lds);
+        return PPQHIP_ERR_UNSUPPORTED;
+    }
+    EpStatArgs q{};
+    p.nc = make_fastdiv((uint32_t)C);
+    p.nvec = (uint32_t)(n >> 2);
+    p.tail = p.nvec * 4u;
+    p.ntail = (int)(n & 3);
+    const bool plane = (epc % 4 == 0);
+    p.epc = make_fastdiv((uint32_t)(plane ? epc / 4 : epc));
+    q.p = p;
+    q.bins = bins;
+    int off = 0;
+    for (int s = 0; s < NS; s++) {
+        const ppqhip_epilogue_sink& k = sinks[s];
+        EpSinkArg& d = q.sink[s];
+        d.on = k.kind != 0;
+        d.store = (RESID && s < 2) ? (k.store != 0) : 1;
+        d.slots = k.slots; d.rows = k.rows;
+        if (k.kind == 3) { d.a0 = k.p0; d.hs = (k.p1 - k.p0) / (float)bins; }
+        else { d.a0 = 0.f; d.hs = k.p0; }
+        if (k.kind >= 2) { d.lds_off = off; off += bins; }
+    }
+    q.full = p.nvec / kTileVec;
+    q.tiles = q.full + ((uint64_t)n > (uint64_t)q.full * kTileElems ? 1u : 0u);
+    int64_t cap = (int64_t)num_cu() * kHistWgPerCu;
+    if (cap > ppqhip_hist_rows()) cap = ppqhip_hist_rows();
+    if (cap > ppqhip_minmax_slots()) cap = ppqhip_minmax_slots();
+    const int grid = (int)((int64_t)q.tiles < cap ? (int64_t)q.tiles : cap);
+    const int stat = kind <= 1 ? EP_MINMAX : (kind == 2 ? EP_HIST_SYM : EP_HIST_ASYM);
+    const bool nt = n * (RESID ? 2 : 1) >= kHistNtElems;
+    if (plane) {
+        if (nt) launch_stat_kind<RESID, BIAS_B, true, true>(q, stat, clip != 0, grid, lds, st);
+        else launch_stat_kind<RESID, BIAS_B, true, false>(q, stat, clip != 0, grid, lds, st);
+    } else {
+        if (nt) launch_stat_kind<RESID, BIAS_B, false, true>(q, stat, clip != 0, grid, lds, st);
+        else launch_stat_kind<RESID, BIAS_B, false, false>(q, stat, clip != 0, grid, lds, st);
+    }
+    return finish_launch(what);
 }
 
 int validate(int64_t n, int64_t C, int64_t epc, const char* what) {
@@ -173,4 +477,27 @@
     return finish_launch("bias_add_act");
 }
 
-}
+int ppqhip_bias_act_stat(float* y, const float* bias, int64_t n, int64_t num_channel, int64_t elem_per_channel, int relu,
+                         const ppqhip_epilogue_sink* sinks, void* stream) {
+    if (int st = validate(n, num_channel, elem_per_channel, "bias_act_stat")) return st;
+    if (!y || !bias) { set_error("bias_act_stat: null pointer"); return PPQHIP_ERR_INVALID_VALUE; }
+    EpArgs p{};
+    p.a = y; p.bias_a = bias;
+    return launch_epilogue_stat<false, false>(p, n, num_channel, elem_per_channel, aligned16(y), relu, sinks, (hipStream_t)stream,
+                                              "bias_act_stat");
+}
+
+int ppqhip_bias_add_act_stat(float* a, const float* bias_a, float* b, const float* bias_b, float* out, int64_t n,
+                             int64_t num_channel, int64_t elem_per_channel, int relu, const ppqhip_epilogue_sink* sinks,
+                             void* stream) {
+    if (int st = validate(n, num_channel, elem_per_channel, "bias_add_act_stat")) return st;
+    if (!a || !bias_a || !b || !out) { set_error("bias_add_act_stat: null pointer"); return PPQHIP_ERR_INVALID_VALUE; }
+    EpArgs p{};
+    p.a = a; p.bias_a = bias_a; p.b = b; p.bias_b = bias_b; p.out = out;
+    const bool aligned = aligned16(a) && aligned16(b) && aligned16(out);
+    hipStream_t s = (hipStream_t)stream;
+    if (bias_b) return launch_epilogue_stat<true, true>(p, n, num_channel, elem_per_channel, aligned, relu, sinks, s, "bias_add_act_stat");
+    return launch_epilogue_stat<true, false>(p, n, num_channel, elem_per_channel, aligned, relu, sinks, s, "bias_add_act_stat");
+}
+
+}
diff --git a/ppq_amd/csrc/hist.hip b/ppq_amd/csrc/hist.hip
--- a/ppq_amd/csrc/hist.hip
+++ b/ppq_amd/csrc/hist.hip
@@ -1,91 +1,12 @@
 #include "common.hpp"
+#include "hist_binner.hpp"
 
 namespace ppqhip {
 
 constexpr int kMaxLdsBins = 16384;
 constexpr int kLdsBudgetInts = 2048;
-constexpr int kHistBlock = 512;
-constexpr int kHistWgPerCu = 2;
-constexpr int kHistU = 2;
 constexpr int kHistMinTiles = 2;
 constexpr int kHistAtomicMaxWg = 128;
-constexpr long long kHistNtElems = 48ll << 20;
-constexpr int kHistRows = kNumCU * kHistWgPerCu;
-constexpr uint32_t kTileVec = (uint32_t)kHistBlock * kHistU;
-constexpr uint32_t kTileElems = kTileVec * 4;
-static_assert(kHistBlock % 64 == 0 && kHistBlock >= 64 && kHistBlock <= 1024, "histogram workgroup: whole waves");
-
-typedef float v2f __attribute__((ext_vector_type(2)));
-
-struct BinRule {
-    float a;
-    float hs;
-    float rcp;
-    int bins;
-    int clip;
-    int asym;
-};
-static BinRule make_rule(float a, float hs, int bins, int clip, int asym) {
-    BinRule r; r.a = a; r.hs = hs; r.rcp = 1.0f / hs; r.bins = bins; r.clip = clip; r.asym = asym;
-    return r;
-}
-
-__device__ __forceinline__ bool quotient_is_safe(float t) {
-    return __builtin_fabsf(t - __builtin_rintf(t)) >= __builtin_fabsf(t) * 0x1p-22f;
-}
-
-__device__ __forceinline__ int f2i_abs(float t) {
-    int r;
-    asm("v_cvt_i32_f32_e64 %0, |%1|" : "=v"(r) : "v"(t));
-    return r;
-}
-__device__ __forceinline__ int f2i_floor(float t) {
-    int r;
-    asm("v_cvt_flr_i32_f32 %0, %1" : "=v"(r) : "v"(t));
-    return r;
-}
-
-template <bool ASYM, bool CLIP, bool HOT>
-struct Binner : WaveBinCounter<ASYM, CLIP, HOT> {
-    using Base = WaveBinCounter<ASYM, CLIP, HOT>;
-    using Base::h; using Base::last; using Base::hot_bin; using Base::hot_cnt;
-    float a0, hs, rcp;
-
-    __device__ __forceinline__ void set_rule(float a, float scale) { a0 = a; hs = scale; rcp = 1.0f / scale; }
-
-    __device__ __forceinline__ void bins4(const float4& v, int (&b)[4]) const {
-        v2f x01 = {v.x, v.y}, x23 = {v.z, v.w};
-        if (ASYM) { x01 = x01 - a0; x23 = x23 - a0; }
-        const v2f t01 = x01 * rcp, t23 = x23 * rcp;
-        const v2f r01 = {__builtin_rintf(t01.x), __builtin_rintf(t01.y)};
-        const v2f r23 = {__builtin_rintf(t23.x), __builtin_rintf(t23.y)};
-        const v2f d01 = t01 - r01, d23 = t23 - r23;
-        const v2f e01 = t01 * 0x1p-22f, e23 = t23 * 0x1p-22f;
-        const bool u0 = !(__builtin_fabsf(d01.x) >= __builtin_fabsf(e01.x));
-        const bool u1 = !(__builtin_fabsf(d01.y) >= __builtin_fabsf(e01.y));
-        const bool u2 = !(__builtin_fabsf(d23.x) >= __builtin_fabsf(e23.x));
-        const bool u3 = !(__builtin_fabsf(d23.y) >= __builtin_fabsf(e23.y));
-        b[0] = ASYM ? f2i_floor(t01.x) : f2i_abs(t01.x);
-        b[1] = ASYM ? f2i_floor(t01.y) : f2i_abs(t01.y);
-        b[2] = ASYM ? f2i_floor(t23.x) : f2i_abs(t23.x);
-        b[3] = ASYM ? f2i_floor(t23.y) : f2i_abs(t23.y);
-        if (u0 | u1 | u2 | u3) {
-            if (u0) b[0] = exact_bin(ASYM ? x01.x : __builtin_fabsf(v.x));
-            if (u1) b[1] = exact_bin(ASYM ? x01.y : __builtin_fabsf(v.y));
-            if (u2) b[2] = exact_bin(ASYM ? x23.x : __builtin_fabsf(v.z));
-            if (u3) b[3] = exact_bin(ASYM ? x23.y : __builtin_fabsf(v.w));
-        }
-    }
-    __device__ __forceinline__ int exact_bin(float a) const { return f2i_sat(__builtin_floorf(a / hs)); }
-
-    __device__ __forceinline__ int bin1(float v) const {
-        const float a = ASYM ? (v - a0) : __builtin_fabsf(v);
-        const float t = a * rcp;
-        if (quotient_is_safe(t)) return ASYM ? f2i_floor(t) : f2i_abs(t);
-        return exact_bin(a);
-    }
-
-};
 
 constexpr int kReduceBins = 32, kReduceSlices = 32, kReduceBlock = kReduceBins * kReduceSlices;
 __global__ __launch_bounds__(kReduceBlock) void hist_reduce_kernel(const int* __restrict__ partial, int count, int bins,
diff --git a/ppq_amd/csrc/hist_binner.hpp b/ppq_amd/csrc/hist_binner.hpp
--- /dev/null
+++ b/ppq_amd/csrc/hist_binner.hpp
@@ -0,0 +1,88 @@
+#pragma once
+
+#include "common.hpp"
+
+namespace ppqhip {
+
+constexpr int kHistBlock = 512;
+constexpr int kHistWgPerCu = 2;
+constexpr int kHistU = 2;
+constexpr long long kHistNtElems = 48ll << 20;
+constexpr int kHistRows = kNumCU * kHistWgPerCu;
+constexpr uint32_t kTileVec = (uint32_t)kHistBlock * kHistU;
+constexpr uint32_t kTileElems = kTileVec * 4;
+static_assert(kHistBlock % 64 == 0 && kHistBlock >= 64 && kHistBlock <= 1024, "histogram workgroup: whole waves");
+
+typedef float v2f __attribute__((ext_vector_type(2)));
+
+struct BinRule {
+    float a;
+    float hs;
+    float rcp;
+    int bins;
+    int clip;
+    int asym;
+};
+inline BinRule make_rule(float a, float hs, int bins, int clip, int asym) {
+    BinRule r; r.a = a; r.hs = hs; r.rcp = 1.0f / hs; r.bins = bins; r.clip = clip; r.asym = asym;
+    return r;
+}
+
+__device__ __forceinline__ bool quotient_is_safe(float t) {
+    return __builtin_fabsf(t - __builtin_rintf(t)) >= __builtin_fabsf(t) * 0x1p-22f;
+}
+
+__device__ __forceinline__ int f2i_abs(float t) {
+    int r;
+    asm("v_cvt_i32_f32_e64 %0, |%1|" : "=v"(r) : "v"(t));
+    return r;
+}
+__device__ __forceinline__ int f2i_floor(float t) {
+    int r;
+    asm("v_cvt_flr_i32_f32 %0, %1" : "=v"(r) : "v"(t));
+    return r;
+}
+
+template <bool ASYM, bool CLIP, bool HOT>
+struct Binner : WaveBinCounter<ASYM, CLIP, HOT> {
+    using Base = WaveBinCounter<ASYM, CLIP, HOT>;
+    using Base::h; using Base::last; using Base::hot_bin; using Base::hot_cnt;
+    float a0, hs, rcp;
+
+    __device__ __forceinline__ void set_rule(float a, float scale) { a0 = a; hs = scale; rcp = 1.0f / scale; }
+
+    __device__ __forceinline__ void bins4(const float4& v, int (&b)[4]) const {
+        v2f x01 = {v.x, v.y}, x23 = {v.z, v.w};
+        if (ASYM) { x01 = x01 - a0; x23 = x23 - a0; }
+        const v2f t01 = x01 * rcp, t23 = x23 * rcp;
+        const v2f r01 = {__builtin_rintf(t01.x), __builtin_rintf(t01.y)};
+        const v2f r23 = {__builtin_rintf(t23.x), __builtin_rintf(t23.y)};
+        const v2f d01 = t01 - r01, d23 = t23 - r23;
+        const v2f e01 = t01 * 0x1p-22f, e23 = t23 * 0x1p-22f;
+        const bool u0 = !(__builtin_fabsf(d01.x) >= __builtin_fabsf(e01.x));
+        const bool u1 = !(__builtin_fabsf(d01.y) >= __builtin_fabsf(e01.y));
+        const bool u2 = !(__builtin_fabsf(d23.x) >= __builtin_fabsf(e23.x));
+        const bool u3 = !(__builtin_fabsf(d23.y) >= __builtin_fabsf(e23.y));
+        b[0] = ASYM ? f2i_floor(t01.x) : f2i_abs(t01.x);
+        b[1] = ASYM ? f2i_floor(t01.y) : f2i_abs(t01.y);
+        b[2] = ASYM ? f2i_floor(t23.x) : f2i_abs(t23.x);
+        b[3] = ASYM ? f2i_floor(t23.y) : f2i_abs(t23.y);
+        if (u0 | u1 | u2 | u3) {
+            if (u0) b[0] = exact_bin(ASYM ? x01.x : __builtin_fabsf(v.x));
+            if (u1) b[1] = exact_bin(ASYM ? x01.y : __builtin_fabsf(v.y));
+            if (u2) b[2] = exact_bin(ASYM ? x23.x : __builtin_fabsf(v.z));
+            if (u3) b[3] = exact_bin(ASYM ? x23.y : __builtin_fabsf(v.w));
+        }
+    }
+    __device__ __forceinline__ int exact_bin(float a) const { return f2i_sat(__builtin_floorf(a / hs)); }
+
+    __device__ __forceinline__ int bin1(float v) const {
+        const float a = ASYM ? (v - a0) : __builtin_fabsf(v);
+        const float t = a * rcp;
+        if (quotient_is_safe(t)) return ASYM ? f2i_floor(t) : f2i_abs(t);
+        return exact_bin(a);
+    }
+
+};
+
+}
diff --git a/ppq_amd/ffi.py b/ppq_amd/ffi.py
--- a/ppq_amd/ffi.py
+++ b/ppq_amd/ffi.py
@@ -183,6 +183,83 @@
     with _DeviceOf(a):
         _raise(lib.ppqhip_bias_add_act(a.data_ptr(), bias_a.data_ptr(), b.data_ptr(), 0 if bias_b is None else bias_b.data_ptr(),
                                        out.data_ptr(), a.numel(), geo[0], geo[1], 1 if relu else 0, _stream()))
+    return out
+
+
+_EPILOGUE_SINK = np.dtype([('slots', '<u8'), ('rows', '<u8'), ('kind', '<i4'), ('num_bins', '<i4'), ('clip_outliers', '<i4'),
+                           ('p0', '<f4'), ('p1', '<f4'), ('store', '<i4')])
+_NOT_FUSED = -2
+
+
+class StatSink:
+    NONE, MINMAX, HIST_SYM, HIST_ASYM = 0, 1, 2, 3
+    __slots__ = ('kind', 'slots', 'rows', 'clip_outliers', 'p0', 'p1', 'store')
+
+    def __init__(self, kind: int, slots=None, rows=None, p0: float = 0.0, p1: float = 0.0, clip_outliers: bool = True,
+                 store: bool = True):
+        self.kind, self.slots, self.rows, self.p0, self.p1 = kind, slots, rows, p0, p1
+        self.clip_outliers, self.store = clip_outliers, store
+
+    def compatible(self, other: 'StatSink') -> bool:
+        if self.kind != other.kind: return False
+        return self.kind == StatSink.MINMAX or (self.rows.shape[1] == other.rows.shape[1]
+                                                and bool(self.clip_outliers) == bool(other.clip_outliers))
+
+
+def _sink_table(sinks, count: int, dev) -> np.ndarray:
+    if len(sinks) != count: raise RuntimeError(_KERNEL_FAILURE + f'expected {count} sinks, got {len(sinks)}')
+    table = np.zeros(count, dtype=_EPILOGUE_SINK)
+    table['store'] = 1
+    for k, sk in enumerate(sinks):
+        if sk is None: continue
+        if sk.kind == StatSink.NONE:
+            if sk.slots is not None: table[k]['slots'] = sk.slots.data_ptr()
+            if sk.rows is not None: table[k]['rows'], table[k]['num_bins'] = sk.rows.data_ptr(), sk.rows.shape[1]
+            table[k]['store'] = int(bool(sk.store))
+            continue
+        if sk.kind == StatSink.MINMAX:
+            t = sk.slots
+            _f32(t, 'Slots')
+            if t.numel() != 2 * lib.ppqhip_minmax_slots() or not t.is_contiguous() or t.device != dev:
+                raise RuntimeError(_KERNEL_FAILURE + 'slots must be a contiguous [minmax_slots(), 2] tensor on the values\' device')
+            table[k]['slots'] = t.data_ptr()
+        elif sk.kind in (StatSink.HIST_SYM, StatSink.HIST_ASYM):
+            t = sk.rows
+            _check(t, torch.int32, 'Rows(Expect to be INT32)')
+            if t.ndim != 2 or t.shape[0] != lib.ppqhip_hist_rows() or not t.is_contiguous() or t.device != dev:
+                raise RuntimeError(_KERNEL_FAILURE + 'rows must be a contiguous [hist_rows(), bins] tensor on the values\' device')
+            table[k]['rows'] = t.data_ptr()
+            table[k]['num_bins'] = t.shape[1]
+            table[k]['clip_outliers'] = int(bool(sk.clip_outliers))
+            table[k]['p0'], table[k]['p1'] = sk.p0, sk.p1
+        else:
+            raise RuntimeError(_KERNEL_FAILURE + f'unknown sink kind {sk.kind}')
+        table[k]['kind'] = sk.kind
+        table[k]['store'] = int(bool(sk.store))
+    return table
+
+
+def bias_act_stat_(y: torch.Tensor, bias: torch.Tensor, sinks) -> bool:
+    geo = _epilogue_geometry([y], [bias])
+    if geo is None: return False
+    table = _sink_table(sinks, 1, y.device)
+    with _DeviceOf(y):
+        st = lib.ppqhip_bias_act_stat(y.data_ptr(), bias.data_ptr(), y.numel(), geo[0], geo[1], 1, table.ctypes.data, _stream())
+    if st == _NOT_FUSED: return False
+    _raise(st)
+    return True
+
+
+def bias_add_act_stat(a: torch.Tensor, bias_a: torch.Tensor, b: torch.Tensor, bias_b, sinks):
+    geo = _epilogue_geometry([a, b], [bias_a] if bias_b is None else [bias_a, bias_b])
+    if geo is None or a.data_ptr() == b.data_ptr(): return None
+    table = _sink_table(sinks, 3, a.device)
+    out = torch.empty_like(a)
+    with _DeviceOf(a):
+        st = lib.ppqhip_bias_add_act_stat(a.data_ptr(), bias_a.data_ptr(), b.data_ptr(), 0 if bias_b is None else bias_b.data_ptr(),
+                                          out.data_ptr(), a.numel(), geo[0], geo[1], 1, table.ctypes.data, _stream())
+    if st == _NOT_FUSED: return None
+    _raise(st)
     return out
 
 
diff --git a/ppq_amd/harness.py b/ppq_amd/harness.py
--- a/ppq_amd/harness.py
+++ b/ppq_amd/harness.py
@@ -236,6 +236,30 @@
     return groups
 
 
+def plan_statistic_sinks(grp: EpilogueGroup, hooks: Dict[str, object]) -> Dict[str, tuple]:
+    from .observer import CalibrationHook
+    hooks = hooks or {}
+    member_hooks = [hooks.get(op.name) for op in grp.ops]
+    if any(h is not None and type(h) is not CalibrationHook for h in member_hooks): return {}
+
+    def hook_of(op): return hooks.get(op.name)
+    relu = grp.relu
+    if grp.kind == 'P1':
+        conv = grp.convs[0]
+        receivers = {'y': [(hook_of(conv), _out_cfg(conv, 0)), (hook_of(relu), _in_cfg(relu, 0)), (hook_of(relu), _out_cfg(relu, 0))]}
+    else:
+        add, conv_a = grp.add, grp.convs[0]
+        conv_b = grp.convs[1] if len(grp.convs) > 1 else None
+        receivers = {'a': [(hook_of(conv_a), _out_cfg(conv_a, 0)), (hook_of(add), _in_cfg(add, 0))],
+                     'b': ([(hook_of(conv_b), _out_cfg(conv_b, 0))] if conv_b is not None else []) + [(hook_of(add), _in_cfg(add, 1))],
+                     'out': [(hook_of(add), _out_cfg(add, 0)), (hook_of(relu), _in_cfg(relu, 0)), (hook_of(relu), _out_cfg(relu, 0))]}
+    plan = {}
+    for slot, pairs in receivers.items():
+        observed = [(h, c) for h, c in pairs if h is not None and c is not None and c in h._observer_table]
+        if len(observed) == 1: plan[slot] = observed[0]
+    return plan
+
+
 class TorchExecutor:
     def __init__(self, graph: BaseGraph, device: str = 'cuda'):
         self._graph = graph
@@ -251,6 +275,7 @@
         self._delegates: Dict[object, Callable] = {}
         self.fuse_epilogues = True
         self._epilogue_cache: Dict[tuple, dict] = {}
+        self.fuse_statistics = False
         self.channels_last = False
         for v in graph.variables.values():
             if v.is_parameter and v.value is not None: v.value = v.value.to(device)
@@ -387,7 +412,7 @@
         return plan
 
     def _run_epilogue(self, grp: EpilogueGroup, raw_of: Callable, hooks) -> Optional[Dict[str, torch.Tensor]]:
-        from .ffi import bias_act_, bias_add_act
+        from .ffi import bias_act_, bias_act_stat_, bias_add_act, bias_add_act_stat
         for conv in grp.convs:
             x, w = raw_of(conv.inputs[0]), conv.inputs[1].value
             if not (isinstance(x, torch.Tensor) and x.is_cuda and x.dtype == torch.float32 and x.dim() == 4
@@ -415,24 +440,54 @@
                                      groups=a.get('group', 1))
             biases[conv.name] = qin[2]
             qins[conv.name] = qin
+        stat_plan = plan_statistic_sinks(grp, hooks) if (self.fuse_statistics and hooks) else {}
+        served = {}
+
+        def sinks_for(slots, like):
+            sinks, first = [], None
+            for slot in slots:
+                sink = None
+                if slot in stat_plan:
+                    hook, cfg = stat_plan[slot]
+                    sink = hook.fused_sink(cfg, like)
+                    if sink is not None and first is not None and not sink.compatible(first): sink = None
+                    if sink is not None:
+                        first = first or sink
+                        served[slot] = (hook, cfg)
+                sinks.append(sink)
+            return sinks
         if grp.kind == 'P1':
             conv = grp.convs[0]
             y = ys[conv.name]
-            if not bias_act_(y, biases[conv.name], relu=True):
-                y.add_(biases[conv.name].view(1, -1, 1, 1)).relu_()
+            sinks = sinks_for(('y',), y) if stat_plan else None
+            if not (served and bias_act_stat_(y, biases[conv.name], sinks)):
+                served = {}
+                if not bias_act_(y, biases[conv.name], relu=True):
+                    y.add_(biases[conv.name].view(1, -1, 1, 1)).relu_()
             tail = {conv.name: y, grp.relu.name: y}
         else:
             conv_a = grp.convs[0]
             a = ys[conv_a.name]
             conv_b = grp.convs[1] if len(grp.convs) > 1 else None
             b = ys[conv_b.name] if conv_b is not None else raw_of(grp.add.inputs[1])
-            out = bias_add_act(a, biases[conv_a.name], b, biases[conv_b.name] if conv_b is not None else None, relu=True)
+            bias_b = biases[conv_b.name] if conv_b is not None else None
+            sinks = sinks_for(('a', 'b', 'out'), a) if stat_plan else None
+            out = bias_add_act_stat(a, biases[conv_a.name], b, bias_b, sinks) if served else None
+            if out is None:
+                served = {}
+                out = bias_add_act(a, biases[conv_a.name], b, bias_b, relu=True)
             if out is None:
                 a.add_(biases[conv_a.name].view(1, -1, 1, 1))
                 if conv_b is not None: b.add_(biases[conv_b.name].view(1, -1, 1, 1))
                 out = F.relu(a + b)
             tail = {conv_a.name: a, grp.add.name: out, grp.relu.name: out}
             if conv_b is not None: tail[conv_b.name] = b
+        for hook, cfg in served.values(): hook.mark_observed(cfg)
+        done = {(id(hook), id(cfg)) for hook, cfg in served.values()}
+
+        def unserved(hook, cfgs):
+            if not done or cfgs is None: return cfgs
+            return [None if (id(hook), id(c)) in done else c for c in cfgs]
         values: Dict[str, torch.Tensor] = {}
         for op in grp.ops:
             hook = hooks.get(op.name)
@@ -443,14 +498,14 @@
                 if quantable:
                     in_cfgs = list(op.config.input_quantization_config)
                     qin = [self.quantize_function(x, c) for x, c in zip(raw_in, in_cfgs)]
-                if hook is not None: hook.pre_forward_hook(inputs=raw_in, quant_inputs=qin, quant_configs=in_cfgs)
+                if hook is not None: hook.pre_forward_hook(inputs=raw_in, quant_inputs=qin, quant_configs=unserved(hook, in_cfgs))
             outs = fp_outs = [tail[op.name]]
             out_cfgs = None
             if quantable:
                 out_cfgs = list(op.config.output_quantization_config)
                 outs = [self.quantize_function(y, c) for y, c in zip(outs, out_cfgs)]
             if hook is not None:
-                outs = hook.post_forward_hook(outputs=fp_outs, quant_outputs=outs, quant_configs=out_cfgs)
+                outs = hook.post_forward_hook(outputs=fp_outs, quant_outputs=outs, quant_configs=unserved(hook, out_cfgs))
             for v, y in zip(op.outputs, outs): values[v.name] = y
         return values
 
diff --git a/ppq_amd/observer.py b/ppq_amd/observer.py
--- a/ppq_amd/observer.py
+++ b/ppq_amd/observer.py
@@ -10,7 +10,7 @@
                    OBSERVER_PERCENTILE, OBSERVER_PERCENTILE_MANUL_OVERRIDE, is_initial, set_activated)
 from .core import QuantizationProperty as P
 from .core import RoundingPolicy
-from .ffi import CUDA, quantile_hint
+from .ffi import CUDA, StatSink, quantile_hint
 from .round import ppq_numerical_round, ppq_round_to_power_of_2
 
 
@@ -206,6 +206,12 @@
     def observe(self, value):
         raise NotImplementedError('Implement this function first.')
 
+    def fused_sink(self, value_like) -> Optional[StatSink]:
+        return None
+
+    def mark_observed(self) -> None:
+        """A producer kernel has added one tensor's statistic into the sink: sets what ``observe`` sets besides launching."""
+
     def render_quantization_config(self):
         raise NotImplementedError('Implement this function first.')
 
@@ -285,6 +291,26 @@
         self._observed = True
         self._host_range = None
 
+    def _sink_allowed(self, value_like) -> bool:
+        cfg = self._quant_cfg
+        return (type(self) in _SINK_OBSERVERS
+                and all(any(k.__dict__['observe'] is fn for fn in _PLAIN_OBSERVE) for k in type(self).__mro__ if 'observe' in k.__dict__)
+                and is_initial(cfg) and cfg.policy.has_property(P.PER_TENSOR) and bool(getattr(value_like, 'is_cuda', False))
+                and (self.queue is None or self.queue.recorder is None))
+
+    def fused_sink(self, value_like) -> Optional[StatSink]:
+        if not self._sink_allowed(value_like): return None
+        if self._range is None:
+            seed = _range_seed(value_like.device)
+            self._range = seed[0].clone()
+            self._slots = seed[1].clone()
+        return StatSink(StatSink.MINMAX, slots=self._slots)
+
+    def mark_observed(self) -> None:
+        self._slots_dirty = True
+        self._observed = True
+        self._host_range = None
+
     def _fold(self) -> None:
         if self._queued_c:
             self._drain()
@@ -363,11 +389,7 @@
         elif self._phase == 'Collating Hist':
             self._losses = None
             if getattr(self, '_best', None) is not None: self._best = None
-            if self._hist is None:
-                self._hist = torch.zeros(size=(self._hist_bins,), dtype=torch.int32, device=value.device)
-                if self._hist_bins <= 16384:
-                    self._rows = torch.zeros(size=(CUDA.hist_rows(), self._hist_bins), dtype=torch.int32,
-                                             device=value.device)
+            self._alloc_hist(value.device)
             if self._quant_cfg.policy.has_property(P.ASYMMETRICAL):
                 if self._rows is not None:
                     if self.queue is not None: self.queue.add_hist(value, self._rows, True, self._min, self._max)
@@ -384,6 +406,29 @@
                     CUDA.Histogram_T(tensor=value, histogram=self._hist, scale=self._hist_scale)
             else:
                 raise TypeError('Quantization Property is invalid, expect either ASYMMETRICAL or SYMMETRICAL config here.')
+
+    def _alloc_hist(self, device) -> None:
+        if self._hist is None:
+            self._hist = torch.zeros(size=(self._hist_bins,), dtype=torch.int32, device=device)
+            if self._hist_bins <= 16384:
+                self._rows = torch.zeros(size=(CUDA.hist_rows(), self._hist_bins), dtype=torch.int32, device=device)
+
+    def fused_sink(self, value_like) -> Optional[StatSink]:
+        if self._phase == 'Detecting Minmax': return super().fused_sink(value_like)
+        if self._phase != 'Collating Hist' or not self._sink_allowed(value_like): return None
+        policy = self._quant_cfg.policy
+        asym = policy.has_property(P.ASYMMETRICAL)
+        if not asym and not policy.has_property(P.SYMMETRICAL): return None
+        self._alloc_hist(value_like.device)
+        if self._rows is None: return None
+        if asym: return StatSink(StatSink.HIST_ASYM, rows=self._rows, p0=self._min, p1=self._max)
+        return StatSink(StatSink.HIST_SYM, rows=self._rows, p0=self._hist_scale)
+
+    def mark_observed(self) -> None:
+        if self._phase == 'Detecting Minmax': return super().mark_observed()
+        self._losses = None
+        if getattr(self, '_best', None) is not None: self._best = None
+        self._rows_dirty = True
 
     def pending_range(self):
         return super().pending_range() if self._phase == 'Detecting Minmax' else None
@@ -664,6 +709,10 @@
         cfg.scale = torch.tensor(scales, dtype=torch.float32, device=dev)
         cfg.offset = torch.tensor(offsets, dtype=torch.float32, device=dev)
         set_activated(cfg)
+
+
+_SINK_OBSERVERS = (TorchMinMaxObserver, TorchHistObserver, TorchMSEObserver)
+_PLAIN_OBSERVE = tuple(k.__dict__['observe'] for k in (BaseTensorObserver, TorchMinMaxObserver, TorchHistObserver))
 
 
 class ConstantObserver(BaseTensorObserver):
@@ -926,6 +975,15 @@
                 ob.observe(v)
                 if not capturing: v.record_stream(self.stream)
 
+    def fused_sink(self, config, value_like) -> Optional[StatSink]:
+        if type(self) is not CalibrationHook or CalibrationHook.__dict__['_observe_all'] is not _PLAIN_OBSERVE_ALL: return None
+        if self.stream is not None or config is None: return None
+        ob = self._observer_table.get(config)
+        return None if ob is None else ob.fused_sink(value_like)
+
+    def mark_observed(self, config) -> None:
+        self._observer_table[config].mark_observed()
+
     def pre_forward_hook(self, inputs: list, quant_inputs: list, quant_configs: list) -> list:
         self._observe_all(inputs, quant_configs)
         return quant_inputs
@@ -942,6 +1000,9 @@
 
     def __str__(self) -> str:
         return ''.join([observer.__str__() + '\n' for _, observer in self._observer_table.items()])
+
+
+_PLAIN_OBSERVE_ALL = CalibrationHook.__dict__['_observe_all']
 
 
 class OperationObserver:
```
